# zhizdev/sparsefusion

Measured on AMD Instinct MI355X. Metric: novel views/sec, distillation steps (2 NGP renders fwd+bwd + VAE enc/dec + 51-eval PLMS + LPIPS), 256^2 / 32x32 latents, 2-view synthetic hydrant, higher is better.
Workload: dtype bf16 MFMA operands / f32 accumulate (UNet); f32 (NGP render)

## Files before the change

### sparsefusion_amd/csrc/attn_ln.h

```cpp
#pragma once
#include "sf_dev.h"

SF_KERNEL(256) void k_layernorm(const float* __restrict__ in, const float* __restrict__ gain,
                                                   const float* __restrict__ bias, void* __restrict__ out,
                                                   const float* __restrict__ resid, int R, int C, float eps, int pre_gelu,
                                                   int out_f32) {
  SF_SHARED float red[8];
  const int row = blockIdx.x, lane = threadIdx.x & 63, wv = threadIdx.x >> 6;
  const float* x = in + (long)row * C;
  float v[8];
  float s = 0.0f;
#pragma unroll
  for (int i = 0; i < 8; ++i) {
    const int c = threadIdx.x + i * 256;
    v[i] = 0.0f;
    if (c < C) { const float t = x[c]; v[i] = pre_gelu ? sf_gelu(t) : t; s += v[i]; }
  }
  s = sf_wave_sum(s);
  if (lane == 0) red[wv] = s;
  sf_sync();
  const float mean = (red[0] + red[1] + red[2] + red[3]) / (float)C;
  float q = 0.0f;
#pragma unroll
  for (int i = 0; i < 8; ++i)
    if (threadIdx.x + i * 256 < C) { const float d = v[i] - mean; q = fmaf(d, d, q); }
  q = sf_wave_sum(q);
  if (lane == 0) red[4 + wv] = q;
  sf_sync();
  const float rstd = sf_rsqrt((red[4] + red[5] + red[6] + red[7]) / (float)C + eps);
#pragma unroll
  for (int i = 0; i < 8; ++i) {
    const int c = threadIdx.x + i * 256;
    if (c < C) {
      float y = (v[i] - mean) * rstd * gain[c];
      if (bias) y += bias[c];
      if (out_f32) {
        if (resid) y += resid[(long)row * C + c];
        reinterpret_cast<float*>(out)[(long)row * C + c] = y;
      } else {
        reinterpret_cast<sf_opnd*>(out)[(long)row * C + c] = (sf_opnd)y;
      }
    }
  }
}

template <int NV>
SF_KERNEL(256) void k_layernorm_wave(const float* __restrict__ in, const float* __restrict__ gain, const float* __restrict__ bias,
                                     void* __restrict__ out, const float* __restrict__ resid, int R, float eps, int pre_gelu, int out_f32) {
  constexpr int C = 256 * NV;
  const int lane = threadIdx.x & 63;
  long row = (long)blockIdx.x * 4 + (threadIdx.x >> 6);
  const bool live = row < R;
  if (!live) row = R - 1;
  f32x4 v[NV], g[NV], bq[NV], rq[NV];
  const float* x = in + row * C;
  const float* bp = bias ? bias : gain;
  const float* rp = resid ? resid + row * C : x;
#pragma unroll
  for (int u = 0; u < NV; ++u) v[u] = *reinterpret_cast<const f32x4*>(x + (lane + 64 * u) * 4);
#pragma unroll
  for (int u = 0; u < NV; ++u) g[u] = *reinterpret_cast<const f32x4*>(gain + (lane + 64 * u) * 4);
#pragma unroll
  for (int u = 0; u < NV; ++u) bq[u] = *reinterpret_cast<const f32x4*>(bp + (lane + 64 * u) * 4);
#pragma unroll
  for (int u = 0; u < NV; ++u) rq[u] = *reinterpret_cast<const f32x4*>(rp + (lane + 64 * u) * 4);
  float s = 0.0f;
#pragma unroll
  for (int u = 0; u < NV; ++u) {
    if (pre_gelu) { v[u][0] = sf_gelu(v[u][0]); v[u][1] = sf_gelu(v[u][1]); v[u][2] = sf_gelu(v[u][2]); v[u][3] = sf_gelu(v[u][3]); }
    s += (v[u][0] + v[u][1]) + (v[u][2] + v[u][3]);
  }
  const float mean = sf_wave_sum(s) / (float)C;
  float q = 0.0f;
#pragma unroll
  for (int u = 0; u < NV; ++u)
#pragma unroll
    for (int j = 0; j < 4; ++j) { const float d = v[u][j] - mean; q = fmaf(d, d, q); }
  const float rstd = sf_rsqrt(sf_wave_sum(q) / (float)C + eps);
  if (!live) return;
#pragma unroll
  for (int u = 0; u < NV; ++u) {
    f32x4 y;
#pragma unroll
    for (int j = 0; j < 4; ++j) y[j] = (v[u][j] - mean) * rstd * g[u][j];
    if (bias) y += bq[u];
    if (out_f32) {
      if (resid) y += rq[u];
      *reinterpret_cast<f32x4*>(reinterpret_cast<float*>(out) + row * C + (lane + 64 * u) * 4) = y;
    } else {
      bf16x4 o;
      o[0] = (sf_opnd)y[0]; o[1] = (sf_opnd)y[1]; o[2] = (sf_opnd)y[2]; o[3] = (sf_opnd)y[3];
      *reinterpret_cast<bf16x4*>(reinterpret_cast<sf_opnd*>(out) + row * C + (lane + 64 * u) * 4) = o;
    }
  }
}

SF_KERNEL(256) void k_layernorm_w256(const float* __restrict__ in, const float* __restrict__ gain, const float* __restrict__ bias,
                                     void* __restrict__ out, const float* __restrict__ resid, int R, float eps, int pre_gelu, int out_f32,
                                     sf_opnd* __restrict__ twin) {
  const int lane = threadIdx.x & 63;
  const long row = (long)blockIdx.x * 4 + (threadIdx.x >> 6);
  if (row >= R) return;
  f32x4 v = *reinterpret_cast<const f32x4*>(in + row * 256 + lane * 4);
  const f32x4 g = *reinterpret_cast<const f32x4*>(gain + lane * 4);
  const f32x4 bq = bias ? *reinterpret_cast<const f32x4*>(bias + lane * 4) : f32x4{0.f, 0.f, 0.f, 0.f};
  const f32x4 rq = (resid && out_f32) ? *reinterpret_cast<const f32x4*>(resid + row * 256 + lane * 4) : f32x4{0.f, 0.f, 0.f, 0.f};
  if (pre_gelu) { v[0] = sf_gelu(v[0]); v[1] = sf_gelu(v[1]); v[2] = sf_gelu(v[2]); v[3] = sf_gelu(v[3]); }
  const float mean = sf_wave_sum((v[0] + v[1]) + (v[2] + v[3])) / 256.0f;
  const f32x4 d = v - mean;
  const float rstd = sf_rsqrt(sf_wave_sum(fmaf(d[0], d[0], fmaf(d[1], d[1], fmaf(d[2], d[2], d[3] * d[3])))) / 256.0f + eps);
  f32x4 y;
#pragma unroll
  for (int j = 0; j < 4; ++j) y[j] = d[j] * rstd * g[j] + bq[j];
  if (out_f32) {
    y = y + rq;
    *reinterpret_cast<f32x4*>(reinterpret_cast<float*>(out) + row * 256 + lane * 4) = y;
    if (twin) {
      bf16x4 o;
      o[0] = (sf_opnd)y[0]; o[1] = (sf_opnd)y[1]; o[2] = (sf_opnd)y[2]; o[3] = (sf_opnd)y[3];
      *reinterpret_cast<bf16x4*>(twin + row * 256 + lane * 4) = o;
    }
  } else {
    bf16x4 o;
    o[0] = (sf_opnd)y[0]; o[1] = (sf_opnd)y[1]; o[2] = (sf_opnd)y[2]; o[3] = (sf_opnd)y[3];
    *reinterpret_cast<bf16x4*>(reinterpret_cast<sf_opnd*>(out) + row * 256 + lane * 4) = o;
  }
}

struct AttnSeg { const float* k; const float* v; int rows, row_stride, batch_stride, head_stride; };
SF_KERNEL(256) void k_attn16(const float* __restrict__ q, void* __restrict__ out, AttnSeg s0, AttnSeg s1,
                                                AttnSeg s2, int heads, int ldq, float scale, int out_f32) {
  SF_SHARED float sq[16][65];
  SF_SHARED float sk[24][65];
  SF_SHARED float sv[24][65];
  SF_SHARED float sim[16][25];
  const int b = blockIdx.x / heads, h = blockIdx.x % heads, t = threadIdx.x & 63, wv = threadIdx.x >> 6;
  for (int i = wv; i < 16; i += 4) sq[i][t] = q[((long)b * 16 + i) * ldq + h * 64 + t] * scale;
  const AttnSeg segs[3] = {s0, s1, s2};
  int J = 0;
#pragma unroll
  for (int s = 0; s < 3; ++s) {
    for (int r = wv; r < segs[s].rows; r += 4) {
      const long off = (long)b * segs[s].batch_stride + (long)r * segs[s].row_stride + (long)h * segs[s].head_stride + t;
      sk[J + r][t] = segs[s].k[off];
      sv[J + r][t] = segs[s].v[off];
    }
    J += segs[s].rows;
  }
  sf_sync();
  for (int e = threadIdx.x; e < 16 * J; e += 256) {
    const int i = e / J, j = e - i * J;
    float a = 0.0f;
#pragma unroll 8
    for (int d = 0; d < 64; ++d) a = fmaf(sq[i][d], sk[j][d], a);
    sim[i][j] = a;
  }
  sf_sync();
  if (threadIdx.x < 16) {
    const int i = threadIdx.x;
    float mx = -INFINITY;
    for (int j = 0; j < J; ++j) mx = fmaxf(mx, sim[i][j]);
    float den = 0.0f;
    for (int j = 0; j < J; ++j) { const float e = expf(sim[i][j] - mx); sim[i][j] = e; den += e; }
    const float inv = 1.0f / den;
    for (int j = 0; j < J; ++j) sim[i][j] *= inv;
  }
  sf_sync();
  for (int i = wv; i < 16; i += 4) {
    float a = 0.0f;
    for (int j = 0; j < J; ++j) a = fmaf(sim[i][j], sv[j][t], a);
    const long o = ((long)b * 16 + i) * (heads * 64) + h * 64 + t;
    if (out_f32) reinterpret_cast<float*>(out)[o] = a;
    else reinterpret_cast<sf_opnd*>(out)[o] = (sf_opnd)a;
  }
}
```

### sparsefusion_amd/csrc/gemm_rows.h

```cpp
#pragma once
#include "sf_dev.h"

#define GR_KC 128
#define GR_LD (GR_KC + 8)

struct GemmRowsArgs {
  const float* x;
  const sf_opnd* W;
  const float* bias;
  float* y;
  int M, N, K, Kp, ldx, ldy, in_silu, out_act;
};

SF_KERNEL(256) void k_gemm_rows(GemmRowsArgs a) {
  SF_SHARED __attribute__((aligned(16))) sf_opnd hi[64 * GR_LD];
  SF_SHARED __attribute__((aligned(16))) sf_opnd lo[64 * GR_LD];
  const int tid = threadIdx.x, lane = tid & 63, wave = tid >> 6;
  const int n = lane & 15, g = lane >> 4;
  const int ncol = blockIdx.x * 64 + wave * 16 + n;
  const sf_opnd* __restrict__ wrow = a.W + (long)min(ncol, a.N - 1) * a.Kp;
  const int MF = (a.M + 15) >> 4;
  f32x4 acc[4];
#pragma unroll
  for (int mf = 0; mf < 4; ++mf) acc[mf] = f32x4{0.f, 0.f, 0.f, 0.f};
  for (int kc = 0; kc < a.K; kc += GR_KC) {
#pragma unroll 2
    for (int it = 0; it < 64 * GR_KC / 8 / 256; ++it) {
      const int idx = tid + it * 256;
      const int m = idx / (GR_KC / 8), k8 = (idx % (GR_KC / 8)) * 8;
      const float* __restrict__ xr = a.x + (long)min(m, a.M - 1) * a.ldx;
      float v[8];
#pragma unroll
      for (int j = 0; j < 8; ++j) v[j] = xr[min(kc + k8 + j, a.K - 1)];
      bf16x8 h, l;
#pragma unroll
      for (int j = 0; j < 8; ++j) {
        float t = (m < a.M && kc + k8 + j < a.K) ? v[j] : 0.0f;
        if (a.in_silu) t = sf_silu(t);
        const sf_opnd hb = (sf_opnd)t;
        h[j] = hb;
        l[j] = (sf_opnd)(t - (float)hb);
      }
      *reinterpret_cast<bf16x8*>(&hi[m * GR_LD + k8]) = h;
      *reinterpret_cast<bf16x8*>(&lo[m * GR_LD + k8]) = l;
    }
    sf_sync();
    const int left = a.K - kc;
    const int steps = left >= GR_KC ? GR_KC / 32 : (left + 31) / 32;
    for (int ks = 0; ks < steps; ++ks) {
      const int k0 = kc + ks * 32 + 8 * g;
      bf16x8 b = *reinterpret_cast<const bf16x8*>(wrow + min(k0, a.Kp - 8));
      if (k0 >= a.Kp) b = bf16x8{0, 0, 0, 0, 0, 0, 0, 0};
      const int col = ks * 32 + 8 * g;
#pragma unroll
      for (int mf = 0; mf < 4; ++mf) {
        if (mf < MF) {
          const bf16x8 ah = *reinterpret_cast<const bf16x8*>(&hi[(mf * 16 + n) * GR_LD + col]);
          const bf16x8 al = *reinterpret_cast<const bf16x8*>(&lo[(mf * 16 + n) * GR_LD + col]);
          acc[mf] = sf_mfma16(ah, b, acc[mf]);
          acc[mf] = sf_mfma16(al, b, acc[mf]);
        }
      }
    }
    sf_sync();
  }
  if (ncol < a.N) {
    const float bv = a.bias ? a.bias[ncol] : 0.0f;
#pragma unroll
    for (int mf = 0; mf < 4; ++mf)
#pragma unroll
      for (int r = 0; r < 4; ++r) {
        const int m = mf * 16 + 4 * g + r;
        if (m < a.M) {
          float v = acc[mf][r] + bv;
          if (a.out_act == 1) v = sf_silu(v);
          else if (a.out_act == 2) v = sf_sigmoid(v);
          a.y[(long)m * a.ldy + ncol] = v;
        }
      }
  }
}

template <int NW>
struct GemmRowsKs {
  static constexpr int ROWS = NW == 8 ? 32 : 64, MFMAX = ROWS / 16;
  static constexpr int WAVE_ELEMS = 2 * ROWS * GR_LD;
  static constexpr int RED = MFMAX * 4 * 64;
  static constexpr int LDS_BYTES = NW * WAVE_ELEMS * 2 + (NW - 1) * RED * 4;
  static_assert(LDS_BYTES <= 163840, "LDS");
};

template <int NW>
SF_KERNEL(NW * 64) void k_gemm_rows_ks(GemmRowsArgs a) {
  using Gk = GemmRowsKs<NW>;
  constexpr int MFMAX = Gk::MFMAX;
  SF_DYN_LDS(lds);
  const int tid = threadIdx.x, lane = tid & 63, wave = sf_uniform(tid >> 6);
  sf_opnd* hi = reinterpret_cast<sf_opnd*>(lds) + wave * Gk::WAVE_ELEMS;
  sf_opnd* lo = hi + Gk::ROWS * GR_LD;
  float* red = reinterpret_cast<float*>(lds + NW * Gk::WAVE_ELEMS * 2);
  const int n = lane & 15, g = lane >> 4;
  const int ncol = blockIdx.x * 16 + n;
  const sf_opnd* __restrict__ wrow = a.W + (long)min(ncol, a.N - 1) * a.Kp;
  const int MF = (a.M + 15) >> 4;
  const bool vec = (a.ldx & 3) == 0 && (a.K & 7) == 0 && (reinterpret_cast<uintptr_t>(a.x) & 15) == 0;
  const float bv = (a.bias ? a.bias : reinterpret_cast<const float*>(a.W))[a.bias ? min(ncol, a.N - 1) : 0];
  f32x4 acc[4];
#pragma unroll
  for (int mf = 0; mf < 4; ++mf) acc[mf] = f32x4{0.f, 0.f, 0.f, 0.f};
  for (int kc = wave * GR_KC; kc < a.K; kc += NW * GR_KC) {
    bf16x8 bw[GR_KC / 32];
#pragma unroll
    for (int ks = 0; ks < GR_KC / 32; ++ks) {
      const int k0 = kc + ks * 32 + 8 * g;
      bw[ks] = *reinterpret_cast<const bf16x8*>(wrow + min(k0, a.Kp - 8));
      if (k0 >= a.Kp) bw[ks] = bf16x8{0, 0, 0, 0, 0, 0, 0, 0};
    }
    const int lim = MF * 16 * (GR_KC / 8);
    if (vec && kc + GR_KC <= a.K) {
      f32x4 xv[4 * MFMAX][2];
#pragma unroll
      for (int it = 0; it < 4 * MFMAX; ++it) {
        const int idx = lane + it * 64;
        if (idx < lim) {
          const int m = idx / (GR_KC / 8), k8 = (idx % (GR_KC / 8)) * 8;
          const float* __restrict__ xr = a.x + (long)min(m, a.M - 1) * a.ldx + kc + k8;
          xv[it][0] = *reinterpret_cast<const f32x4*>(xr);
          xv[it][1] = *reinterpret_cast<const f32x4*>(xr + 4);
        }
      }
#pragma unroll
      for (int it = 0; it < 4 * MFMAX; ++it) {
        const int idx = lane + it * 64;
        if (idx < lim) {
          const int m = idx / (GR_KC / 8), k8 = (idx % (GR_KC / 8)) * 8;
          bf16x8 h, l;
#pragma unroll
          for (int j = 0; j < 8; ++j) {
            float t = m < a.M ? xv[it][j >> 2][j & 3] : 0.0f;
            if (a.in_silu) t = sf_silu(t);
            const sf_opnd hb = (sf_opnd)t;
            h[j] = hb;
            l[j] = (sf_opnd)(t - (float)hb);
          }
          *reinterpret_cast<bf16x8*>(&hi[m * GR_LD + k8]) = h;
          *reinterpret_cast<bf16x8*>(&lo[m * GR_LD + k8]) = l;
        }
      }
    } else
    for (int idx = lane; idx < MF * 16 * (GR_KC / 8); idx += 64) {
      const int m = idx / (GR_KC / 8), k8 = (idx % (GR_KC / 8)) * 8;
      const float* __restrict__ xr = a.x + (long)min(m, a.M - 1) * a.ldx;
      float v[8];
      if (vec && kc + k8 + 8 <= a.K) {
        const f32x4 p = *reinterpret_cast<const f32x4*>(xr + kc + k8), q = *reinterpret_cast<const f32x4*>(xr + kc + k8 + 4);
#pragma unroll
        for (int j = 0; j < 4; ++j) { v[j] = p[j]; v[4 + j] = q[j]; }
      } else {
#pragma unroll
        for (int j = 0; j < 8; ++j) v[j] = xr[min(kc + k8 + j, a.K - 1)];
      }
      bf16x8 h, l;
#pragma unroll
      for (int j = 0; j < 8; ++j) {
        float t = (m < a.M && kc + k8 + j < a.K) ? v[j] : 0.0f;
        if (a.in_silu) t = sf_silu(t);
        const sf_opnd hb = (sf_opnd)t;
        h[j] = hb;
        l[j] = (sf_opnd)(t - (float)hb);
      }
      *reinterpret_cast<bf16x8*>(&hi[m * GR_LD + k8]) = h;
      *reinterpret_cast<bf16x8*>(&lo[m * GR_LD + k8]) = l;
    }
    sf_wave_sync();
    const int left = a.K - kc;
    const int steps = left >= GR_KC ? GR_KC / 32 : (left + 31) / 32;
#pragma unroll
    for (int ks = 0; ks < GR_KC / 32; ++ks) {
      if (ks < steps) {
        const bf16x8 b = bw[ks];
        const int col = ks * 32 + 8 * g;
#pragma unroll
        for (int mf = 0; mf < MFMAX; ++mf) {
          if (mf < MF) {
            const bf16x8 ah = *reinterpret_cast<const bf16x8*>(&hi[(mf * 16 + n) * GR_LD + col]);
            const bf16x8 al = *reinterpret_cast<const bf16x8*>(&lo[(mf * 16 + n) * GR_LD + col]);
            acc[mf] = sf_mfma16(ah, b, acc[mf]);
            acc[mf] = sf_mfma16(al, b, acc[mf]);
          }
        }
      }
    }
    sf_wave_sync();
  }
  if (wave > 0) {
#pragma unroll
    for (int mf = 0; mf < MFMAX; ++mf)
#pragma unroll
      for (int r = 0; r < 4; ++r) red[(wave - 1) * Gk::RED + (mf * 4 + r) * 64 + lane] = acc[mf][r];
  }
  sf_sync();
  if (wave != 0 || ncol >= a.N) return;
#pragma unroll
  for (int mf = 0; mf < MFMAX; ++mf)
#pragma unroll
    for (int r = 0; r < 4; ++r) {
      const int m = mf * 16 + 4 * g + r;
      if (m < a.M) {
        const int o = (mf * 4 + r) * 64 + lane;
        float v = acc[mf][r];
#pragma unroll
        for (int w = 0; w < NW - 1; ++w) v += red[w * Gk::RED + o];
        v += a.bias ? bv : 0.0f;
        if (a.out_act == 1) v = sf_silu(v);
        else if (a.out_act == 2) v = sf_sigmoid(v);
        a.y[(long)m * a.ldy + ncol] = v;
      }
    }
}
```

### sparsefusion_amd/csrc/unet_ops.hip

```cpp

#include "sf_common.h"
#include "plan_ops.h"
#include "sf_dev.h"
#include "gemm_rows.h"
#include "conv_halo.h"
#include "conv_halo_small.h"
#include "conv_igemm.h"
#include "conv_igemm_t.h"
#include "attn_ln.h"
#include <math.h>

typedef __attribute__((ext_vector_type(8))) sf_opnd bf16x8;
typedef __attribute__((ext_vector_type(4))) sf_opnd bf16x4;
typedef __attribute__((ext_vector_type(4))) float f32x4;
typedef __attribute__((address_space(1))) float gfloat;

__device__ __forceinline__ void atomic_add_f32(float* p, float v) {
  (void)__builtin_amdgcn_global_atomic_fadd_f32((gfloat*)p, v);
}
__device__ __forceinline__ float silu_f(float v) { return v / (1.0f + __expf(-v)); }
__device__ __forceinline__ float sigmoid_f(float v) { return 1.0f / (1.0f + __expf(-v)); }
__device__ __forceinline__ float gelu_f(float v) { return 0.5f * v * (1.0f + erff(v * 0.70710678118654752f)); }

__device__ __forceinline__ float wave_sum(float v) {
#pragma unroll
  for (int o = 32; o > 0; o >>= 1) v += __shfl_xor(v, o, 64);
  return v;
}
__device__ __forceinline__ float wave_max(float v) {
#pragma unroll
  for (int o = 32; o > 0; o >>= 1) v = fmaxf(v, __shfl_xor(v, o, 64));
  return v;
}



__global__ __launch_bounds__(256) void k_splitk_reduce(const float* __restrict__ ws, const float* __restrict__ bias,
                                                       const float* __restrict__ resid, float* __restrict__ out, int M,
                                                       int Cout, int npad, int groups, int ldc, int co_off, int accum,
                                                       int relu, int nchw_hw) {
  const long total = (long)M * Cout;
  for (long i = blockIdx.x * 256L + threadIdx.x; i < total; i += (long)gridDim.x * 256) {
    int m, n;
    if (nchw_hw) { n = (int)((i / nchw_hw) % Cout); m = (int)(i / ((long)nchw_hw * Cout)) * nchw_hw + (int)(i % nchw_hw); }
    else { m = (int)(i / Cout); n = (int)(i - (long)m * Cout); }
    float v = bias ? bias[n] : 0.0f;
    for (int g = 0; g < groups; ++g) v += ws[((long)g * M + m) * npad + n];
    const long o = nchw_hw ? i : (long)m * ldc + co_off + n;
    if (resid) v += resid[o];
    if (accum) v += out[o];
    if (relu == 1) v = fmaxf(v, 0.0f);
    else if (relu == 2) v = 0.5f * v * (1.0f + erff(v * 0.70710678118654752f));
    out[o] = v;
  }
}

#define GN_CHUNKS_PER_BLOCK 2048

struct LazySrc {
  int mode, groups, npad, M;
  const float* a;
  const float* b;
  const float* r;
};

__device__ __forceinline__ f32x4 lazy_load4(const LazySrc& L, float* __restrict__ dst, int b, long m, int c, int C) {
  float* d = dst + m * C + c;
  f32x4 v;
  if (L.mode == 1) {
    v = L.b ? *reinterpret_cast<const f32x4*>(L.b + c) : f32x4{0.f, 0.f, 0.f, 0.f};
    for (int g = 0; g < L.groups; ++g) v += *reinterpret_cast<const f32x4*>(L.a + ((long)g * L.M + m) * L.npad + c);
    if (L.r) v += *reinterpret_cast<const f32x4*>(L.r + m * C + c);
  } else {
    const f32x4 h = *reinterpret_cast<const f32x4*>(L.a + m * C + c);
    const f32x4 g = *reinterpret_cast<const f32x4*>(L.b + (long)b * C + c);
    const f32x4 r = *reinterpret_cast<const f32x4*>((L.r ? L.r : d) + (L.r ? m * C + c : 0));
    v = h * g + r;
  }
  *reinterpret_cast<f32x4*>(d) = v;
  return v;
}

__device__ __forceinline__ f32x4 gn_load(const float* __restrict__ s1, const float* __restrict__ s2, int b, int HW, int C1,
                                         int C2, int p, int c, float s2_scale) {
  if (c < C1) return *reinterpret_cast<const f32x4*>(s1 + ((long)b * HW + p) * C1 + c);
  f32x4 v = *reinterpret_cast<const f32x4*>(s2 + ((long)b * HW + p) * C2 + (c - C1));
  return v * s2_scale;
}

__global__ __launch_bounds__(256) void k_gn_stats(float* __restrict__ s1, const float* __restrict__ s2,
                                                  double* __restrict__ stats, int HW, int C1, int C2, int slices,
                                                  float s2_scale, LazySrc lz, int G) {
  __shared__ double red[8];
  const int C = C1 + C2, Cg = C / G, cg4 = Cg / 4;
  const int bg = blockIdx.x / slices, sl = blockIdx.x % slices;
  const int b = bg / G, g = bg % G;
  const int chunks = HW * cg4;
  const int per = (chunks + slices - 1) / slices;
  const int c0 = sl * per, c1 = min(chunks, c0 + per);
  float s = 0.0f, q = 0.0f;
  for (int ch = c0 + threadIdx.x; ch < c1; ch += 256) {
    const int p = ch / cg4, c = g * Cg + (ch - p * cg4) * 4;
    const f32x4 v = (lz.mode && c < C1) ? lazy_load4(lz, s1, b, (long)b * HW + p, c, C1)
                                        : gn_load(s1, s2, b, HW, C1, C2, p, c, s2_scale);
    s += (v[0] + v[1]) + (v[2] + v[3]);
    q = fmaf(v[0], v[0], q); q = fmaf(v[1], v[1], q); q = fmaf(v[2], v[2], q); q = fmaf(v[3], v[3], q);
  }
  double ds = (double)wave_sum(s), dq = (double)wave_sum(q);
  const int lane = threadIdx.x & 63, wv = threadIdx.x >> 6;
  if (lane == 0) { red[wv] = ds; red[4 + wv] = dq; }
  __syncthreads();
  if (threadIdx.x == 0) {
    typedef __attribute__((address_space(1))) double gdouble;
    (void)__builtin_amdgcn_global_atomic_fadd_f64((gdouble*)(stats + bg * 2), red[0] + red[1] + red[2] + red[3]);
    (void)__builtin_amdgcn_global_atomic_fadd_f64((gdouble*)(stats + bg * 2 + 1), red[4] + red[5] + red[6] + red[7]);
  }
}

__global__ __launch_bounds__(256) void k_gn_stats_px(const float* __restrict__ s1, double* __restrict__ stats, int HW, int C,
                                                     int G, int slabs) {
  __shared__ float ls[256], lq[256];
  const int b = blockIdx.x / slabs, sl = blockIdx.x % slabs;
  const int c4 = C / 4, ppi = 256 / c4;
  const int chunk = threadIdx.x % c4, pofs = threadIdx.x / c4;
  const int per = (HW + slabs - 1) / slabs;
  const int p0 = sl * per, p1 = min(HW, p0 + per);
  float s = 0.0f, q = 0.0f;
  for (int p = p0 + pofs; p < p1; p += ppi) {
    const f32x4 v = *reinterpret_cast<const f32x4*>(s1 + ((long)b * HW + p) * C + chunk * 4);
    s += (v[0] + v[1]) + (v[2] + v[3]);
    q = fmaf(v[0], v[0], q); q = fmaf(v[1], v[1], q); q = fmaf(v[2], v[2], q); q = fmaf(v[3], v[3], q);
  }
  ls[threadIdx.x] = s; lq[threadIdx.x] = q;
  __syncthreads();
  if ((int)threadIdx.x < G) {
    const int cpg = c4 / G;
    double ds = 0.0, dq = 0.0;
    for (int po = 0; po < ppi; ++po)
      for (int k = 0; k < cpg; ++k) {
        const int idx = po * c4 + threadIdx.x * cpg + k;
        ds += (double)ls[idx]; dq += (double)lq[idx];
      }
    typedef __attribute__((address_space(1))) double gdouble;
    (void)__builtin_amdgcn_global_atomic_fadd_f64((gdouble*)(stats + ((long)b * G + threadIdx.x) * 2), ds);
    (void)__builtin_amdgcn_global_atomic_fadd_f64((gdouble*)(stats + ((long)b * G + threadIdx.x) * 2 + 1), dq);
  }
}

__global__ __launch_bounds__(256) void k_gn_apply(const float* __restrict__ s1, const float* __restrict__ s2,
                                                  const float* __restrict__ gamma, const float* __restrict__ beta,
                                                  const float* __restrict__ ss, const double* __restrict__ stats,
                                                  sf_opnd* __restrict__ out, sf_opnd* __restrict__ raw, int B, int HW, int C1,
                                                  int C2, int ss_stride, float eps, float s2_scale, int no_silu, int G) {
  const int C = C1 + C2, Cg = C / G, c4 = C / 4;
  const long total = (long)B * HW * c4;
  const double inv_n = 1.0 / ((double)HW * Cg);
  for (long i = blockIdx.x * 256L + threadIdx.x; i < total; i += (long)gridDim.x * 256) {
    const int c = (int)(i % c4) * 4;
    const long bp = i / c4;
    const int p = (int)(bp % HW), b = (int)(bp / HW);
    const int g = c / Cg;
    const double m = stats[(b * G + g) * 2] * inv_n;
    const double var = stats[(b * G + g) * 2 + 1] * inv_n - m * m;
    const float mean = (float)m, rstd = rsqrtf((float)(var > 0.0 ? var : 0.0) + eps);
    const f32x4 v = gn_load(s1, s2, b, HW, C1, C2, p, c, s2_scale);
    const f32x4 ga = *reinterpret_cast<const f32x4*>(gamma + c), be = *reinterpret_cast<const f32x4*>(beta + c);
    bf16x4 o, r;
#pragma unroll
    for (int j = 0; j < 4; ++j) {
      float y = (v[j] - mean) * rstd * ga[j] + be[j];
      if (ss) y = y * (ss[(long)b * ss_stride + c + j] + 1.0f) + ss[(long)b * ss_stride + C + c + j];
      if (!no_silu) y = silu_f(y);
      o[j] = (sf_opnd)y;
      r[j] = (sf_opnd)v[j];
    }
    *reinterpret_cast<bf16x4*>(out + ((long)b * HW + p) * C + c) = o;
    if (raw) *reinterpret_cast<bf16x4*>(raw + ((long)b * HW + p) * C + c) = r;
  }
}

template <int NT, int NCH>
__global__ __launch_bounds__(NT) void k_gn_one(float* __restrict__ s1, const float* __restrict__ s2, const float* __restrict__ gamma,
                                               const float* __restrict__ beta, const float* __restrict__ ss, sf_opnd* __restrict__ out,
                                               sf_opnd* __restrict__ raw, int HW, int C1, int C2, int ss_stride, float eps, float s2_scale,
                                               int no_silu, LazySrc lz, int G) {
  __shared__ double red[2][NT / 64];
  const int C = C1 + C2, Cg = C / G, cg4 = Cg / 4;
  const int b = blockIdx.x / G, g = blockIdx.x - b * G;
  const int chunks = HW * cg4;
  f32x4 v[NCH];
  float s = 0.0f, q = 0.0f;
#pragma unroll
  for (int k = 0; k < NCH; ++k) {
    const int ch = threadIdx.x + k * NT;
    v[k] = f32x4{0.f, 0.f, 0.f, 0.f};
    if (ch < chunks) {
      const int p = ch / cg4, c = g * Cg + (ch - p * cg4) * 4;
      v[k] = (lz.mode && c < C1) ? lazy_load4(lz, s1, b, (long)b * HW + p, c, C1) : gn_load(s1, s2, b, HW, C1, C2, p, c, s2_scale);
      s += (v[k][0] + v[k][1]) + (v[k][2] + v[k][3]);
      q = fmaf(v[k][0], v[k][0], q); q = fmaf(v[k][1], v[k][1], q); q = fmaf(v[k][2], v[k][2], q); q = fmaf(v[k][3], v[k][3], q);
    }
  }
  const double ds = (double)wave_sum(s), dq = (double)wave_sum(q);
  const int lane = threadIdx.x & 63, wv = threadIdx.x >> 6;
  if (lane == 0) { red[0][wv] = ds; red[1][wv] = dq; }
  __syncthreads();
  double ts = 0.0, tq = 0.0;
#pragma unroll
  for (int w = 0; w < NT / 64; ++w) { ts += red[0][w]; tq += red[1][w]; }
  const double inv_n = 1.0 / ((double)HW * Cg);
  const double m = ts * inv_n, var = tq * inv_n - m * m;
  const float mean = (float)m, rstd = rsqrtf((float)(var > 0.0 ? var : 0.0) + eps);
#pragma unroll
  for (int k = 0; k < NCH; ++k) {
    const int ch = threadIdx.x + k * NT;
    if (ch < chunks) {
      const int p = ch / cg4, c = g * Cg + (ch - p * cg4) * 4;
      const f32x4 ga = *reinterpret_cast<const f32x4*>(gamma + c), be = *reinterpret_cast<const f32x4*>(beta + c);
      bf16x4 o, r;
#pragma unroll
      for (int j = 0; j < 4; ++j) {
        float y = (v[k][j] - mean) * rstd * ga[j] + be[j];
        if (ss) y = y * (ss[(long)b * ss_stride + c + j] + 1.0f) + ss[(long)b * ss_stride + C + c + j];
        if (!no_silu) y = silu_f(y);
        o[j] = (sf_opnd)y;
        r[j] = (sf_opnd)v[k][j];
      }
      *reinterpret_cast<bf16x4*>(out + ((long)b * HW + p) * C + c) = o;
      if (raw) *reinterpret_cast<bf16x4*>(raw + ((long)b * HW + p) * C + c) = r;
    }
  }
}


template <int GEMV_ROWS>
__global__ __launch_bounds__(256) void k_gemv(const float* __restrict__ x, const sf_opnd* __restrict__ W,
                                              const float* __restrict__ bias, float* __restrict__ y, int M, int N, int K,
                                              int Kp, int ldx, int ldy, int in_silu, int out_act) {
  const int n0 = (blockIdx.x * 4 + (threadIdx.x >> 6)) * GEMV_ROWS, lane = threadIdx.x & 63;
  if (n0 >= N) return;
  float acc[GEMV_ROWS][8];
#pragma unroll
  for (int r = 0; r < GEMV_ROWS; ++r)
#pragma unroll
    for (int m = 0; m < 8; ++m) acc[r][m] = 0.0f;
  for (int k = lane * 8; k < Kp; k += 512) {
    bf16x8 w[GEMV_ROWS];
#pragma unroll
    for (int r = 0; r < GEMV_ROWS; ++r) {
      const int n = min(n0 + r, N - 1);
      w[r] = *reinterpret_cast<const bf16x8*>(W + (long)n * Kp + k);
    }
#pragma unroll
    for (int m = 0; m < 8; ++m) {
      if (m < M) {
        float xv[8];
#pragma unroll
        for (int j = 0; j < 8; ++j) {
          xv[j] = (k + j < K) ? x[(long)m * ldx + k + j] : 0.0f;
          if (in_silu) xv[j] = silu_f(xv[j]);
        }
#pragma unroll
        for (int r = 0; r < GEMV_ROWS; ++r)
#pragma unroll
          for (int j = 0; j < 8; ++j) acc[r][m] = fmaf((float)w[r][j], xv[j], acc[r][m]);
      }
    }
  }
#pragma unroll
  for (int r = 0; r < GEMV_ROWS; ++r) {
#pragma unroll
    for (int m = 0; m < 8; ++m) {
      if (m < M) {
        float v = wave_sum(acc[r][m]);
        if (lane == 0 && n0 + r < N) {
          if (bias) v += bias[n0 + r];
          if (out_act == 1) v = silu_f(v);
          else if (out_act == 2) v = sigmoid_f(v);
          y[(long)m * ldy + n0 + r] = v;
        }
      }
    }
  }
}


__global__ __launch_bounds__(256) void k_gca_logits(float* __restrict__ h, const float* __restrict__ wk,
                                                    const float* __restrict__ bk, float* __restrict__ logit, int rows, int C,
                                                    LazySrc lz) {
  const int p = blockIdx.x * 4 + (threadIdx.x >> 6), lane = threadIdx.x & 63;
  if (p >= rows) return;
  float a = 0.0f;
  for (int c = lane * 4; c < C; c += 256) {
    const f32x4 x = lz.mode ? lazy_load4(lz, h, 0, (long)p, c, C) : *reinterpret_cast<const f32x4*>(h + (long)p * C + c);
    const f32x4 w = *reinterpret_cast<const f32x4*>(wk + c);
    a += x[0] * w[0] + x[1] * w[1] + x[2] * w[2] + x[3] * w[3];
  }
  a = wave_sum(a);
  if (lane == 0) logit[p] = a + bk[0];
}

__global__ __launch_bounds__(256) void k_gca_logits_wg(float* __restrict__ h, const float* __restrict__ wk,
                                                       const float* __restrict__ bk, float* __restrict__ logit, int C, LazySrc lz) {
  __shared__ float red[4];
  const int p = blockIdx.x;
  float a = 0.0f;
  for (int c = threadIdx.x * 4; c < C; c += 1024) {
    const f32x4 x = lz.mode ? lazy_load4(lz, h, 0, (long)p, c, C) : *reinterpret_cast<const f32x4*>(h + (long)p * C + c);
    const f32x4 w = *reinterpret_cast<const f32x4*>(wk + c);
    a += x[0] * w[0] + x[1] * w[1] + x[2] * w[2] + x[3] * w[3];
  }
  a = wave_sum(a);
  if ((threadIdx.x & 63) == 0) red[threadIdx.x >> 6] = a;
  __syncthreads();
  if (threadIdx.x == 0) logit[p] = (red[0] + red[1]) + (red[2] + red[3]) + bk[0];
}

__global__ __launch_bounds__(256) void k_gca_pool(const float* __restrict__ h, const float* __restrict__ logit,
                                                  float* __restrict__ pooled, int HW, int C, int chunks, int csplit) {
  __shared__ float red[8];
  __shared__ float e[32];
  const int cs = blockIdx.x % csplit, bp = blockIdx.x / csplit;
  const int b = bp / chunks, pc = bp % chunks;
  const int lane = threadIdx.x & 63, wv = threadIdx.x >> 6;
  const float* lg = logit + (long)b * HW;
  float mx = -INFINITY;
  for (int p = threadIdx.x; p < HW; p += 256) mx = fmaxf(mx, lg[p]);
  mx = wave_max(mx);
  if (lane == 0) red[wv] = mx;
  __syncthreads();
  mx = fmaxf(fmaxf(red[0], red[1]), fmaxf(red[2], red[3]));
  float s = 0.0f;
  for (int p = threadIdx.x; p < HW; p += 256) s += expf(lg[p] - mx);
  s = wave_sum(s);
  if (lane == 0) red[4 + wv] = s;
  const int p0 = pc * 32;
  if (threadIdx.x < 32) e[threadIdx.x] = (p0 + (int)threadIdx.x < HW) ? expf(lg[p0 + threadIdx.x] - mx) : 0.0f;
  __syncthreads();
  const float inv = 1.0f / (red[4] + red[5] + red[6] + red[7]);
  const int np = min(32, HW - p0);
  const float* hb = h + ((long)b * HW + p0) * C;
  for (int c = cs * 256 + threadIdx.x; c < C; c += 256 * csplit) {
    float a = 0.0f;
    for (int p = 0; p < np; ++p) a = fmaf(e[p], hb[(long)p * C + c], a);
    atomic_add_f32(pooled + (long)b * C + c, a * inv);
  }
}

__global__ __launch_bounds__(256) void k_gate_res(const float* __restrict__ h, const float* __restrict__ gate,
                                                  const float* __restrict__ res, float* __restrict__ out, int B, int HW,
                                                  int C) {
  const long n4 = (long)B * HW * C / 4;
  for (long i = blockIdx.x * 256L + threadIdx.x; i < n4; i += (long)gridDim.x * 256) {
    const long e = i * 4;
    const int c = (int)(e % C);
    const int b = (int)(e / ((long)HW * C));
    const f32x4 hv = *reinterpret_cast<const f32x4*>(h + e);
    const f32x4 gv = *reinterpret_cast<const f32x4*>(gate + (long)b * C + c);
    const f32x4 rv = *reinterpret_cast<const f32x4*>((res ? res : out) + e);
    *reinterpret_cast<f32x4*>(out + e) = hv * gv + rv;
  }
}
__global__ __launch_bounds__(256) void k_pack_in(const float* __restrict__ cond, const float* __restrict__ x,
                                                 float* __restrict__ out, int B, int HW, int Cc, int Cx, int Cp) {
  const long n = (long)B * HW * Cp;
  for (long i = blockIdx.x * 256L + threadIdx.x; i < n; i += (long)gridDim.x * 256) {
    const int c = (int)(i % Cp);
    const long bp = i / Cp;
    const int p = (int)(bp % HW), b = (int)(bp / HW);
    float v = 0.0f;
    if (c < Cc) v = cond[((long)b * Cc + c) * HW + p];
    else if (c < Cc + Cx) v = x[((long)b * Cx + (c - Cc)) * HW + p];
    out[i] = v;
  }
}
__global__ __launch_bounds__(256) void k_pack_act(const float* __restrict__ src, bf16x8* __restrict__ out, int N, int K, int ld,
                                                  int T) {
  const int kchunks = (K + 31) / 32, n_frags = (N + 15) / 16;
  const long total = (long)n_frags * kchunks * 64;
  for (long i = blockIdx.x * 256L + threadIdx.x; i < total; i += (long)gridDim.x * 256) {
    const int lane = (int)(i & 63);
    const long r = i >> 6;
    const int ks = (int)(r % kchunks), nf = (int)(r / kchunks);
    const int n = nf * 16 + (lane & 15), c0 = ks * 32 + 8 * (lane >> 4);
    bf16x8 v;
#pragma unroll
    for (int j = 0; j < 8; ++j) {
      const int c = c0 + j;
      float x = 0.0f;
      if (n < N && c < K) x = T ? src[(long)c * ld + n] : src[(long)n * ld + c];
      v[j] = (sf_opnd)x;
    }
    out[i] = v;
  }
}

__global__ __launch_bounds__(256) void k_softmax_rows(const float* __restrict__ in, sf_opnd* __restrict__ out, int N, float scale) {
  __shared__ float red[8];
  const float* x = in + (long)blockIdx.x * N;
  const int lane = threadIdx.x & 63, wv = threadIdx.x >> 6;
  float mx = -INFINITY;
  for (int i = threadIdx.x; i < N; i += 256) mx = fmaxf(mx, x[i] * scale);
  mx = wave_max(mx);
  if (lane == 0) red[wv] = mx;
  __syncthreads();
  mx = fmaxf(fmaxf(red[0], red[1]), fmaxf(red[2], red[3]));
  float s = 0.0f;
  for (int i = threadIdx.x; i < N; i += 256) s += expf(x[i] * scale - mx);
  s = wave_sum(s);
  if (lane == 0) red[4 + wv] = s;
  __syncthreads();
  const float inv = 1.0f / (red[4] + red[5] + red[6] + red[7]);
  for (int i = threadIdx.x; i < N; i += 256) out[(long)blockIdx.x * N + i] = (sf_opnd)(expf(x[i] * scale - mx) * inv);
}

__global__ __launch_bounds__(256) void k_unpack_out(const float* __restrict__ in, float* __restrict__ out, int B, int HW,
                                                    int C, int ldi) {
  const long n = (long)B * C * HW;
  for (long i = blockIdx.x * 256L + threadIdx.x; i < n; i += (long)gridDim.x * 256) {
    const int p = (int)(i % HW);
    const long bc = i / HW;
    const int c = (int)(bc % C), b = (int)(bc / C);
    out[i] = in[((long)b * HW + p) * ldi + c];
  }
}
__global__ __launch_bounds__(256) void k_add(const float* __restrict__ a, float* __restrict__ out, long n) {
  for (long i = blockIdx.x * 256L + threadIdx.x; i < n; i += (long)gridDim.x * 256) out[i] += a[i];
}

__global__ void k_time_emb(const float* __restrict__ t, const float* __restrict__ w, float* __restrict__ out, int B,
                           int half) {
  const int i = blockIdx.x * blockDim.x + threadIdx.x;
  if (i >= B * half) return;
  const int b = i / half, j = i - b * half;
  const float fr = t[b] * w[j] * 2.0f * 3.14159265358979323846f;
  float* o = out + (long)b * (1 + 2 * half);
  if (j == 0) o[0] = t[b];
  o[1 + j] = sinf(fr);
  o[1 + half + j] = cosf(fr);
}

template <int WM, int WN>
static void launch_conv(const ConvArgs& a, bool a_fp32, int blocks, hipStream_t st) {
  if (a_fp32) k_conv_igemm<WM, WN, true><<<blocks, 256, 0, st>>>(a);
  else k_conv_igemm<WM, WN, false><<<blocks, 256, 0, st>>>(a);
}

static unsigned long long g_igemm_t_launches = 0;
extern "C" uint64_t sf_conv_igemm_t_launches(void) { return g_igemm_t_launches; }
static bool launch_conv_t(const ConvArgs& a, int WM, int WN, bool a_fp32, int blocks, hipStream_t st) {
  if (a.B != 1 || a.H != a.W || a.kh != a.kw || a.accum || a.resid || a.relu || a.co_off) return false;
  const int epi = a.pixshuf ? SF_IGT_PIXSHUF : SF_IGT_SPLITK;
  if (a.pixshuf ? (!a.slots_out || !a.bias || a.ldc * 4 != a.Cout || a.groups != 1) : (a.groups < 2 || !a.ws)) return false;
#define SF_TRY_IGT(hl_, cin_, cout_, k_, s_, p_, ups_, wm_, wn_, g_, f32_, epi_) \
  if (a.H == (1 << hl_) && a.Cin == cin_ && a.Cout == cout_ && a.kh == k_ && a.stride == s_ && a.pad == p_ && a.ups == ups_ && WM == wm_ && \
      WN == wn_ && a.groups == g_ && a_fp32 == (bool)f32_ && epi == epi_ && a.Ho == ((1 << hl_) + 2 * p_ - k_) / s_ + 1 && a.Wo == a.Ho) { \
    k_conv_igemm_t<hl_, cin_, cout_, k_, s_, p_, ups_, wm_, wn_, g_, (bool)f32_, epi_><<<blocks, 256, 0, st>>>(a); \
    ++g_igemm_t_launches; \
    return true; \
  }
  SF_IGEMM_T_VARIANTS(SF_TRY_IGT)
#undef SF_TRY_IGT
  return false;
}

static int conv_glds_depth() { return 4; }
template <int BNF, int NST, bool GN>
static int launch_conv_glds(const ConvArgs& a, int nblk, double* part, int cg, hipStream_t st) {
  static unsigned mask = 0;
  const uint32_t lds = conv_glds_lds_bytes(BNF, NST);
  int dev = 0;
  if (hipGetDevice(&dev) != hipSuccess) SF_FAIL(SF_ERR_LAUNCH, "hipGetDevice failed");
  if (dev >= 32 || !(mask & (1u << dev))) {
    if (hipFuncSetAttribute(reinterpret_cast<const void*>(&k_conv_glds<BNF, NST, GN>), hipFuncAttributeMaxDynamicSharedMemorySize, (int)lds) != hipSuccess)
      SF_FAIL(SF_ERR_LAUNCH, "hipFuncSetAttribute(max dynamic LDS) failed");
    if (dev < 32) mask |= 1u << dev;
  }
  k_conv_glds<BNF, NST, GN><<<nblk, 512, lds, st>>>(a, part, cg);
  SF_CHECK_LAUNCH("conv_glds");
  return SF_OK;
}
static bool conv_halo_enabled() { return true; }
template <int BNF, int NST, bool GN>
static int launch_conv_halo(const ConvArgs& a, int nblk, double* part, int cg, hipStream_t st) {
  static unsigned mask = 0;
  const uint32_t lds = conv_halo_lds_bytes(BNF, NST);
  int dev = 0;
  if (hipGetDevice(&dev) != hipSuccess) SF_FAIL(SF_ERR_LAUNCH, "hipGetDevice failed");
  if (dev >= 32 || !(mask & (1u << dev))) {
    if (hipFuncSetAttribute(reinterpret_cast<const void*>(&k_conv3_halo<BNF, NST, GN>), hipFuncAttributeMaxDynamicSharedMemorySize, (int)lds) != hipSuccess)
      SF_FAIL(SF_ERR_LAUNCH, "hipFuncSetAttribute(max dynamic LDS) failed");
    if (dev < 32) mask |= 1u << dev;
  }
  k_conv3_halo<BNF, NST, GN><<<nblk, 512, lds, st>>>(a, part, cg);
  SF_CHECK_LAUNCH("conv3_halo");
  return SF_OK;
}
template <int BNF, bool GN>
static int launch_conv_halo_nst(const ConvArgs& a, int nblk, double* part, int cg, int nst, hipStream_t st) {
  return nst == 3 ? launch_conv_halo<BNF, 3, GN>(a, nblk, part, cg, st) : launch_conv_halo<BNF, 4, GN>(a, nblk, part, cg, st);
}

template <int BNF, int NST, int MAPL>
static int launch_conv_halo_sm(const ConvArgs& a, int nblk, hipStream_t st) {
  static unsigned mask = 0;
  const uint32_t lds = conv_halo_sm_lds_bytes(BNF, NST, MAPL);
  int dev = 0;
  if (hipGetDevice(&dev) != hipSuccess) SF_FAIL(SF_ERR_LAUNCH, "hipGetDevice failed");
  if (dev >= 32 || !(mask & (1u << dev))) {
    if (hipFuncSetAttribute(reinterpret_cast<const void*>(&k_conv3_halo_sm<BNF, NST, MAPL>), hipFuncAttributeMaxDynamicSharedMemorySize, (int)lds) != hipSuccess)
      SF_FAIL(SF_ERR_LAUNCH, "hipFuncSetAttribute(max dynamic LDS) failed");
    if (dev < 32) mask |= 1u << dev;
  }
  k_conv3_halo_sm<BNF, NST, MAPL><<<nblk, 512, lds, st>>>(a);
  SF_CHECK_LAUNCH("conv3_halo_sm");
  return SF_OK;
}
template <int BNF>
static int launch_conv_halo_sm_nst(const ConvArgs& a, int nblk, int nst, hipStream_t st) {
  if (a.H == 4) return nst == 3 ? launch_conv_halo_sm<BNF, 3, 2>(a, nblk, st) : launch_conv_halo_sm<BNF, 4, 2>(a, nblk, st);
  return nst == 3 ? launch_conv_halo_sm<BNF, 3, 3>(a, nblk, st) : launch_conv_halo_sm<BNF, 4, 3>(a, nblk, st);
}

template <int BNF, bool GN>
static int launch_conv_glds_nst(const ConvArgs& a, int nblk, double* part, int cg, int nst, hipStream_t st) {
  return nst == 3 ? launch_conv_glds<BNF, 3, GN>(a, nblk, part, cg, st) : launch_conv_glds<BNF, 4, GN>(a, nblk, part, cg, st);
}

static int conv_splitk_tail(const sf_op& op, const ConvArgs& a, int M, hipStream_t st) {
  if (a.groups <= 1) return SF_OK;
  if (!a.ws) SF_FAIL(SF_ERR_INVALID, "conv: split-K needs a workspace");
  if (op.flags & 8) return SF_OK;
  k_splitk_reduce<<<sf_grid_cap(sf_div_up((long)M * a.Cout, 256)), 256, 0, st>>>(a.ws, a.bias, a.resid, a.out, M, a.Cout, a.npad,
                                                                                a.groups, a.ldc, a.co_off, a.accum, a.relu, a.out_nchw_hw);
  SF_CHECK_LAUNCH("splitk_reduce");
  return SF_OK;
}

static int run_conv(const sf_op& op, hipStream_t st) {
  ConvArgs a;
  a.in = op.p[0]; a.w = (const bf16x8*)op.p[1]; a.bias = (const float*)op.p[2]; a.out = (float*)op.p[3];
  a.resid = (const float*)op.p[4]; a.ws = (float*)op.p[5];
  a.accum = (op.flags & 4) ? 1 : 0;
  a.B = op.i[0]; a.H = op.i[1]; a.W = op.i[2]; a.Cin = op.i[3]; a.Ho = op.i[4]; a.Wo = op.i[5]; a.Cout = op.i[6];
  a.ldc = op.i[7]; a.co_off = op.i[8]; a.kh = op.i[9]; a.kw = op.i[10]; a.stride = op.i[11]; a.pad = op.i[12];
  a.groups = op.i[13] > 0 ? op.i[13] : 1;
  const int tile = op.i[14];
  const int WM = tile / 16, WN = tile % 16;
  a.pixshuf = (op.flags & 2) ? 1 : 0;
  a.slots_out = (float*)op.p[7];
  a.out_nchw_hw = (op.flags & 256) ? op.i[4] * op.i[5] : 0;
  a.ups = (op.flags & 16) ? 1 : 0;
  a.relu = (op.flags & 32) ? 1 : ((op.flags & 64) ? 2 : 0);
  if (a.ups && ((a.H | a.W) & 1)) SF_FAIL(SF_ERR_INVALID, "conv: upsampled input dims must be even");
  if (a.Cin % 32) SF_FAIL(SF_ERR_INVALID, "conv: Cin_pad must be a multiple of 32");
  if (a.pixshuf && a.groups != 1) SF_FAIL(SF_ERR_INVALID, "conv: pixel-shuffle epilogue cannot be split-K");
  a.cchunks = a.Cin / 32;
  a.KS = a.kh * a.kw * a.cchunks;
  const int M = a.B * a.Ho * a.Wo;
  a.m_frags = (M + 15) / 16;
  a.n_frags = (a.Cout + 15) / 16;
  a.m_tiles = (a.m_frags + WM - 1) / WM;
  a.n_tiles = (a.n_frags + WN - 1) / WN;
  a.npad = a.n_frags * 16;
  if (a.pixshuf) a.groups = 1;
  if (a.slots_out && (!a.pixshuf || tile >= 256 || (a.Cout / 4) % 16 || a.ldc % 16 || a.co_off % 16 || M % 16 || (a.Ho * a.Wo) % 16))
    SF_FAIL(SF_ERR_INVALID, "conv: output slots ride on the pixel-shuffle epilogue only (16 | Cout / 4, ldc, co_off, Ho * Wo)");
  if (a.out_nchw_hw && (a.groups < 2 || (op.flags & (8 | 4)) || op.p[4] || tile >= 256 || a.co_off || a.ldc != a.Cout))
    SF_FAIL(SF_ERR_INVALID, "conv: NCHW output is written by the (non-deferred) split-K reduction of a plain conv only");
  a.steps_per_wave = (a.KS + a.groups * 4 - 1) / (a.groups * 4);
  const int blocks = a.m_tiles * a.n_tiles * a.groups;
  const bool f32 = (op.flags & 1) != 0;
  if (tile >= 256) {
    const int bnf = (tile - 256) & 15, sel = (tile - 256) >> 4;
    if (sel != 0 && sel != 1 && sel != 3 && sel != 4 && sel != 6 && sel != 7 && sel != 8 && sel != 9)
      SF_FAIL(SF_ERR_INVALID, "conv: unknown LDS kernel selector %d", sel);
    const bool glds_ok = !f32 && a.Cin % 64 == 0 && a.Cout % 4 == 0 && a.ldc % 4 == 0 && a.co_off % 4 == 0 && (bnf == 8 || bnf == 4);
    if (sel >= 3 && !glds_ok) SF_FAIL(SF_ERR_INVALID, "conv: k_conv_glds takes operand-type activations with Cin %% 64 == 0 and float4-aligned output rows only");
    const bool special = a.groups != 1 || a.pixshuf;
    if (special && ((op.flags & 128) || sel == 6 || sel == 7 || (a.groups != 1 && !a.ws) || (a.pixshuf && ((op.flags & 4) || op.p[4] || a.relu))))
      SF_FAIL(SF_ERR_INVALID, "conv: split-K / pixel shuffle on the LDS-tiled kernels: no GroupNorm partials, not k_conv3_halo; no residual / accumulate / ReLU under the shuffle");
    const bool sm_ok = glds_ok && conv_halo_sm_ok(a) && !a.pixshuf && !(op.flags & 128);
    if (sel >= 8 && !sm_ok) SF_FAIL(SF_ERR_INVALID, "conv: k_conv3_halo_sm takes 3x3 / stride 1 / pad 1 layers on 4x4 / 8x8 maps, groups <= Cin / 64");
    const int sm = sel >= 8 ? sel - 5 : ((sel == 0 && sm_ok) ? conv_glds_depth() : 0);
    if (!sm && a.groups > (((glds_ok && sel != 1) ? a.KS : a.KS + 1) >> 1)) SF_FAIL(SF_ERR_INVALID, "conv: more split-K groups than stages");
    if (a.groups == 1 && a.pixshuf) a.ws = nullptr;
    a.m_tiles = (a.m_frags + 7) / 8;
    a.n_tiles = (a.n_frags + bnf - 1) / bnf;
    const int nblk = a.m_tiles * a.n_tiles * a.groups;
    const bool halo_ok = glds_ok && conv_halo_ok(a) && M % 128 == 0 && !special;
    if ((sel == 6 || sel == 7) && !halo_ok) SF_FAIL(SF_ERR_INVALID, "conv: k_conv3_halo takes 3x3 / stride 1 / pad 1 layers with W %% 16 == 0, H %% 8 == 0 only");
    if (sm) {
      if (int rc = bnf == 8 ? launch_conv_halo_sm_nst<8>(a, nblk, sm, st) : launch_conv_halo_sm_nst<4>(a, nblk, sm, st)) return rc;
      return conv_splitk_tail(op, a, M, st);
    }
    const int glds = (glds_ok && sel != 1 && sel < 6) ? (sel >= 3 ? sel : conv_glds_depth()) : 0;
    const int halo = (sel == 6 || sel == 7) ? sel - 3 : ((sel == 0 && halo_ok && glds && conv_halo_enabled()) ? glds : 0);
    if (op.flags & 128) {
      double* part = (double*)op.p[6];
      const int cg = op.i[15];
      if (!part || (cg != 4 && cg != 8 && cg != 16) || a.Cout % cg || a.co_off || a.ldc != a.Cout || (a.Ho * a.Wo) % 128)
        SF_FAIL(SF_ERR_INVALID, "conv: GroupNorm-partials epilogue needs whole rows, 128 | Ho*Wo, group width 4 / 8 / 16");
      if (halo) return bnf == 8 ? launch_conv_halo_nst<8, true>(a, nblk, part, cg, halo, st) : launch_conv_halo_nst<4, true>(a, nblk, part, cg, halo, st);
      if (glds) return bnf == 8 ? launch_conv_glds_nst<8, true>(a, nblk, part, cg, glds, st) : launch_conv_glds_nst<4, true>(a, nblk, part, cg, glds, st);
      if (bnf == 8) {
        if (f32) k_conv_lds_gn<8, true><<<nblk, 256, 0, st>>>(a, part, cg); else k_conv_lds_gn<8, false><<<nblk, 256, 0, st>>>(a, part, cg);
      } else if (bnf == 4) {
        if (f32) k_conv_lds_gn<4, true><<<nblk, 256, 0, st>>>(a, part, cg); else k_conv_lds_gn<4, false><<<nblk, 256, 0, st>>>(a, part, cg);
      } else {
        SF_FAIL(SF_ERR_INVALID, "conv: unsupported LDS tile %d", bnf);
      }
      SF_CHECK_LAUNCH("conv_lds_gn");
      return SF_OK;
    }
    if (halo) return bnf == 8 ? launch_conv_halo_nst<8, false>(a, nblk, nullptr, 0, halo, st) : launch_conv_halo_nst<4, false>(a, nblk, nullptr, 0, halo, st);
    if (glds) {
      if (int rc = bnf == 8 ? launch_conv_glds_nst<8, false>(a, nblk, nullptr, 0, glds, st) : launch_conv_glds_nst<4, false>(a, nblk, nullptr, 0, glds, st)) return rc;
      return conv_splitk_tail(op, a, M, st);
    }
    if (bnf == 8) {
      if (f32) k_conv_lds<8, true><<<nblk, 256, 0, st>>>(a); else k_conv_lds<8, false><<<nblk, 256, 0, st>>>(a);
    } else if (bnf == 4) {
      if (f32) k_conv_lds<4, true><<<nblk, 256, 0, st>>>(a); else k_conv_lds<4, false><<<nblk, 256, 0, st>>>(a);
    } else {
      SF_FAIL(SF_ERR_INVALID, "conv: unsupported LDS tile %d", bnf);
    }
    SF_CHECK_LAUNCH("conv_lds");
    return conv_splitk_tail(op, a, M, st);
  }
  if ((op.flags & 512) && launch_conv_t(a, WM, WN, f32, blocks, st)) {
    SF_CHECK_LAUNCH("conv_igemm_t");
    return conv_splitk_tail(op, a, M, st);
  }
  switch (tile) {
    case 1 * 16 + 1: launch_conv<1, 1>(a, f32, blocks, st); break;
    case 1 * 16 + 2: launch_conv<1, 2>(a, f32, blocks, st); break;
    case 1 * 16 + 4: launch_conv<1, 4>(a, f32, blocks, st); break;
    case 2 * 16 + 1: launch_conv<2, 1>(a, f32, blocks, st); break;
    case 2 * 16 + 2: launch_conv<2, 2>(a, f32, blocks, st); break;
    case 2 * 16 + 4: launch_conv<2, 4>(a, f32, blocks, st); break;
    case 4 * 16 + 1: launch_conv<4, 1>(a, f32, blocks, st); break;
    case 4 * 16 + 2: launch_conv<4, 2>(a, f32, blocks, st); break;
    case 4 * 16 + 4: launch_conv<4, 4>(a, f32, blocks, st); break;
    default: SF_FAIL(SF_ERR_INVALID, "conv: unsupported wave tile %dx%d", WM, WN);
  }
  SF_CHECK_LAUNCH("conv_igemm");
  return conv_splitk_tail(op, a, M, st);
}

static int lazy_from_op(const sf_op& op, int ibase, int M, LazySrc& lz) {
  lz.mode = op.i[ibase]; lz.groups = op.i[ibase + 1]; lz.npad = op.i[ibase + 2]; lz.M = M;
  lz.a = (const float*)op.p[8]; lz.b = (const float*)op.p[9]; lz.r = (const float*)op.p[10];
  if (lz.mode < 0 || lz.mode > 2) SF_FAIL(SF_ERR_INVALID, "lazy source: unknown mode %d", lz.mode);
  if (lz.mode && !lz.a) SF_FAIL(SF_ERR_INVALID, "lazy source: missing operand");
  if (lz.mode == 1 && (lz.groups < 1 || lz.npad % 4)) SF_FAIL(SF_ERR_INVALID, "lazy source: bad split-K geometry");
  if (lz.mode == 2 && !lz.b) SF_FAIL(SF_ERR_INVALID, "lazy source: gate missing");
  return SF_OK;
}

static int run_gn(const sf_op& op, hipStream_t st) {
  const int B = op.i[0], HW = op.i[1], C1 = op.i[2], C2 = op.i[3];
  const int C = C1 + C2, G = op.i[8] > 0 ? op.i[8] : 8;
  if (C % (4 * G) || C1 % 4 || !op.p[7])
    SF_FAIL(SF_ERR_INVALID, "gn_act: unsupported shape HW=%d C=%d G=%d (or missing stats buffer)", HW, C, G);
  const int chunks = HW * (C / G) / 4;
  LazySrc lz;
  if (int rc = lazy_from_op(op, 5, B * HW, lz)) return rc;
  const int c4 = C / 4;
  if (!(op.flags & (2 | 4)) && (B * G >= 256 || (B * G >= 64 && (long)B * HW * C <= (1L << 19)) || (op.flags & 8)) && chunks <= 1024 * 16) {
    float* s1 = (float*)op.p[0];
    const float *s2 = (const float*)op.p[1], *ga = (const float*)op.p[2], *be = (const float*)op.p[3], *ssp = (const float*)op.p[4];
    sf_opnd *o = (sf_opnd*)op.p[5], *rw = (sf_opnd*)op.p[6];
#define SF_GN_ONE(NT, NCH) k_gn_one<NT, NCH><<<B * G, NT, 0, st>>>(s1, s2, ga, be, ssp, o, rw, HW, C1, C2, op.i[4], op.f[0], op.f[1], op.flags & 1, lz, G)
    if (chunks <= 256 * 2) SF_GN_ONE(256, 2);
    else if (chunks <= 256 * 4) SF_GN_ONE(256, 4);
    else if (chunks <= 256 * 8) SF_GN_ONE(256, 8);
    else if (chunks <= 256 * 16) SF_GN_ONE(256, 16);
    else if (chunks <= 1024 * 8) SF_GN_ONE(1024, 8);
    else SF_GN_ONE(1024, 16);
#undef SF_GN_ONE
    SF_CHECK_LAUNCH("gn_one");
    return SF_OK;
  }
  if (op.flags & 2) {
    if (op.p[1] || lz.mode) SF_FAIL(SF_ERR_INVALID, "gn_act: ready-made statistics need a plain single source");
  } else if (!op.p[1] && !lz.mode && C / G <= 16 && c4 <= 256 && 256 % c4 == 0) {
    const int ppi = 256 / c4;
    int slabs = HW / (ppi * 16);
    slabs = slabs < 1 ? 1 : (slabs > 1024 ? 1024 : slabs);
    k_gn_stats_px<<<B * slabs, 256, 0, st>>>((const float*)op.p[0], (double*)op.p[7], HW, C, G, slabs);
  } else {
    const int per_block = lz.mode == 1 ? 256 : GN_CHUNKS_PER_BLOCK;
    int slices = (chunks + per_block - 1) / per_block;
    const int want = 128 / (B * G), max_slices = (chunks + 255) / 256;
    if (slices < want) slices = want < max_slices ? want : max_slices;
    if (slices < 1) slices = 1;
    k_gn_stats<<<B * G * slices, 256, 0, st>>>((float*)op.p[0], (const float*)op.p[1], (double*)op.p[7], HW, C1, C2, slices,
                                               op.f[1], lz, G);
  }
  SF_CHECK_LAUNCH("gn_stats");
  const long total = (long)B * HW * (C / 4);
  k_gn_apply<<<sf_grid_cap(sf_div_up(total, 256)), 256, 0, st>>>(
      (const float*)op.p[0], (const float*)op.p[1], (const float*)op.p[2], (const float*)op.p[3], (const float*)op.p[4],
      (const double*)op.p[7], (sf_opnd*)op.p[5], (sf_opnd*)op.p[6], B, HW, C1, C2, op.i[4], op.f[0], op.f[1], op.flags & 1, G);
  SF_CHECK_LAUNCH("gn_apply");
  return SF_OK;
}

static int run_ln(const sf_op& op, hipStream_t st) {
  const int R = op.i[0], C = op.i[1];
  if (C % 64 || C > 2048) SF_FAIL(SF_ERR_INVALID, "layernorm: C must be a multiple of 64 and <= 2048");
  if (C == 256 && R >= 1024) {
    k_layernorm_w256<<<sf_div_up(R, 4), 256, 0, st>>>((const float*)op.p[0], (const float*)op.p[1], (const float*)op.p[2], op.p[3],
                                                      (const float*)op.p[4], R, op.f[0], op.flags & 1, (op.flags & 2) ? 1 : 0, (sf_opnd*)op.p[5]);
    SF_CHECK_LAUNCH("layernorm_w256");
    return SF_OK;
  }
  if (op.p[5]) SF_FAIL(SF_ERR_INVALID, "layernorm: the operand-type twin output exists for >= 1024 rows of 256 channels only");
  if (R <= 256 && (C == 512 || C == 1024 || C == 2048) && !(op.flags & 4) &&
      !(((uintptr_t)op.p[0] | (uintptr_t)op.p[1] | (uintptr_t)op.p[2] | (uintptr_t)op.p[3] | (uintptr_t)op.p[4]) & 15)) {
    const uint32_t grid = sf_div_up(R, 4);
    if (C == 512) k_layernorm_wave<2><<<grid, 256, 0, st>>>((const float*)op.p[0], (const float*)op.p[1], (const float*)op.p[2], op.p[3], (const float*)op.p[4], R, op.f[0], op.flags & 1, (op.flags & 2) ? 1 : 0);
    else if (C == 1024) k_layernorm_wave<4><<<grid, 256, 0, st>>>((const float*)op.p[0], (const float*)op.p[1], (const float*)op.p[2], op.p[3], (const float*)op.p[4], R, op.f[0], op.flags & 1, (op.flags & 2) ? 1 : 0);
    else k_layernorm_wave<8><<<grid, 256, 0, st>>>((const float*)op.p[0], (const float*)op.p[1], (const float*)op.p[2], op.p[3], (const float*)op.p[4], R, op.f[0], op.flags & 1, (op.flags & 2) ? 1 : 0);
    SF_CHECK_LAUNCH("layernorm_wave");
    return SF_OK;
  }
  k_layernorm<<<R, 256, 0, st>>>((const float*)op.p[0], (const float*)op.p[1], (const float*)op.p[2], op.p[3],
                                              (const float*)op.p[4], R, C, op.f[0], op.flags & 1, (op.flags & 2) ? 1 : 0);
  SF_CHECK_LAUNCH("layernorm");
  return SF_OK;
}

static int run_gemv(const sf_op& op, hipStream_t st) {
  const int M = op.i[0], N = op.i[1];
  if (M > 64) SF_FAIL(SF_ERR_INVALID, "gemv: at most 64 rows");
  if (M > 8 || (M == 8 && N <= 4096 && !(op.flags & 8))) {
    GemmRowsArgs a{(const float*)op.p[0], (const sf_opnd*)op.p[1], (const float*)op.p[2], (float*)op.p[3], M, N, op.i[2], op.i[3], op.i[4],
                   op.i[5], (int)(op.flags & 1), (int)((op.flags >> 1) & 3)};
    if (a.Kp < 8 || a.Kp % 8) SF_FAIL(SF_ERR_INVALID, "gemv: padded K must be a multiple of 8");
    if (N <= 4096 && !(op.flags & 8)) {
      const bool w8 = M <= 32 && a.K > 4 * GR_KC;
      static unsigned mask = 0;
      int dev = 0;
      if (hipGetDevice(&dev) != hipSuccess) SF_FAIL(SF_ERR_LAUNCH, "hipGetDevice failed");
      if (dev >= 32 || !(mask & (1u << dev))) {
        if (hipFuncSetAttribute(reinterpret_cast<const void*>(&k_gemm_rows_ks<4>), hipFuncAttributeMaxDynamicSharedMemorySize, GemmRowsKs<4>::LDS_BYTES) != hipSuccess ||
            hipFuncSetAttribute(reinterpret_cast<const void*>(&k_gemm_rows_ks<8>), hipFuncAttributeMaxDynamicSharedMemorySize, GemmRowsKs<8>::LDS_BYTES) != hipSuccess)
          SF_FAIL(SF_ERR_LAUNCH, "gemv: cannot raise the dynamic LDS limit of k_gemm_rows_ks");
        if (dev < 32) mask |= 1u << dev;
      }
      if (w8) k_gemm_rows_ks<8><<<sf_div_up(N, 16), 512, GemmRowsKs<8>::LDS_BYTES, st>>>(a);
      else k_gemm_rows_ks<4><<<sf_div_up(N, 16), 256, GemmRowsKs<4>::LDS_BYTES, st>>>(a);
      SF_CHECK_LAUNCH("gemm_rows_ks");
      return SF_OK;
    }
    k_gemm_rows<<<sf_div_up(N, 64), 256, 0, st>>>(a);
    SF_CHECK_LAUNCH("gemm_rows");
    return SF_OK;
  }
  if (N <= 2048)
    k_gemv<1><<<sf_div_up(N, 4), 256, 0, st>>>((const float*)op.p[0], (const sf_opnd*)op.p[1], (const float*)op.p[2], (float*)op.p[3], M,
                                              N, op.i[2], op.i[3], op.i[4], op.i[5], op.flags & 1, (op.flags >> 1) & 3);
  else
    k_gemv<4><<<sf_div_up(N, 16), 256, 0, st>>>((const float*)op.p[0], (const sf_opnd*)op.p[1], (const float*)op.p[2], (float*)op.p[3], M,
                                               N, op.i[2], op.i[3], op.i[4], op.i[5], op.flags & 1, (op.flags >> 1) & 3);
  SF_CHECK_LAUNCH("gemv");
  return SF_OK;
}

static int run_attn(const sf_op& op, hipStream_t st) {
  AttnSeg s[3];
  int J = 0;
  for (int k = 0; k < 3; ++k) {
    s[k].k = (const float*)op.p[2 + 2 * k]; s[k].v = (const float*)op.p[3 + 2 * k];
    s[k].rows = op.i[4 + 4 * k]; s[k].row_stride = op.i[5 + 4 * k]; s[k].batch_stride = op.i[6 + 4 * k];
    s[k].head_stride = op.i[7 + 4 * k];
    J += s[k].rows;
  }
  if (J < 1 || J > 24) SF_FAIL(SF_ERR_INVALID, "attn: 1..24 keys");
  k_attn16<<<op.i[0] * op.i[1], 256, 0, st>>>((const float*)op.p[0], op.p[1], s[0], s[1], s[2], op.i[1], op.i[2], op.f[0], op.flags & 1);
  SF_CHECK_LAUNCH("attn16");
  return SF_OK;
}

static int run_gca_pool(const sf_op& op, hipStream_t st) {
  const int B = op.i[0], HW = op.i[1], C = op.i[2];
  if (HW > 1024 || C % 32 || !op.p[4]) SF_FAIL(SF_ERR_INVALID, "gca_pool: HW <= 1024, C %% 32 == 0, logits scratch required");
  LazySrc lz;
  if (int rc = lazy_from_op(op, 3, B * HW, lz)) return rc;
  if (lz.mode == 2) SF_FAIL(SF_ERR_INVALID, "gca_pool: only split-K lazy sources");
  if (B * HW <= 256)
    k_gca_logits_wg<<<B * HW, 256, 0, st>>>((float*)op.p[0], (const float*)op.p[1], (const float*)op.p[2], (float*)op.p[4], C, lz);
  else
    k_gca_logits<<<sf_div_up(B * HW, 4), 256, 0, st>>>((float*)op.p[0], (const float*)op.p[1], (const float*)op.p[2],
                                                      (float*)op.p[4], B * HW, C, lz);
  SF_CHECK_LAUNCH("gca_logits");
  const int chunks = (HW + 31) / 32;
  const int csplit = chunks < 8 ? (C + 255) / 256 : 1;
  k_gca_pool<<<B * chunks * csplit, 256, 0, st>>>((const float*)op.p[0], (const float*)op.p[4], (float*)op.p[3], HW, C, chunks,
                                                  csplit);
  SF_CHECK_LAUNCH("gca_pool");
  return SF_OK;
}

static int run_eltwise(const sf_op& op, hipStream_t st) {
  switch (op.flags) {
    case 1: {
      const long n4 = (long)op.i[0] * op.i[1] * op.i[2] / 4;
      k_gate_res<<<sf_grid_cap(sf_div_up(n4, 256)), 256, 0, st>>>((const float*)op.p[0], (const float*)op.p[1],
                                                                 (const float*)op.p[2], (float*)op.p[3], op.i[0], op.i[1], op.i[2]);
      break;
    }
    case 2: {
      const long n = (long)op.i[0] * op.i[1] * op.i[4];
      k_pack_in<<<sf_grid_cap(sf_div_up(n, 256)), 256, 0, st>>>((const float*)op.p[0], (const float*)op.p[1], (float*)op.p[3],
                                                               op.i[0], op.i[1], op.i[2], op.i[3], op.i[4]);
      break;
    }
    case 3: {
      const long n = (long)op.i[0] * op.i[1] * op.i[2];
      k_unpack_out<<<sf_grid_cap(sf_div_up(n, 256)), 256, 0, st>>>((const float*)op.p[0], (float*)op.p[3], op.i[0], op.i[1],
                                                                  op.i[2], op.i[3]);
      break;
    }
    case 4: {
      const long n = (long)(uint32_t)op.i[0];
      k_add<<<sf_grid_cap(sf_div_up(n, 256)), 256, 0, st>>>((const float*)op.p[0], (float*)op.p[3], n);
      break;
    }
    case 5: {
      const long total = (long)((op.i[0] + 15) / 16) * ((op.i[1] + 31) / 32) * 64;
      k_pack_act<<<sf_grid_cap(sf_div_up(total, 256)), 256, 0, st>>>((const float*)op.p[0], (bf16x8*)op.p[3], op.i[0], op.i[1],
                                                                   op.i[2], op.i[3]);
      break;
    }
    case 6:
      k_softmax_rows<<<op.i[0], 256, 0, st>>>((const float*)op.p[0], (sf_opnd*)op.p[3], op.i[1], op.f[0]);
      break;
    case 7: case 8: case 9: return sf_plan_extra_op(&op, st);
    default: SF_FAIL(SF_ERR_INVALID, "eltwise: unknown mode %d", op.flags);
  }
  SF_CHECK_LAUNCH("eltwise");
  return SF_OK;
}


static int plan_run_impl(const sf_op* ops, uint32_t n_ops, hipStream_t st_main, hipEvent_t* ev) {
  for (uint32_t k = 0; k < n_ops; ++k) {
    const sf_op& op = ops[k];
    int rc = SF_OK;
    hipStream_t st = st_main;
    if (ev && hipEventRecord(ev[k], st) != hipSuccess) SF_FAIL(SF_ERR_LAUNCH, "plan: hipEventRecord failed");
    switch (op.type) {
      case SF_OP_CONV: rc = run_conv(op, st); break;
      case SF_OP_GN_ACT: rc = run_gn(op, st); break;
      case SF_OP_LN: rc = run_ln(op, st); break;
      case SF_OP_GEMV: rc = run_gemv(op, st); break;
      case SF_OP_ATTN: rc = run_attn(op, st); break;
      case SF_OP_GCA_POOL: rc = run_gca_pool(op, st); break;
      case SF_OP_ELTWISE: rc = run_eltwise(op, st); break;
      case SF_OP_MEMSET:
        if (hipMemsetAsync(op.p[0], 0, (size_t)(uint32_t)op.i[0] * 4, st) != hipSuccess) SF_FAIL(SF_ERR_LAUNCH, "memset failed");
        break;
      case SF_OP_SPLITK_REDUCE: {
        const int M = op.i[0], Cout = op.i[1];
        if (!op.p[0] || !op.p[3] || op.i[3] < 1) SF_FAIL(SF_ERR_INVALID, "splitk_reduce: bad operands");
        k_splitk_reduce<<<sf_grid_cap(sf_div_up((long)M * Cout, 256)), 256, 0, st>>>(
            (const float*)op.p[0], (const float*)op.p[1], (const float*)op.p[2], (float*)op.p[3], M, Cout, op.i[2], op.i[3], Cout, 0, 0, 0, 0);
        if (hipGetLastError() != hipSuccess) SF_FAIL(SF_ERR_LAUNCH, "splitk_reduce launch failed");
        break;
      }
      case SF_OP_TIME_EMB:
        k_time_emb<<<sf_div_up(op.i[0] * op.i[1], 64), 64, 0, st>>>((const float*)op.p[0], (const float*)op.p[1], (float*)op.p[3],
                                                                  op.i[0], op.i[1]);
        if (hipGetLastError() != hipSuccess) SF_FAIL(SF_ERR_LAUNCH, "time_emb launch failed");
        break;
      case SF_OP_POOL:
      case SF_OP_LPIPS: rc = sf_plan_extra_op(&op, st); break;
      case SF_OP_EFT: rc = sf_plan_eft_op(&op, st); break;
      case SF_OP_INITX: rc = sf_plan_initx_op(&op, st); break;
      case SF_OP_GN_FINALIZE: {
        const int G = op.i[2];
        if (!op.p[0] || !op.p[1] || op.i[0] < 1 || op.i[1] < 1 || G < 1 || G > 256 || 256 % G)
          SF_FAIL(SF_ERR_INVALID, "gn_finalize: bad operands");
        k_gn_finalize<<<op.i[0] * G, 256, 0, st>>>((const double*)op.p[0], (double*)op.p[1], op.i[1], G);
        SF_CHECK_LAUNCH("gn_finalize");
        rc = SF_OK;
        break;
      }
      case SF_OP_FCONV:
        if (op.flags & 16) {
          if (k + 1 >= n_ops) SF_FAIL(SF_ERR_INVALID, "plan: a paired fconv needs a successor");
          rc = sf_plan_fused_pair(&op, &ops[k + 1], st);
          if (!rc) {
            ++k;
            if (ev && hipEventRecord(ev[k], st) != hipSuccess) SF_FAIL(SF_ERR_LAUNCH, "plan: hipEventRecord failed");
          }
          break;
        }
        rc = sf_plan_fused_op(&op, st);
        break;
      case SF_OP_SLOTS:
      case SF_OP_GCA: rc = sf_plan_fused_op(&op, st); break;
      default: SF_FAIL(SF_ERR_INVALID, "plan: unknown op type %d at %u", op.type, k);
    }
    if (rc) {
      char tmp[400];
      snprintf(tmp, sizeof(tmp), "%s", sf_err_buf);
      snprintf(sf_err_buf, sizeof(sf_err_buf), "plan op %u (type %d): %s", k, op.type, tmp);
      return rc;
    }
  }
  if (ev && hipEventRecord(ev[n_ops], st_main) != hipSuccess) SF_FAIL(SF_ERR_LAUNCH, "plan: hipEventRecord failed");
  return SF_OK;
}

extern "C" int sf_plan_run(const sf_op* ops, uint32_t n_ops, void* stream) {
  return plan_run_impl(ops, n_ops, (hipStream_t)stream, nullptr);
}

extern "C" int sf_plan_profile(const sf_op* ops, uint32_t n_ops, void* stream, float* h_ms) {
  hipStream_t st = (hipStream_t)stream;
  hipEvent_t* ev = new hipEvent_t[n_ops + 1];
  uint32_t made = 0;
  int rc = SF_OK;
  for (; made <= n_ops; ++made)
    if (hipEventCreate(&ev[made]) != hipSuccess) { rc = SF_ERR_LAUNCH; break; }
  if (rc == SF_OK) rc = plan_run_impl(ops, n_ops, st, ev);
  else snprintf(sf_err_buf, sizeof(sf_err_buf), "plan_profile: hipEventCreate failed");
  if (rc == SF_OK && hipEventSynchronize(ev[n_ops]) != hipSuccess) rc = SF_ERR_LAUNCH;
  for (uint32_t k = 0; k < n_ops && rc == SF_OK; ++k)
    if (hipEventElapsedTime(&h_ms[k], ev[k], ev[k + 1]) != hipSuccess) rc = SF_ERR_LAUNCH;
  for (uint32_t k = 0; k < made; ++k) (void)hipEventDestroy(ev[k]);
  delete[] ev;
  return rc;
}

#if SF_OPERAND_F16
static inline uint16_t f32_to_bf16_rne(float f) {
  const _Float16 h = (_Float16)f;
  uint16_t u;
  memcpy(&u, &h, 2);
  return u;
}
#else
static inline uint16_t f32_to_bf16_rne(float f) {
  uint32_t u;
  memcpy(&u, &f, 4);
  if ((u & 0x7fffffffu) > 0x7f800000u) return (uint16_t)((u >> 16) | 0x40);
  u += 0x7fffu + ((u >> 16) & 1u);
  return (uint16_t)(u >> 16);
}
#endif

extern "C" uint64_t sf_conv_packed_elems(uint32_t Cout, uint32_t cin_pad, uint32_t kh, uint32_t kw) {
  const uint64_t nfr = (Cout + 15) / 16;
  return nfr * kh * kw * (cin_pad / 32) * 64 * 8;
}

extern "C" int sf_conv_pack_weights(const float* h_w, uint32_t Cout, uint32_t Cin, uint32_t cin_pad, uint32_t kh,
                                    uint32_t kw, uint16_t* h_out) {
  if (cin_pad % 32 || cin_pad < Cin) SF_FAIL(SF_ERR_INVALID, "pack: cin_pad must be a multiple of 32 and >= Cin");
  const uint32_t nfr = (Cout + 15) / 16, cch = cin_pad / 32, taps = kh * kw;
  const uint64_t KS = (uint64_t)taps * cch;
  for (uint32_t nf = 0; nf < nfr; ++nf)
    for (uint32_t tap = 0; tap < taps; ++tap)
      for (uint32_t cc = 0; cc < cch; ++cc)
        for (uint32_t lane = 0; lane < 64; ++lane) {
          const uint32_t n = nf * 16 + (lane & 15);
          uint16_t* dst = h_out + (((uint64_t)nf * KS + (uint64_t)tap * cch + cc) * 64 + lane) * 8;
          for (uint32_t j = 0; j < 8; ++j) {
            const uint32_t c = cc * 32 + 8 * (lane >> 4) + j;
            float v = 0.0f;
            if (n < Cout && c < Cin) v = h_w[((uint64_t)n * Cin + c) * taps + tap];
            dst[j] = f32_to_bf16_rne(v);
          }
        }
  return SF_OK;
}

struct Coef6 { float alpha, sigma, alpha_next, c, noise_scale, clip; };
__global__ __launch_bounds__(256) void k_plms_update(const float* x, const float* __restrict__ eps,
                                                     const float* __restrict__ noise, Coef6 k, long n,
                                                     float* x_prev, float* __restrict__ x0) {
  for (long i = blockIdx.x * 256L + threadIdx.x; i < n; i += (long)gridDim.x * 256) {
    const float xv = x[i];
    float s = __fdiv_rn(__fsub_rn(xv, __fmul_rn(k.sigma, eps[i])), fmaxf(k.alpha, 1e-8f));
    s = fminf(fmaxf(s, -k.clip), k.clip);
    const float mean = __fmul_rn(k.alpha_next, __fadd_rn(__fdiv_rn(__fmul_rn(xv, __fsub_rn(1.0f, k.c)), k.alpha), __fmul_rn(k.c, s)));
    float out = mean;
    if (noise) out = __fadd_rn(mean, __fmul_rn(k.noise_scale, noise[i]));
    x_prev[i] = out;
    if (x0) x0[i] = s;
  }
}
__global__ __launch_bounds__(256) void k_plms_combine(const float* __restrict__ e0, const float* __restrict__ e1,
                                                      const float* __restrict__ e2, const float* __restrict__ e3, float c0,
                                                      float c1, float c2, float c3, long n, float* __restrict__ out,
                                                      float* __restrict__ keep) {
  for (long i = blockIdx.x * 256L + threadIdx.x; i < n; i += (long)gridDim.x * 256) {
    if (keep) keep[i] = e0[i];
    float v = c0 * e0[i];
    if (e1) v += c1 * e1[i];
    if (e2) v += c2 * e2[i];
    if (e3) v += c3 * e3[i];
    out[i] = v;
  }
}

__global__ __launch_bounds__(256) void k_plms_step(const float* __restrict__ e0, const float* __restrict__ e1,
                                                   const float* __restrict__ e2, const float* __restrict__ e3, float c0, float c1,
                                                   float c2, float c3, float* __restrict__ keep, const float* x,
                                                   const float* __restrict__ noise, Coef6 k, long n, float* x_prev,
                                                   int step_blocks, const float* __restrict__ row_src, float* __restrict__ row_dst, long row_n4) {
  if ((int)blockIdx.x >= step_blocks) {
    const long nb = gridDim.x - step_blocks;
    for (long i = (blockIdx.x - step_blocks) * 256L + threadIdx.x; i < row_n4; i += nb * 256)
      reinterpret_cast<float4*>(row_dst)[i] = reinterpret_cast<const float4*>(row_src)[i];
    return;
  }
  for (long i = blockIdx.x * 256L + threadIdx.x; i < n; i += (long)step_blocks * 256) {
    if (keep) keep[i] = e0[i];
    float v = c0 * e0[i];
    if (e1) v += c1 * e1[i];
    if (e2) v += c2 * e2[i];
    if (e3) v += c3 * e3[i];
    const float xv = x[i];
    float s = __fdiv_rn(__fsub_rn(xv, __fmul_rn(k.sigma, v)), fmaxf(k.alpha, 1e-8f));
    s = fminf(fmaxf(s, -k.clip), k.clip);
    const float mean = __fmul_rn(k.alpha_next, __fadd_rn(__fdiv_rn(__fmul_rn(xv, __fsub_rn(1.0f, k.c)), k.alpha), __fmul_rn(k.c, s)));
    float out = mean;
    if (noise) out = __fadd_rn(mean, __fmul_rn(k.noise_scale, noise[i]));
    x_prev[i] = out;
  }
}

extern "C" int sf_plms_step(const float* e0, const float* e1, const float* e2, const float* e3, const float* h_c4, float* keep_e0,
                            const float* x, const float* noise, const float* h_coef6, uint64_t n, float* x_prev,
                            const float* row_src, float* row_dst, uint64_t row_n, void* stream) {
  if (!e0 || !h_c4 || !x || !h_coef6 || !x_prev) SF_FAIL(SF_ERR_INVALID, "plms_step: null argument");
  if (n == 0) return SF_OK;
  if (row_n && (!row_src || !row_dst || row_n % 4 || ((uintptr_t)row_src | (uintptr_t)row_dst) % 16)) SF_FAIL(SF_ERR_INVALID, "plms_step: the row copy wants 16-byte aligned rows of 4 n floats");
  Coef6 k{h_coef6[0], h_coef6[1], h_coef6[2], h_coef6[3], h_coef6[4], h_coef6[5]};
  const int sb = (int)sf_grid_cap(sf_div_up(n, 256));
  const int rb = row_n ? (int)sf_grid_cap(sf_div_up(row_n / 4, 256)) : 0;
  k_plms_step<<<sb + rb, 256, 0, (hipStream_t)stream>>>(e0, e1, e2, e3, h_c4[0], h_c4[1], h_c4[2], h_c4[3], keep_e0, x,
                                                        noise, k, (long)n, x_prev, sb, row_src, row_dst, (long)(row_n / 4));
  SF_CHECK_LAUNCH("plms_step");
  return SF_OK;
}

extern "C" int sf_plms_update(const float* x, const float* eps, const float* noise, const float* h_coef6, uint64_t n,
                              float* x_prev, float* x0, void* stream) {
  if (!x || !eps || !h_coef6 || !x_prev) SF_FAIL(SF_ERR_INVALID, "plms_update: null argument");
  if (n == 0) return SF_OK;
  Coef6 k{h_coef6[0], h_coef6[1], h_coef6[2], h_coef6[3], h_coef6[4], h_coef6[5]};
  k_plms_update<<<sf_grid_cap(sf_div_up(n, 256)), 256, 0, (hipStream_t)stream>>>(x, eps, noise, k, (long)n, x_prev, x0);
  SF_CHECK_LAUNCH("plms_update");
  return SF_OK;
}

extern "C" int sf_plms_combine(const float* e0, const float* e1, const float* e2, const float* e3, const float* h_c4,
                               uint64_t n, float* out, float* keep_e0, void* stream) {
  if (!e0 || !h_c4 || !out) SF_FAIL(SF_ERR_INVALID, "plms_combine: null argument");
  if (n == 0) return SF_OK;
  k_plms_combine<<<sf_grid_cap(sf_div_up(n, 256)), 256, 0, (hipStream_t)stream>>>(e0, e1, e2, e3, h_c4[0], h_c4[1], h_c4[2],
                                                                                  h_c4[3], (long)n, out, keep_e0);
  SF_CHECK_LAUNCH("plms_combine");
  return SF_OK;
}
```

### sparsefusion_amd/plan.py

```python
import torch

from . import _lib

OP_CONV, OP_GN_ACT, OP_LN, OP_GEMV, OP_ATTN, OP_GCA_POOL, OP_ELTWISE, OP_MEMSET, OP_TIME_EMB, OP_SPLITK_REDUCE = range(1, 11)
OP_FCONV, OP_SLOTS, OP_GCA, OP_INITX, OP_GN_FINALIZE = 14, 15, 16, 17, 18
FNORM_NONE, FNORM_GN_SELF, FNORM_GN_SLOTS, FNORM_LN, FNORM_ATTN = range(5)
LDS_MAX = 163840
SKIP_SCALE = 2 ** -0.5


class _Arena:

    def __init__(self, nbytes=None, device=None):
        self.off = 0
        self.buf = torch.empty(nbytes, dtype=torch.uint8, device=device) if nbytes else None

    def alloc(self, nbytes):
        nbytes = (nbytes + 255) // 256 * 256
        off = self.off
        self.off += nbytes
        return (self.buf.data_ptr() + off) if self.buf is not None else (1 << 20) + off


class _T:
    __slots__ = ("ptr", "rows", "C", "HW", "lazy", "slots", "writer", "twin")

    def __init__(self, ptr, rows, C, HW=None):
        self.ptr, self.rows, self.C, self.HW = ptr, rows, C, HW
        self.lazy = None
        self.slots = None
        self.twin = None
        self.writer = None


class PlanOwner:
    conv_waves_target = 1024
    lds_conv_min_blocks = 0
    lds_mid_min_rows = 0
    lds_mid_min_batch = 8
    gn_epilogue = False
    gn_one = True
    ln_wave = True
    tb_stride = 0
    lazy_consumers = 0
    ss_total = 0
    igemm_t = 0
    igemm_t_variants = ()
    tile_override = None

    def conv_tiling(self, m_frags, n_frags, KS, pixshuf=False):
        ov = self.tile_override
        if ov and (m_frags, n_frags, KS, bool(pixshuf)) in ov:
            return ov[(m_frags, n_frags, KS, bool(pixshuf))]
        best = None
        mfma = m_frags * n_frags * KS
        w_bytes = n_frags * KS * 1024
        for WM in (1, 2, 4):
            if m_frags % WM or (m_frags <= 4 and WM != m_frags and m_frags in (1, 2, 4)):
                continue
            for WN in (1, 2, 4):
                if n_frags % WN:
                    continue
                tiles = (m_frags // WM) * (n_frags // WN)
                for groups in ((1,) if pixshuf else (1, 2, 4, 8, 16, 32)):
                    if groups > 1 and KS // (4 * groups) < 2:
                        continue
                    waves = tiles * groups * 4
                    util = min(1.0, waves / self.conv_waves_target)
                    t_hbm = w_bytes / 4.0e12 / util
                    t_l2 = mfma * 1024 * (1.0 / WN + 1.0 / WM) / 12.0e12 / util
                    t_mfma = mfma * 20 / (1024 * 2.1e9) / util
                    t_part = (2.0 * groups * m_frags * n_frags * 1024 / 3.0e12 + 2.0e-6) if groups > 1 else 0.0
                    cost = max(t_hbm, t_l2, t_mfma) + t_part + 1e-9 * WM * WN
                    if best is None or cost < best[0]:
                        best = (cost, WM, WN, groups)
        return best[1], best[2], best[3]


class Plan:

    def __init__(self, unet, B, device, sizing=None):
        self.u, self.B, self.dev = unet, B, device
        self.ops = []
        self.graph = None
        if sizing is None:
            self.zero, self.misc = _Arena(), _Arena()
        else:
            self.zero, self.misc = _Arena(sizing[0], device), _Arena(sizing[1], device)
        self.w = unet._packed(device)
        self.written = set()
        self.ws_need = [0, 0]
        self.ws_ptrs = [self.misc.alloc(sizing[2]) if sizing is not None else 0,
                        self.misc.alloc(sizing[3]) if sizing is not None and len(sizing) > 3 and sizing[3] else 0]
        self.ws_owners = [None, None]

    @property
    def ws_bytes(self):
        return self.ws_need[0]

    @property
    def ws2_bytes(self):
        return self.ws_need[1]

    @property
    def ws_owner(self):
        return next((o for o in self.ws_owners if o is not None and o.lazy is not None), None)

    def acquire_ws(self, nbytes, avoid=()):
        for i in sorted(range(2), key=lambda j: (self.ws_owners[j] is not None and self.ws_owners[j].lazy is not None, j)):
            o = self.ws_owners[i]
            if o is not None and o.lazy is not None:
                if any(o is t for t in avoid):
                    continue
                self.need(o)
            self.ws_need[i] = max(self.ws_need[i], nbytes)
            self.ws_owners[i] = None
            return i
        raise AssertionError("no split-K workspace available")

    def f32(self, rows, C, HW=None):
        return _T(self.misc.alloc(rows * C * 4), rows, C, HW)

    def bf16(self, rows, C, HW=None):
        return _T(self.misc.alloc(rows * C * 2), rows, C, HW)

    def op(self, type_, flags=0, p=(), i=(), f=()):
        o = _lib.SfOp()
        o.type, o.flags = type_, flags
        for k, v in enumerate(p):
            o.p[k] = v if v else None
        for k, v in enumerate(i):
            o.i[k] = int(v)
        for k, v in enumerate(f):
            o.f[k] = float(v)
        self.ops.append(o)

    def wptr(self, name):
        return self.w[name].data_ptr()

    def need(self, t):
        if t is None or t.lazy is None:
            return t
        lz, t.lazy = t.lazy, None
        if lz[0] == "splitk":
            _, ws, bias, resid, groups, npad, wi = lz
            self.op(OP_SPLITK_REDUCE, 0, p=(ws, bias, resid, t.ptr), i=(t.rows, t.C, npad, groups))
            self.ws_owners[wi] = None
        else:
            _, h, gate, res = lz
            self.op(OP_ELTWISE, 1, p=(h, gate, res, t.ptr), i=(self.B, t.HW, t.C))
        return t

    def take_lazy(self, t, allow):
        if t.lazy is None or t.lazy[0] not in allow:
            self.need(t)
            return (0, 0, 0), (0, 0, 0)
        lz, t.lazy = t.lazy, None
        if lz[0] == "splitk":
            self.ws_owners[lz[6]] = None
            return (lz[1], lz[2], lz[3]), (1, lz[4], lz[5])
        return (lz[1], lz[2], lz[3]), (2, 0, 0)

    def conv(self, x, x_f32, H, W, wname, bname, out, ldc, co_off, Cout, k, stride=1, pad=0, resid=None, pixshuf=False,
             defer=False, w_ptr=None, batch=None, out_hw=None, upsampled=False, relu=False, gelu=False, twin=None, want_slots=False,
             nchw=False, defer_max_groups=8):
        B = self.B if batch is None else batch
        self.need(x)
        self.need(resid)
        Ho, Wo = out_hw or ((H + 2 * pad - k) // stride + 1, (W + 2 * pad - k) // stride + 1)
        M = B * Ho * Wo
        m_frags, n_frags = (M + 15) // 16, (Cout + 15) // 16
        KS = k * k * (x.C // 32)
        WM, WN, groups = self.u.conv_tiling(m_frags, n_frags, KS, pixshuf)
        accum = (out.ptr, co_off) in self.written
        self.written.add((out.ptr, co_off))
        tile = WM * 16 + WN
        twin_ws = 0
        lds_min = self.u.lds_conv_min_blocks
        mid = self.u.lds_mid_min_rows if B >= self.u.lds_mid_min_batch else 0
        if lds_min and n_frags >= 4 and (not pixshuf or (mid and M >= mid and Cout % 4 == 0)):
            bnf = 8 if n_frags > 4 else 4
            blocks = ((m_frags + 7) // 8) * ((n_frags + bnf - 1) // bnf)
            if bnf == 8 and blocks < 256:
                bnf, blocks = 4, ((m_frags + 7) // 8) * ((n_frags + 3) // 4)
            halo = (k == 3 and stride == 1 and pad == 1 and not x_f32 and x.C % 64 == 0 and W % 16 == 0 and H % 8 == 0 and M % 128 == 0
                    and Cout % 4 == 0 and ldc % 4 == 0 and co_off % 4 == 0 and (Ho, Wo) == (H, W) and not pixshuf)
            if blocks >= (min(lds_min, 64) if halo else lds_min) and not pixshuf:
                tile, groups = 256 + bnf, 1
                if twin is not None and ldc == Cout and co_off == 0:
                    twin_ws = twin.ptr
            elif mid and M >= mid:
                glds_ok = not x_f32 and x.C % 64 == 0 and Cout % 4 == 0 and ldc % 4 == 0 and co_off % 4 == 0
                stages = KS // 2 if glds_ok else (KS + 1) // 2
                g = 1 if pixshuf else max(1, min(256 // blocks, stages // 4, 16))
                if glds_ok and k == 3 and stride == 1 and pad == 1 and H == W and H in (4, 8) and not pixshuf:
                    g = max(1, min(256 // blocks, x.C // 128, 16))
                tile, groups = 256 + bnf, g
        ws, wi = 0, 0
        if groups > 1:
            wi = self.acquire_ws(groups * M * n_frags * 16 * 4)
            ws = self.ws_ptrs[wi]
        elif twin_ws:
            ws = twin_ws
        defer = bool(defer and not relu and not gelu and 1 < groups <= defer_max_groups and not accum and not pixshuf and co_off == 0 and ldc == Cout == out.C and M == out.rows
                     and (self.u.lazy_consumers & 1))
        bias, res = self.wptr(bname) if bname else 0, resid.ptr if resid else 0
        slots = 0
        if want_slots and pixshuf and tile < 256 and (Cout // 4) % 16 == 0 and ldc % 16 == 0 and co_off % 16 == 0 and (Ho * Wo) % 16 == 0 and not accum:
            slots = self.misc.alloc(4 * M // 16 * (ldc // 16) * 2 * 4)
        nchw = bool(nchw and groups > 1 and not defer and not accum and not resid and tile < 256 and co_off == 0 and ldc == Cout)
        igt = False
        if self.u.igemm_t and tile < 256 and B == 1 and H == W and (Ho, Wo) == ((H + 2 * pad - k) // stride + 1,) * 2 and not (accum or res or relu or gelu or co_off):
            key = (H.bit_length() - 1, x.C, Cout, k, stride, pad, int(bool(upsampled)), WM, WN, groups, int(bool(x_f32)), 1 if pixshuf else 0)
            if key in self.u.igemm_t_variants and H == 1 << key[0] and (self.u.igemm_t >> self.u.igemm_t_variants.index(key)) & 1:
                igt = bool(slots and bias and ldc * 4 == Cout) if pixshuf else groups > 1
        self.op(OP_CONV, (1 if x_f32 else 0) | (2 if pixshuf else 0) | (4 if accum else 0) | (8 if defer else 0) |
                (16 if upsampled else 0) | (32 if relu else 0) | (64 if gelu else 0) | (256 if nchw else 0) | (512 if igt else 0),
                p=(x.ptr, w_ptr if w_ptr is not None else self.wptr(wname), bias, out.ptr, res, ws, 0, slots),
                i=(B, H, W, x.C, Ho, Wo, Cout, ldc, co_off, k, k, stride, pad, groups, tile))
        if defer:
            out.lazy = ("splitk", ws, bias, res, groups, n_frags * 16, wi)
            self.ws_owners[wi] = out
        out.slots = slots or None
        self.last_conv_nchw = nchw
        out.writer = self.ops[-1] if (tile >= 256 and co_off == 0 and ldc == Cout == out.C and M == out.rows) else None
        out.twin = twin if (twin is not None and tile >= 256 and groups == 1 and ws == twin.ptr) else None
        return Ho, Wo

    def gn_act(self, x, skip, gname, ss_ptr, out, raw=None, silu=True, groups=8, eps=1e-5):
        C1, C2 = x.C, (skip.C if skip else 0)
        self.need(skip)
        lp, li = self.take_lazy(x, ("splitk", "gate"))
        stats = self.zero.alloc(self.B * groups * 2 * 8)
        ready = 0
        wr = x.writer
        cg = (C1 // groups) if not skip else 0
        if (self.u.gn_epilogue and wr is not None and not (wr.flags & 128) and li[0] == 0 and cg in (4, 8, 16)
                and x.HW and x.HW % 128 == 0 and x.rows == self.B * x.HW):
            part = self.misc.alloc(x.rows // 128 * groups * 2 * 8)
            wr.flags |= 128
            wr.p[6] = part or None
            wr.i[15] = cg
            self.op(OP_GN_FINALIZE, 0, p=(part, stats), i=(self.B, x.HW // 128, groups))
            ready = 2
        self.op(OP_GN_ACT, (0 if silu else 1) | ready | (0 if self.u.gn_one else 4),
                p=(x.ptr, skip.ptr if skip else 0, self.wptr(gname + ".weight"), self.wptr(gname + ".bias"), ss_ptr, out.ptr,
                   raw.ptr if raw else 0, stats) + lp,
                i=(self.B, x.HW, C1, C2, self.u.tb_stride) + li + (groups,), f=(eps, SKIP_SCALE))

    def ln(self, x, gname, bname, out, C, rows, eps=1e-5, gelu=False, out_f32=False, resid=None, twin=None):
        self.need(x)
        self.need(resid)
        assert twin is None or (out_f32 and C == 256 and rows >= 1024)
        self.op(OP_LN, (1 if gelu else 0) | (2 if out_f32 else 0) | (0 if self.u.ln_wave else 4),
                p=(x.ptr, self.wptr(gname), self.wptr(bname) if bname else 0, out.ptr, resid.ptr if resid else 0, twin.ptr if twin else 0),
                i=(rows, C), f=(eps,))
        out.twin = twin

    def gemv(self, x_ptr, M, ldx, wname, bname, y_ptr, ldy, N, K, in_silu=False, out_act=0):
        Kp = (K + 7) // 8 * 8
        step = 8 if M <= 8 else 64
        for m0 in range(0, M, step):
            mm = min(step, M - m0)
            self.op(OP_GEMV, (1 if in_silu else 0) | (out_act << 1),
                    p=(x_ptr + m0 * ldx * 4, self.wptr(wname), self.wptr(bname) if bname else 0, y_ptr + m0 * ldy * 4),
                    i=(mm, N, K, Kp, ldx, ldy))

    def attn(self, q, out, segs, heads, ldq, scale, out_f32=False):
        p = [q.ptr, out.ptr]
        i = [self.B, heads, ldq, 0]
        for s in (segs + [None] * 3)[:3]:
            if s is None:
                p += [0, 0]
                i += [0, 0, 0, 0]
            else:
                p += [s[0], s[1]]
                i += list(s[2:])
        self.op(OP_ATTN, 1 if out_f32 else 0, p=p, i=i, f=(scale,))

    def tview(self, t):
        off = t.ptr - self.misc.buf.data_ptr()
        return self.misc.buf[off:off + t.rows * t.C * 4].view(torch.float32).view(t.rows, t.C)
```

### sparsefusion_amd/unet.py

```python
import math
import os

import numpy as np
import torch
import torch.nn as nn

from . import _lib
from .plan import (FNORM_ATTN, FNORM_GN_SELF, FNORM_GN_SLOTS, FNORM_LN, FNORM_NONE, LDS_MAX, OP_ATTN, OP_CONV, OP_ELTWISE, OP_FCONV, OP_GCA,
                   OP_GCA_POOL, OP_GEMV, OP_GN_ACT, OP_GN_FINALIZE, OP_INITX, OP_LN, OP_MEMSET, OP_SLOTS, OP_SPLITK_REDUCE, OP_TIME_EMB,
                   SKIP_SCALE, Plan, PlanOwner, _T)

PAIR_TILES = {(1, 1, 1), (1, 1, 2), (1, 2, 2), (2, 2, 2), (4, 2, 2)}
PIPE_TILES = {(1, 1, 4), (1, 2, 4), (1, 1, 6), (1, 2, 6), (2, 1, 6), (2, 2, 6), (2, 1, 8), (2, 2, 8), (2, 1, 12), (2, 2, 12), (4, 1, 16), (4, 2, 16)}
CONV3S_VARIANTS = {(5, 256, 5, 2, 2), (5, 256, 3, 2, 2), (4, 256, 4, 1, 1), (4, 256, 2, 1, 1), (4, 512, 4, 1, 2), (4, 512, 2, 1, 2),
                   (3, 512, 3, 1, 1), (3, 1024, 3, 1, 1), (5, 256, 5, 4, 2), (5, 256, 3, 4, 2),
                   (4, 256, 2, 2, 1), (4, 256, 2, 2, 2), (4, 512, 2, 2, 2), (3, 512, 3, 2, 1), (3, 1024, 3, 2, 1), (3, 1024, 3, 2, 2)}
CONV3S_RC_VARIANTS = {(5, 256, 256, 256, 3, 2, 2), (4, 512, 256, 512, 2, 1, 2), (3, 1024, 512, 1024, 3, 1, 1)}
IGEMM_T_VARIANTS = ((5, 256, 256, 4, 2, 1, 0, 2, 2, 4, 1, 0), (4, 256, 512, 4, 2, 1, 0, 1, 2, 8, 1, 0), (3, 512, 1024, 4, 2, 1, 0, 1, 1, 4, 1, 0),
                    (2, 1024, 4096, 1, 1, 0, 0, 1, 1, 1, 1, 1), (3, 1024, 2048, 1, 1, 0, 0, 1, 1, 1, 1, 1), (4, 512, 1024, 1, 1, 0, 0, 1, 2, 1, 1, 1),
                    (5, 256, 4, 3, 1, 1, 0, 1, 1, 4, 1, 0))
ATTN_LDS_BYTES = 8 * 16 * 36 * 4 + 2 * 8 * 4 * 68 * 4
TILE_PICKS = {(4, 32, 128, False): (1, 2, 8),
              (4, 128, 32, True): (1, 1, 1),
              (16, 64, 16, True): (1, 2, 1),
              (64, 1, 72, False): (1, 1, 4),
              (64, 16, 128, False): (2, 4, 4), (16, 32, 128, False): (1, 4, 4), (4, 64, 256, False): (1, 2, 4),
              (4, 64, 288, False): (1, 4, 4), (4, 256, 32, True): (1, 2, 1), (16, 128, 32, True): (1, 4, 1),
              (64, 64, 16, True): (1, 2, 1)}

SWITCHES = (
    ("conv_waves_target", 1024, "waves wanted per conv launch (4 per CU) before split-K stops"),
    ("lds_conv_min_blocks", 96, "use k_conv_lds when a layer has at least this many 128 x 128 output tiles"),
    ("lds_mid_min_rows", 128, "r06: convs of >= this many rows that have too few 128-row tiles for lds_conv_min_blocks run on the LDS-tiled kernels with split-K groups (Plan.conv); 0 = off"),
    ("igemm_t", 127, "the one-of-a-kind implicit GEMMs of the B = 1 eval on k_conv_igemm_t (compile-time geometry, csrc/conv_igemm_t.h; op flag 512): bit j = row j of IGEMM_T_VARIANTS; 0: k_conv_igemm"),
    ("gca4", 15, "the 4x4 level of the B = 1 eval on compile-time geometry (csrc/fused_gca4.h): bit 0 the stand-alone GlobalContext pooling on k_gca_pool4_t (0: k_gca_pool, op field i[8] bit 0), bit 1 the stand-alone res_conv on k_conv4_1x1_t (0: k_conv_fused, op flag 256), bit 2 pooling || res_conv on k_gca_pool4_rc_t (0: k_gca_pool_rc, both), bit 3 net0 of the 16x16 down blocks on k_gca_net0_t<256, 16> (0: k_gca_net0<16>, op field i[5] bit 0)"),
    ("merged_down_conv4", True, "r06: the merged 3x3 + 1x1 conv of the last Downsample on k_conv4_gn<64, 0, false> at B = 1; False: k_conv_igemm"),
    ("rc_small_tiles", 32, "r06: bit mask of map sides (32 | 16 | 8) whose B >= 2 (conv1 || res_conv) pairs keep the B = 1 tile of k_conv3s_rc (32: B = 2 eval 1.155 -> 1.139 ms, B = 4 1.562 -> 1.520; 32 | 16: B = 4 1.580, B = 8 2.451 -> 2.550)"),
    ("gn_one", True, "r06: GroupNorm passes of B >= 32 plans (B * 8 >= 256 workgroups) in one launch (k_gn_one); False: k_gn_stats + k_gn_apply everywhere"),
    ("lds_mid_min_batch", 8, "... in plans of at least this many images (the B = 1 .. 4 plans keep their measured kernels)"),
    ("unfused_min_rows_4", 256, "r06: 4x4-level ResnetBlocks with B*16 >= this leave the fused kernels (as unfused_min_rows at 32x32 / 16x16; measured: B = 8 loses 0.12 ms, B = 16 gains 0.22, B = 32 0.49); 0 = never"),
    ("unfused_min_rows_8", 1024, "... 8x8 level (k_conv3_halo_sm; measured: B = 8 loses 0.14 ms, B = 16 gains 0.04, B = 32 0.56)"),
    ("unfused_lin_min_rows", 256, "r06: attention / feed-forward linears of the 4x4 level with >= this many token rows leave the fused kernels (measured: B = 16 3.683 -> 3.670 ms, B = 32 4.664 -> 4.472)"),
    ("unfused_min_rows_16", 4096, "r06: the 16x16 level's own threshold (0 = unfused_min_rows; measured with k_gemm_rows_ks / the r06 plans: B = 16 3.641 -> 3.313 ms; 2048 rows lose: B = 8 2.454 -> 2.512)"),
    ("unfused_min_rows_32", 0, "... 32x32 level (4096 rows lose: B = 4 1.575 -> 1.686 ms)"),
    ("unfused_min_rows", 8192, "ResnetBlocks with B*H*W >= this at the 32x32 / 16x16 levels leave the fused kernels (_Plan.resnet; measured r03: B = 8 eval 3.33 -> 2.96 ms, B = 32 11.5 -> 7.8 ms, B = 4 unchanged)"),
    ("lazy_consumers", 3, "bit 0: split-K reductions, bit 1: gated residuals are materialised by their first consumer"),
    ("fused", True, "GroupNorm inside the conv launches (k_conv_fused) wherever the layer fits; False = the first-round plan"),
    ("pair_res_conv", True, "conv1 || res_conv of a ResnetBlock in one launch"),
    ("res_conv_beside_pool", True, "4x4 gca blocks: the res_conv shares the GlobalContext pooling launch instead"),
    ("initx_direct", True, "latent half of the init conv as one direct-convolution launch"),
    ("big_tile_min_batch", 2, "batch from which the 8x8 / 16x16 / 32x32 maps use 32- / 32- / 64-pixel tiles (r03: B = 2 eval 1.70 -> 1.50 ms, B = 4 2.62 -> 2.02, B = 32 16.4 -> 11.5; at B = 1 they would leave half the CUs idle; 999 = never)"),
    ("gca_epilogue_pool", True, "GlobalContext pooling in conv2's epilogue (False = k_gca_pool launch)"),
    ("fconv_pipe", True, "slot-GroupNorm 3x3 convs on k_conv_fused_pipe (staging || matrix work)"),
    ("producer_slots", True, "r04: k_init_x / the Upsample epilogue leave their consumers' statistics slots, the final conv's split-K reduction writes NCHW (False: the r03 k_slots / k_unpack_out launches; parity tests)"),
    ("attn_in_out_proj", True, "the 16-token attention core in the prologue of its output projection (False: k_attn16 launch; parity tests)"),
    ("ln_wave", True, "r05: LayerNorm of <= 256 rows of 512 | 1024 | 2048 channels on k_layernorm_wave (False: op flag 4 = k_layernorm)"),
    ("gate_t", True, "r05: GlobalContext gate with a compile-time hidden width (k_gca_gate_t; False: k_gca_gate)"),
    ("conv4_reduce_min_batch", 4, "r05: from this batch on a 4x4 split-K conv1 is reduced by its own launch instead of by conv2's gather (0 = never)"),
    ("conv4_mb", True, "r05: even B: the 4x4 GroupNorm-self convs run 2 | 4 images per workgroup (k_conv4_gn_mb; False = op field i[19] bit 0)"),
    ("conv4_slices_max_batch", 4, "r05: up to this batch the 4x4 GroupNorm-self convs keep 4 input-channel slices (= k_conv4_gn's geometry); 0 = the workgroup-count rule alone"),
    ("conv3s", True, "r06: the recurring single-source slot-GroupNorm 3x3 convs on k_conv3s (compile-time geometry, csrc/fused_conv3s.h); False: op field i[19] bit 1 = k_conv_fused_pipe"),
    ("conv3s_tw32", 8, "r06: tile width of k_conv3s's 2-D pixel tiles per map size (0 = full-width strips)"),
    ("conv3s_tw16", 4, "... 16x16 maps"),
    ("conv3s_tw8", 0, "... 8x8 maps"),
    ("conv4", True, "r05: the 4x4 level's GroupNorm-self 3x3 convs on k_conv4_gn (csrc/fused_conv4.h); False: op flag 128 = k_conv_fused (parity tests)"),
    ("use_hip_graph", True, "replay one captured hipGraph per eval instead of ~370 host launches"),
)


def init_x_weight_table(ws, dtype=torch.bfloat16):
    parts, offs, acc = [], [], 0
    for w in ws:
        cw, ci, k, _ = w.shape
        steps = {15: 30, 7: 7, 3: 2}[k]
        nfr = cw // 16
        wp = torch.zeros(cw, 4, k + 2, 16 + 2)
        wp[:, :ci, :k, :k] = w
        t = torch.zeros(steps, nfr, 64, 8)
        for s in range(steps):
            for g in range(4):
                if k == 15:
                    ky, kx0 = s // 2, 8 * (s % 2) + 2 * g
                elif k == 7:
                    ky, kx0 = s, 2 * g
                else:
                    ky, kx0 = 2 * s + g // 2, 2 * (g % 2)
                blk = wp[:, :, ky, kx0:kx0 + 2]
                t[s, :, g * 16:(g + 1) * 16, :] = blk.permute(0, 2, 1).reshape(nfr, 16, 8)
        parts.append(t.reshape(-1))
        offs.append(acc)
        acc += steps * nfr
    return torch.cat(parts).to(dtype).view(torch.int16).contiguous(), offs


def _cast_tuple(v, n):
    return tuple(v) if isinstance(v, (tuple, list)) else (v,) * n


def unet_param_spec(dim=256, dim_mults=(1, 2, 4, 4), num_resnet_blocks=(2, 2, 2, 2),
                    layer_attns=(False, False, False, True), cond_images_channels=256, channels=4, cond_dim=None,
                    attn_heads=8, attn_dim_head=64, ff_mult=2, learned_sinu_pos_emb_dim=16, max_conditional_len=256):
    cond_dim = cond_dim or dim
    tdim = dim * 4
    inner = attn_heads * attn_dim_head
    dims = [dim] + [dim * m for m in dim_mults]
    in_out = list(zip(dims[:-1], dims[1:]))
    n_lv = len(in_out)
    nres = _cast_tuple(num_resnet_blocks, n_lv)
    attns = _cast_tuple(layer_attns, n_lv)
    spec = [("null_conditional_embed", (1, max_conditional_len, cond_dim)), ("null_conditional_hidden", (1, tdim))]
    cin0 = channels + cond_images_channels
    scales = [dim // 2, dim // 4]
    scales.append(dim - sum(scales))
    for i, (k, co) in enumerate(zip((3, 7, 15), scales)):
        spec += [(f"init_conv.convs.{i}.weight", (co, cin0, k, k)), (f"init_conv.convs.{i}.bias", (co,))]
    spec += [("to_time_hiddens.0.weights", (learned_sinu_pos_emb_dim // 2,)),
             ("to_time_hiddens.1.weight", (tdim, learned_sinu_pos_emb_dim + 1)), ("to_time_hiddens.1.bias", (tdim,)),
             ("to_time_cond.0.weight", (tdim, tdim)), ("to_time_cond.0.bias", (tdim,)),
             ("to_time_tokens.0.weight", (cond_dim * 2, tdim)), ("to_time_tokens.0.bias", (cond_dim * 2,)),
             ("norm_cond.weight", (cond_dim,)), ("norm_cond.bias", (cond_dim,))]

    def resnet(p, cin, cout, gca, cross):
        s = [(f"{p}.time_mlp.1.weight", (cout * 2, tdim)), (f"{p}.time_mlp.1.bias", (cout * 2,))]
        if cross:
            s += [(f"{p}.cross_attn.fn.null_kv", (2, attn_dim_head)), (f"{p}.cross_attn.fn.norm.g", (cout,)),
                  (f"{p}.cross_attn.fn.to_q.weight", (inner, cout)), (f"{p}.cross_attn.fn.to_kv.weight", (inner * 2, cond_dim)),
                  (f"{p}.cross_attn.fn.to_out.0.weight", (cout, inner)), (f"{p}.cross_attn.fn.to_out.1.g", (cout,))]
        for b, ci in (("block1", cin), ("block2", cout)):
            s += [(f"{p}.{b}.groupnorm.weight", (ci,)), (f"{p}.{b}.groupnorm.bias", (ci,)),
                  (f"{p}.{b}.project.weight", (cout, ci, 3, 3)), (f"{p}.{b}.project.bias", (cout,))]
        if gca:
            s += [(f"{p}.gca.to_k.weight", (1, cout, 1, 1)), (f"{p}.gca.to_k.bias", (1,)),
                  (f"{p}.gca.net.0.weight", (max(3, cout // 2), cout, 1, 1)), (f"{p}.gca.net.0.bias", (max(3, cout // 2),)),
                  (f"{p}.gca.net.2.weight", (cout, max(3, cout // 2), 1, 1)), (f"{p}.gca.net.2.bias", (cout,))]
        if cin != cout:
            s += [(f"{p}.res_conv.weight", (cout, cin, 1, 1)), (f"{p}.res_conv.bias", (cout,))]
        return s

    def attention(p, d, context):
        s = [(f"{p}.null_kv", (2, attn_dim_head)), (f"{p}.norm.g", (d,)), (f"{p}.to_q.weight", (inner, d)),
             (f"{p}.to_kv.weight", (attn_dim_head * 2, d))]
        if context:
            s += [(f"{p}.to_context.0.weight", (cond_dim,)), (f"{p}.to_context.0.bias", (cond_dim,)),
                  (f"{p}.to_context.1.weight", (attn_dim_head * 2, cond_dim)), (f"{p}.to_context.1.bias", (attn_dim_head * 2,))]
        return s + [(f"{p}.to_out.0.weight", (d, inner)), (f"{p}.to_out.1.g", (d,))]

    def transformer(p, d):
        hid = int(d * ff_mult)
        return attention(f"{p}.layers.0.0.fn", d, True) + [
            (f"{p}.layers.0.1.0.g", (1, d, 1, 1)), (f"{p}.layers.0.1.1.weight", (hid, d, 1, 1)),
            (f"{p}.layers.0.1.3.g", (1, hid, 1, 1)), (f"{p}.layers.0.1.4.weight", (d, hid, 1, 1))]

    for lv, (di, do) in enumerate(in_out):
        last = lv == n_lv - 1
        spec += resnet(f"downs.{lv}.1", di, di, False, False)
        for r in range(nres[lv]):
            spec += resnet(f"downs.{lv}.2.{r}", di, di, True, False)
        if attns[lv]:
            spec += transformer(f"downs.{lv}.3", di)
        if not last:
            spec += [(f"downs.{lv}.4.weight", (do, di, 4, 4)), (f"downs.{lv}.4.bias", (do,))]
        else:
            spec += [(f"downs.{lv}.4.fns.0.weight", (do, di, 3, 3)), (f"downs.{lv}.4.fns.0.bias", (do,)),
                     (f"downs.{lv}.4.fns.1.weight", (do, di, 1, 1)), (f"downs.{lv}.4.fns.1.bias", (do,))]
    for ui, lv in enumerate(reversed(range(n_lv))):
        di, do = in_out[lv]
        last = ui == n_lv - 1
        spec += resnet(f"ups.{ui}.0", do + di, do, False, False)
        for r in range(nres[lv]):
            spec += resnet(f"ups.{ui}.1.{r}", do + di, do, True, False)
        if attns[lv]:
            spec += transformer(f"ups.{ui}.2", do)
        if not last:
            spec += [(f"ups.{ui}.3.net.0.weight", (di * 4, do, 1, 1)), (f"ups.{ui}.3.net.0.bias", (di * 4,))]
    mid = dims[-1]
    spec += resnet("mid_block1", mid, mid, False, True)
    spec += attention("mid_attn.fn.fn", mid, False)
    spec += resnet("mid_block2", mid, mid, False, True)
    spec += resnet("final_res_block", dim, dim, True, False)
    spec += [("final_conv.weight", (channels, dim, 3, 3)), ("final_conv.bias", (channels,))]
    return spec


class _Node(nn.Module):
    """Anonymous container used to reproduce the reference's dotted parameter names."""


def _register(root, dotted, tensor):
    parts = dotted.split(".")
    node = root
    for p in parts[:-1]:
        if p not in node._modules:
            node.add_module(p, _Node())
        node = node._modules[p]
    node.register_parameter(parts[-1], nn.Parameter(tensor))


class _Plan(Plan):

    def fused_geometry(self, H, C, Cout, norm, k):
        B = self.B
        if not self.u.fused or H not in (4, 8, 16, 32) or C % 32 or Cout % 16:
            return None
        TR, WM = {4: (4, 1), 8: (2, 1), 16: (1, 1), 32: (1, 2)}[H]
        if B >= self.u.big_tile_min_batch and H in (8, 16, 32):
            fit3 = self._fused_geometry(H, C, Cout, norm if k == 3 else FNORM_GN_SLOTS, 3, 2 * TR, 2 * WM)
            g = self._fused_geometry(H, C, Cout, norm, k, 2 * TR, 2 * WM)
            if fit3 is not None and g is not None:
                return g
        return self._fused_geometry(H, C, Cout, norm, k, TR, WM)

    def _fused_geometry(self, H, C, Cout, norm, k, TR, WM):
        B = self.B
        n_frags = Cout // 16
        MT = B * (H // TR)
        h = k // 2

        pipe_ok = (self.u.fconv_pipe and norm == FNORM_GN_SLOTS and k == 3 and C % 128 == 0
                   and ((TR + 2) * H) % 8 == 0)

        def lds_bytes(S_, WN_):
            if pipe_ok and S_ == 1 and (WM, WN_, (TR + 2) * H // 8) in PIPE_TILES:
                return self.pipe_lds_bytes(H, C, TR, WM, WN_)
            Cs = C // S_
            stride = Cs * 2 + ((32 - (Cs * 2) % 256) + 256) % 256
            return ((TR + 2 * h) * (H + 2 * h) + 1) * stride + 8192 * WM * WN_ + 2 * Cs * 4 + 2688 + (ATTN_LDS_BYTES + 16 if norm == FNORM_ATTN else 0)

        cand = [1]
        if norm in (FNORM_GN_SELF, FNORM_GN_SLOTS):
            if C % 8:
                return None
            Cg = C // 8
            if Cg % 4 or (norm == FNORM_GN_SLOTS and Cg % 16):
                return None
            if norm == FNORM_GN_SELF:
                if H != 4:
                    return None
                cand = [d for d in (1, 2, 4, 8) if (C // 32) % d == 0 and (C // d) % Cg == 0]
        cand = [d for d in cand if lds_bytes(d, 1) <= LDS_MAX]
        if not cand:
            return None
        S = next((d for d in cand if MT * n_frags * d >= 256), cand[-1])
        if ((B <= self.u.conv4_slices_max_batch or (self.u.conv4_mb and B % 2 == 0)) and self.u.conv4
                and norm == FNORM_GN_SELF and H == 4 and k == 3 and C in (1024, 2048) and 4 in cand):
            S = 4
        WN = 2 if (n_frags % 2 == 0 and MT * (n_frags // 2) * S >= 256 and lds_bytes(S, 2) <= LDS_MAX and norm != FNORM_GN_SELF) else 1
        return TR, WM, WN, S

    @staticmethod
    def pipe_lds_bytes(H, C, TR, WM, WN, pool=False):
        buf = (((TR + 2) * (H + 2) + 1) * 288 + 15) // 16 * 16
        return 2 * buf + 4096 * (WM * WN + (WM if pool else 0)) + 2 * C * 4 + 2688 + (9 * (C // 32) * 64 if pool else 0)

    def ensure_slots(self, t):
        if t.slots is not None and t.lazy is None:
            return t
        assert t.rows % 16 == 0 and t.C % 16 == 0
        slots = self.misc.alloc(t.rows // 16 * (t.C // 16) * 2 * 4)
        if t.lazy is not None and t.lazy[0] == "gate" and t.lazy[3] and t.lazy[3] != t.ptr:
            _, h, gate, res = t.lazy
            t.lazy = None
            self.op(OP_SLOTS, 0, p=(h, gate, res, t.ptr, slots), i=(t.rows, t.C, t.HW))
        elif t.lazy is not None and t.lazy[0] == "splitk" and not t.lazy[3] and t.lazy[5] % 4 == 0:
            _, ws, bias, _, groups, npad, wi = t.lazy
            t.lazy = None
            self.ws_owners[wi] = None
            self.op(OP_SLOTS, 0, p=(0, 0, 0, t.ptr, slots, ws, bias), i=(t.rows, t.C, t.HW or t.rows, groups, npad))
        else:
            self.need(t)
            self.op(OP_SLOTS, 0, p=(t.ptr, 0, 0, 0, slots), i=(t.rows, t.C, t.HW or t.rows))
        t.slots = slots
        return t

    def fconv(self, x, skip, H, wname, bname, out, Cout, k, norm, geom, gname=None, ss_ptr=0, silu=True, resid=None,
              want_slots=False, pre_gelu=False, beta_name=None, ldc=None, co_off=0, logit=None, out_gelu=False,
              pair_first=False, pair_lazy=None, pool=None, attn=None):
        TR, WM, WN, S = geom
        B = self.B
        C1, C2 = x.C, (skip.C if skip else 0)
        self.need(skip)
        self.need(resid)
        if norm == FNORM_GN_SLOTS:
            self.ensure_slots(x)
            if skip:
                self.ensure_slots(skip)
        ldc = ldc or Cout
        accum = (out.ptr, co_off) in self.written
        n_frags = (Cout + 15) // 16
        ws, wi = 0, 0
        if S > 1:
            assert not accum and ldc == Cout and co_off == 0
            wi = self.acquire_ws(S * x.rows * n_frags * 16 * 4, avoid=(x,))
            ws = self.ws_ptrs[wi]
        else:
            self.written.add((out.ptr, co_off))
        lp, li = (0, 0, 0), (0, 0, 0)
        x_ptr = x.ptr
        if pair_lazy is not None:
            lp, li = pair_lazy
            if li[0]:
                x_ptr = 0
        elif x.lazy is not None:
            if x.lazy[0] == "gate" and (not x.lazy[3] or x.lazy[3] == x.ptr):
                self.need(x)
            else:
                lp, li = self.take_lazy(x, ("splitk", "gate"))
        slots_out = 0
        if want_slots and S == 1:
            if out.slots is None:
                out.slots = self.misc.alloc(out.rows // 16 * (ldc // 16) * 2 * 4)
            slots_out = out.slots
        bias, res = (self.wptr(bname) if bname else 0), (resid.ptr if resid else 0)
        gam = self.wptr(gname + ".weight") if norm in (FNORM_GN_SELF, FNORM_GN_SLOTS) else (self.wptr(gname) if gname else 0)
        bet = self.wptr(gname + ".bias") if norm in (FNORM_GN_SELF, FNORM_GN_SLOTS) else (self.wptr(beta_name) if beta_name else 0)
        assert not (out_gelu and S > 1)
        pipe = self.pipe_ok(C1, C2, H, geom, norm, k, silu) and li[0] == 0 and pair_lazy is None
        if pool is not None:
            assert pipe and logit is None and not accum and resid is None and ldc == Cout and co_off == 0
            logit = pool
        ap, ai, af = (), (), ()
        if attn is not None:
            segs, ldq, scale = attn
            assert norm == FNORM_ATTN and len(segs) <= 3 and not silu and x.lazy is None and lp == (0, 0, 0)
            segs = list(segs) + [(0, 0, 0, 0, 0, 0)] * (3 - len(segs))
            assert all((sv - sk) % 4 == 0 and 0 <= (sv - sk) // 4 < (1 << 24) for sk, sv, *_ in segs)
            ap = tuple(sk for sk, *_ in segs)
            ai = (ldq,) + tuple(v for _, _, rows, rs, bs, hs in segs for v in (rows, rs, bs, hs))
            af = tuple((sv - sk) // 4 for sk, sv, *_ in segs) + (scale,)
        elif norm == FNORM_GN_SELF and not self.u.conv4_mb:
            ai = (1,)
        elif pipe:
            code = 0 if self.u.conv3s else 2
            tw = self.conv3s_tw(H)
            if (code == 0 and tw and tw != H and C2 == 0 and Cout == C1 and ldc == Cout and co_off == 0 and not accum and not out_gelu and not pre_gelu
                    and not pair_first and pair_lazy is None and (logit is None or pool is not None) and bname
                    and (H.bit_length() - 1, C1, tw.bit_length() - 1, WM, WN) in CONV3S_VARIANTS):
                code |= tw << 2
            elif (code == 0 and pair_first and C2 and ldc == Cout and co_off == 0 and not accum and not out_gelu and not pre_gelu and logit is None and bname
                    and (H.bit_length() - 1, C1, C2, Cout, (tw or H).bit_length() - 1, WM, WN) in CONV3S_RC_VARIANTS):
                code |= (tw if tw != H else 0) << 2
            ai = (code,)
# ... 17 lines not shown
    def conv3s_tw(self, H):
        return getattr(self.u, f"conv3s_tw{H}")

    def pipe_ok(self, C1, C2, H, geom, norm, k, silu=True):
        TR, WM, WN, S = geom
        return bool(self.u.fconv_pipe and norm == FNORM_GN_SLOTS and k == 3 and S == 1 and silu
                    and (C1 + C2) % 128 == 0 and C1 % 4 == 0 and ((TR + 2) * H) % 8 == 0 and (WM, WN, (TR + 2) * H // 8) in PIPE_TILES)

    def resnet_fused(self, name, x, skip, cout, H, gca=False, cross=False):
        B, HW = self.B, H * H
        cin = x.C + (skip.C if skip else 0)
        rows = B * HW
        norm = FNORM_GN_SELF if H == 4 else FNORM_GN_SLOTS
        g1 = self.fused_geometry(H, cin, cout, norm, 3)
        g2 = self.fused_geometry(H, cout, cout, norm, 3)
        gr = self.fused_geometry(H, cin, cout, FNORM_NONE, 1) if cin != cout else g1
        if g1 is None or g2 is None or gr is None or x.C % 32 or rows % 16:
            return None
        if (B >= 2 and (self.u.rc_small_tiles & H) and cin != cout and skip is not None and self.u.conv3s
                and self.u.pair_res_conv):
            TR0, WM0 = {8: (2, 1), 16: (1, 1), 32: (1, 2)}[H]
            s1, sr = self._fused_geometry(H, cin, cout, norm, 3, TR0, WM0), self._fused_geometry(H, cin, cout, FNORM_NONE, 1, TR0, WM0)
            tw = self.conv3s_tw(H) or H
            if (s1 is not None and sr is not None and s1[1:3] == sr[1:3] and sr[3] == 1
                    and (H.bit_length() - 1, x.C, skip.C, cout, tw.bit_length() - 1, s1[1], s1[2]) in CONV3S_RC_VARIANTS):
                g1, gr = s1, sr
        slots = norm == FNORM_GN_SLOTS
        h = self.f32(rows, cout, HW)
        pair = (cin != cout and self.u.pair_res_conv and g1[1:3] == gr[1:3] and gr[3] == 1
                and (g1[1], g1[2], norm) in PAIR_TILES)
        late_rc = (cin != cout and gca and H == 4 and self.u.res_conv_beside_pool and gr[1:4] == (1, 1, 1)
                   and cout % 64 == 0 and cout <= 2048 and cin <= 4096)
        conv4_geom = (H == 4 and self.u.conv4 and g1[1:3] == (1, 1) and g1[3] > 1 and cin // g1[3] in (256, 512)
                      and (cin // 8) * 2 == cin // g1[3])
        pair = pair and not late_rc and not conv4_geom
        lz = self.fconv(x, skip, H, f"{name}.block1.project.weight", f"{name}.block1.project.bias", h, cout, 3, norm, g1,
                        gname=f"{name}.block1.groupnorm", want_slots=slots, pair_first=pair)
        rc = None
        emit_rc = None
        if cin != cout:
            rc = self.f32(rows, cout, HW)
            emit_rc = lambda first=False: self.fconv(x, skip, H, f"{name}.res_conv.weight", f"{name}.res_conv.bias", rc, cout, 1,
                                                     FNORM_NONE, gr, silu=False, pair_lazy=lz if pair else None, pair_first=first)
            if not late_rc:
                emit_rc()
                thr = self.u.conv4_reduce_min_batch
                if pair and thr and B >= thr and H == 4 and norm == FNORM_GN_SELF and h.lazy is not None and h.lazy[0] == "splitk":
                    self.need(h)
        if cross:
            h = self.cross_attention(f"{name}.cross_attn.fn", h)
        ss_ptr = self.ss.ptr + self.u.ss_offset[name] * 4
        w2, b2, gn2 = f"{name}.block2.project.weight", f"{name}.block2.project.bias", f"{name}.block2.groupnorm"
        res = rc if rc is not None else x
        out = self.f32(rows, cout, HW)
        if not gca:
            self.fconv(h, None, H, w2, b2, out, cout, 3, norm, g2, gname=gn2, ss_ptr=ss_ptr, resid=res, want_slots=slots)
            return out
        h2 = self.f32(rows, cout, HW)
        if (self.u.gca_epilogue_pool and cout % 64 == 0 and cout <= 2048 and HW % 16 == 0 and HW // 16 <= 64
                and self.pipe_ok(cout, 0, H, g2, norm, 3) and h.lazy is None and f"{name}.__weff__" in self.w
                and self.pipe_lds_bytes(H, cout, g2[0], g2[1], g2[2], pool=True) <= LDS_MAX):
            if late_rc:
                emit_rc()
            pbuf = self.f32(rows // 16, cout + 2)
            self.fconv(h, None, H, w2, b2, h2, cout, 3, norm, g2, gname=gn2, ss_ptr=ss_ptr, pool=(self.wptr(f"{name}.__weff__"), pbuf.ptr))
            self.gca_fused(name, h2, cout, res, out, None, 0, slots, pooled=(pbuf.ptr, pbuf.ptr + rows // 16 * cout * 4, HW // 16))
            return out
        if cout % 64 == 0 and cout <= 2048 and HW % 16 == 0:
            nparts = g2[3] * (cout // 16)
            lpart = self.f32(nparts, rows)
            self.fconv(h, None, H, w2, b2, h2, cout, 3, norm, g2, gname=gn2, ss_ptr=ss_ptr,
                       logit=(self.wptr(f"{name}.gca.to_k.weight"), lpart.ptr))
            self.gca_fused(name, h2, cout, res, out, lpart, nparts, slots, before_pool=emit_rc if late_rc else None)
            return out
        if late_rc:
            emit_rc()
        self.fconv(h, None, H, w2, b2, h2, cout, 3, norm, g2, gname=gn2, ss_ptr=ss_ptr)
        gate = self.gca_gate(name, h2, cout)
        out.lazy = ("gate", h2.ptr, gate.ptr, res.ptr)
        return out

    def gca_fused(self, name, h2, cout, res, out, lpart, nparts, want_slots, pooled=None, before_pool=None):
        B, HW, rows = self.B, h2.HW, h2.rows
        chunks = min(8, HW // 16)
        CH = HW // chunks
        hidc = max(3, cout // 2)
        part_pool, part_ms, hid = self.f32(B * chunks, cout), self.f32(B * chunks, 2), self.f32(B, hidc)
        ws = bias = groups = npad = 0
        if h2.lazy is not None:
            assert h2.lazy[0] == "splitk" and not h2.lazy[3]
            _, ws, bias, _, groups, npad, wi = h2.lazy
            h2.lazy = None
            self.ws_owners[wi] = None
        if before_pool is None:
            self.need(res)
        if pooled is not None:
            pp, pm, chunks = pooled
        else:
            pp, pm = part_pool.ptr, part_ms.ptr
            if before_pool is not None:
                before_pool(True)
            keep4 = B == 1 and HW == 16 and not (self.u.gca4 >> (2 if before_pool is not None else 0)) & 1
            self.op(OP_GCA, 1, p=(h2.ptr, ws, bias, lpart.ptr, pp, pm), i=(rows, cout, HW, CH, chunks, nparts, groups, npad, 1 if keep4 else 0))
        if want_slots:
            out.slots = self.misc.alloc(rows // 16 * (cout // 16) * 2 * 4)
        self.op(OP_GCA, 2, p=(pp, pm, self.wptr(f"{name}.gca.net.0.weight"), self.wptr(f"{name}.gca.net.0.bias"),
                              hid.ptr), i=(B, cout, (cout + 7) // 8 * 8, hidc, chunks,
                                           0 if self.u.gate_t and not (B == 1 and cout == 256 and 8 < chunks <= 16 and not self.u.gca4 & 8) else 1))
        self.op(OP_GCA, 3, p=(h2.ptr, res.ptr, hid.ptr, self.wptr(f"{name}.gca.net.2.weight"), self.wptr(f"{name}.gca.net.2.bias"),
                              out.ptr, out.slots or 0), i=(rows, cout, HW, hidc, (hidc + 7) // 8 * 8, 0 if self.u.gate_t else 1))

    def gca_gate(self, name, h2, cout):
        B, HW = self.B, h2.HW
        pooled = _T(self.zero.alloc(B * cout * 4), B, cout)
        hid = self.f32(B, max(3, cout // 2))
        gate = self.f32(B, cout)
        logits = self.f32(B, HW)
        lp, li = self.take_lazy(h2, ("splitk",))
        self.op(OP_GCA_POOL, 0, p=(h2.ptr, self.wptr(f"{name}.gca.to_k.weight"), self.wptr(f"{name}.gca.to_k.bias"), pooled.ptr,
                                   logits.ptr, 0, 0, 0) + lp, i=(B, HW, cout) + li)
        self.gemv(pooled.ptr, B, cout, f"{name}.gca.net.0.weight", f"{name}.gca.net.0.bias", hid.ptr, hid.C, hid.C, cout,
                  out_act=1)
        self.gemv(hid.ptr, B, hid.C, f"{name}.gca.net.2.weight", f"{name}.gca.net.2.bias", gate.ptr, cout, cout, hid.C,
                  out_act=2)
        return gate

    def resnet(self, name, x, skip, cout, H, gca=False, cross=False):
        B, HW = self.B, H * H
        cin = x.C + (skip.C if skip else 0)
        rows = B * HW
        lvl = getattr(self.u, f"unfused_min_rows_{H}") if H in (4, 8, 16, 32) else 0
        big = (rows >= (lvl or self.u.unfused_min_rows) and H % 16 == 0 and cin % 64 == 0
               and cout % 64 == 0)
        low = lvl if H in (4, 8) else 0
        big = big or bool(low and rows >= low and self.u.lds_mid_min_rows and cin % 64 == 0 and cout % 64 == 0)
        if self.u.fused and not big:
            y = self.resnet_fused(name, x, skip, cout, H, gca, cross)
            if y is not None:
                return y
        a1 = self.bf16(rows, cin, HW)
        raw = self.bf16(rows, cin, HW) if cin != cout else None
        self.gn_act(x, skip, f"{name}.block1.groupnorm", 0, a1, raw)
        h = self.f32(rows, cout, HW)
        self.conv(a1, False, H, H, f"{name}.block1.project.weight", f"{name}.block1.project.bias", h, cout, 0, cout, 3, 1, 1,
                  defer=True)
        if cross:
            h = self.cross_attention(f"{name}.cross_attn.fn", h)
        a2 = self.bf16(rows, cout, HW)
        ss_ptr = self.ss.ptr + self.u.ss_offset[name] * 4
        self.gn_act(h, None, f"{name}.block2.groupnorm", ss_ptr, a2)
        out = self.f32(rows, cout, HW)
        w2, b2 = f"{name}.block2.project.weight", f"{name}.block2.project.bias"
        if gca:
            h2 = self.f32(rows, cout, HW)
            self.conv(a2, False, H, H, w2, b2, h2, cout, 0, cout, 3, 1, 1, defer=True)
            pooled = _T(self.zero.alloc(B * cout * 4), B, cout)
            hid = self.f32(B, max(3, cout // 2))
            gate = self.f32(B, cout)
            logits = self.f32(B, HW)
            lp, li = self.take_lazy(h2, ("splitk",))
            self.op(OP_GCA_POOL, 0, p=(h2.ptr, self.wptr(f"{name}.gca.to_k.weight"), self.wptr(f"{name}.gca.to_k.bias"), pooled.ptr,
                                       logits.ptr, 0, 0, 0) + lp, i=(B, HW, cout) + li)
            self.gemv(pooled.ptr, B, cout, f"{name}.gca.net.0.weight", f"{name}.gca.net.0.bias", hid.ptr, hid.C, hid.C, cout,
                      out_act=1)
            self.gemv(hid.ptr, B, hid.C, f"{name}.gca.net.2.weight", f"{name}.gca.net.2.bias", gate.ptr, cout, cout, hid.C,
                      out_act=2)
            if raw is not None:
                self.conv(raw, False, H, H, f"{name}.res_conv.weight", f"{name}.res_conv.bias", out, cout, 0, cout, 1)
                out.lazy = ("gate", h2.ptr, gate.ptr, 0)
            else:
                out.lazy = ("gate", h2.ptr, gate.ptr, x.ptr)
            if not (self.u.lazy_consumers & 2):
                self.need(out)
        else:
            if raw is not None:
                self.conv(raw, False, H, H, f"{name}.res_conv.weight", f"{name}.res_conv.bias", out, cout, 0, cout, 1)
                self.conv(a2, False, H, H, w2, b2, out, cout, 0, cout, 3, 1, 1)
            else:
                self.conv(a2, False, H, H, w2, b2, out, cout, 0, cout, 3, 1, 1, resid=x)
        return out

    def _attn_out(self, name, att, x, d, rows):
        o = self.f32(rows, d)
        self.conv(att, False, 1, rows // self.B, f"{name}.to_out.0.weight", None, o, d, 0, d, 1)
        y = self.f32(rows, d, x.HW)
        self.ln(o, f"{name}.to_out.1.g", None, y, d, rows, out_f32=True, resid=x)
        return y

    def lin_geometry(self, x, N, norm):
        if x.HW != 16 or x.rows != self.B * 16:
            return None
        if x.rows >= self.u.unfused_lin_min_rows and self.u.lds_mid_min_rows:
            return None
        return self.fused_geometry(4, x.C, N, norm, 1)

    def attention_fused(self, name, x, context, cross):
        B, d, rows = self.B, x.C, x.rows
        heads, dh = self.u.attn_heads, self.u.attn_dim_head
        inner = heads * dh
        nq = inner if cross else inner + 2 * dh
        g1, g2 = self.lin_geometry(x, nq, FNORM_LN), None
        if g1 is None or d % 32:
            return None
        att = _T(self.misc.alloc(rows * inner * 4), rows, inner, 16)
        g2 = self.lin_geometry(att, d, FNORM_ATTN)
        if g2 is None:
            return None
        self.need(x)
        qkv = self.f32(rows, nq, 16)
        self.fconv(x, None, 4, f"{name}.to_q.weight" if cross else f"{name}.__qkv__", None, qkv, nq, 1, FNORM_LN, g1,
                   gname=f"{name}.norm.g", silu=False)
        nk = self.wptr(f"{name}.null_kv")
        segs = []
        if cross:
            kvp = self.tb.ptr + self.u.tb_off[name] * 4
            segs = [(nk, nk + dh * 4, 1, 0, 0, 0), (kvp, kvp + inner * 4, 2, inner * 2, self.u.tb_stride, dh)]
        else:
            if context:
                ckvp = self.tb.ptr + self.u.tb_off[name] * 4
                segs.append((ckvp, ckvp + dh * 4, 2, 2 * dh, self.u.tb_stride, 0))
            kp = qkv.ptr + inner * 4
            segs += [(nk, nk + dh * 4, 1, 0, 0, 0), (kp, kp + dh * 4, 16, nq, 16 * nq, 0)]
        o = self.f32(rows, d, 16)
        nkeys, per_head = sum(sg[2] for sg in segs), any(sg[5] for sg in segs if sg[2])
        if self.u.attn_in_out_proj and heads == 8 and dh == 64 and len(segs) <= 3 and 1 <= nkeys <= (4 if per_head else 24):
            qv = _T(qkv.ptr, rows, inner, 16)
            self.fconv(qv, None, 4, f"{name}.to_out.0.weight", None, o, d, 1, FNORM_ATTN, g2, silu=False, attn=(segs, nq, dh ** -0.5))
        else:
            self.attn(qkv, att, segs, heads, nq, dh ** -0.5, out_f32=True)
            self.fconv(att, None, 4, f"{name}.to_out.0.weight", None, o, d, 1, FNORM_NONE, g2, silu=False)
        y = self.f32(rows, d, x.HW)
        self.ln(o, f"{name}.to_out.1.g", None, y, d, rows, out_f32=True, resid=x)
        return y

    def cross_attention(self, name, h):
        if self.u.fused:
            y = self.attention_fused(name, h, False, True)
            if y is not None:
                return y
        B, d, rows = self.B, h.C, h.rows
        heads, dh = self.u.attn_heads, self.u.attn_dim_head
        inner = heads * dh
        xn = self.bf16(rows, d)
        self.ln(h, f"{name}.norm.g", None, xn, d, rows)
        q = self.f32(rows, inner)
        self.conv(xn, False, 1, rows // B, f"{name}.to_q.weight", None, q, inner, 0, inner, 1)
        att = self.bf16(rows, inner)
        nk = self.wptr(f"{name}.null_kv")
        kvp = self.tb.ptr + self.u.tb_off[name] * 4
        segs = [(nk, nk + dh * 4, 1, 0, 0, 0), (kvp, kvp + inner * 4, 2, inner * 2, self.u.tb_stride, dh)]
        self.attn(q, att, segs, heads, inner, dh ** -0.5)
        return self._attn_out(name, att, h, d, rows)

    def self_attention(self, name, x, context):
        if self.u.fused:
            y = self.attention_fused(name, x, context, False)
            if y is not None:
                return y
        B, d, rows = self.B, x.C, x.rows
        heads, dh = self.u.attn_heads, self.u.attn_dim_head
        inner = heads * dh
        xn = self.bf16(rows, d)
        self.ln(x, f"{name}.norm.g", None, xn, d, rows)
        q, kv = self.f32(rows, inner), self.f32(rows, 2 * dh)
        self.conv(xn, False, 1, rows // B, f"{name}.to_q.weight", None, q, inner, 0, inner, 1)
        self.conv(xn, False, 1, rows // B, f"{name}.to_kv.weight", None, kv, 2 * dh, 0, 2 * dh, 1)
        segs = []
        if context:
            ckvp = self.tb.ptr + self.u.tb_off[name] * 4
            segs.append((ckvp, ckvp + dh * 4, 2, 2 * dh, self.u.tb_stride, 0))
        nk = self.wptr(f"{name}.null_kv")
        tok = rows // B
        segs += [(nk, nk + dh * 4, 1, 0, 0, 0), (kv.ptr, kv.ptr + dh * 4, tok, 2 * dh, tok * 2 * dh, 0)]
        att = self.bf16(rows, inner)
        self.attn(q, att, segs, heads, inner, dh ** -0.5)
        return self._attn_out(name, att, x, d, rows)

    def transformer(self, name, x):
        B, d, rows = self.B, x.C, x.rows
        x1 = self.self_attention(f"{name}.layers.0.0.fn", x, True)
        hid = int(d * self.u.ff_mult)
        if self.u.fused:
            ga, gb = self.lin_geometry(x1, hid, FNORM_LN), None
            if ga is not None and hid % 32 == 0:
                f1 = self.f32(rows, hid, 16)
                gb = self.lin_geometry(f1, d, FNORM_LN)
            if ga is not None and gb is not None:
                self.fconv(x1, None, 4, f"{name}.layers.0.1.1.weight", None, f1, hid, 1, FNORM_LN, ga,
                           gname=f"{name}.layers.0.1.0.g", silu=False, out_gelu=True)
                x2 = self.f32(rows, d, x.HW)
                self.fconv(f1, None, 4, f"{name}.layers.0.1.4.weight", None, x2, d, 1, FNORM_LN, gb,
                           gname=f"{name}.layers.0.1.3.g", silu=False, resid=x1)
                return x2
        xn = self.bf16(rows, d)
        self.ln(x1, f"{name}.layers.0.1.0.g", None, xn, d, rows)
        f1 = self.f32(rows, hid)
        self.conv(xn, False, 1, rows // B, f"{name}.layers.0.1.1.weight", None, f1, hid, 0, hid, 1)
        xn3 = self.bf16(rows, hid)
        self.ln(f1, f"{name}.layers.0.1.3.g", None, xn3, hid, rows, gelu=True)
        x2 = self.f32(rows, d, x.HW)
        self.conv(xn3, False, 1, rows // B, f"{name}.layers.0.1.4.weight", None, x2, d, 0, d, 1, resid=x1)
        return x2

    def emit_time(self, rows, tb_ptr, t_ptr):
        u = self.u
        st = u.tb_stride
        half = u.learned_sinu_pos_emb_dim // 2
        heads, dh = u.attn_heads, u.attn_dim_head
        four, hid, t = self.f32(rows, 2 * half + 1), self.f32(rows, u.tdim), self.f32(rows, u.tdim)
        tok = self.f32(rows, 2 * u.cond_dim)
        self.op(OP_TIME_EMB, 0, p=(t_ptr, self.wptr("to_time_hiddens.0.weights"), 0, four.ptr), i=(rows, half))
        self.gemv(four.ptr, rows, four.C, "to_time_hiddens.1.weight", "to_time_hiddens.1.bias", hid.ptr, u.tdim, u.tdim, four.C, out_act=1)
        self.gemv(hid.ptr, rows, u.tdim, "to_time_cond.0.weight", "to_time_cond.0.bias", t.ptr, u.tdim, u.tdim, u.tdim)
        self.gemv(hid.ptr, rows, u.tdim, "to_time_tokens.0.weight", "to_time_tokens.0.bias", tok.ptr, 2 * u.cond_dim, 2 * u.cond_dim, u.tdim)
        c = self.f32(2 * rows, u.cond_dim)
        self.ln(tok, "norm_cond.weight", "norm_cond.bias", c, u.cond_dim, 2 * rows, out_f32=True)
        self.gemv(t.ptr, rows, u.tdim, "__time_mlps__.weight", "__time_mlps__.bias", tb_ptr, st, u.ss_total, u.tdim, in_silu=True)
        for name, off in u.tb_off.items():
            if name.endswith(".cross_attn.fn"):
                n_out, src, wname, bname = 2 * heads * dh, c, f"{name}.to_kv.weight", None
            else:
                src = self.f32(2 * rows, u.cond_dim)
                self.ln(c, f"{name}.to_context.0.weight", f"{name}.to_context.0.bias", src, u.cond_dim, 2 * rows, out_f32=True)
                n_out, wname, bname = 2 * dh, f"{name}.to_context.1.weight", f"{name}.to_context.1.bias"
            for tk in range(2):
                self.gemv(src.ptr + tk * u.cond_dim * 4, rows, 2 * u.cond_dim, wname, bname, tb_ptr + (off + tk * n_out) * 4, st,
                          n_out, u.cond_dim)

    def build(self):
        u, B = self.u, self.B
        R = u.image_size
        HW = R * R
        cin0 = u.channels + u.cond_images_channels
        cpad = (cin0 + 31) // 32 * 32
        self.x_in, self.t_in = self.f32(B, u.channels * HW), self.f32(B, 1)
        self.cond_in = self.f32(B, u.cond_images_channels * HW)
        self.tb = self.f32(B, u.tb_stride)
        self.ss = self.tb
        self.emit_time(B, self.tb.ptr, self.t_in.ptr)
        self.n_time_ops = len(self.ops)
        self.op(OP_MEMSET, 0, p=(self.zero.buf.data_ptr() if self.zero.buf is not None else 1,), i=(0,))
        memset_op = self.ops[-1]
        xin = self.f32(B * HW, cpad, HW)
        self.op(OP_ELTWISE, 2, p=(self.cond_in.ptr, self.x_in.ptr, 0, xin.ptr), i=(B, HW, u.cond_images_channels, u.channels, cpad))
        x = self.f32(B * HW, u.dim, HW)
        co = 0
        for i, k in enumerate((3, 7, 15)):
            cw = u.spec_shapes[f"init_conv.convs.{i}.weight"][0]
            self.conv(xin, True, R, R, f"init_conv.convs.{i}.weight", f"init_conv.convs.{i}.bias", x, u.dim, co, cw, k, 1, k // 2)
            co += cw
        self.n_init_ops = len(self.ops)
        self.x0, self.base = x, self.f32(B * HW, u.dim, HW)
        full_ops, full_written, self.ops, self.written = self.ops, self.written, [], set()
        cws = [u.spec_shapes[f"init_conv.convs.{i}.weight"][0] for i in range(3)]
        if (u.initx_direct and u.fused and R % 8 == 0 and u.channels <= 4 and cws[0] in (64, 128)
                and cws[1] in (32, 64) and cws[2] in (32, 64) and "__init_xw__" in self.w):
            offs, woffs = [0, cws[0], cws[0] + cws[1]], u.initx_woffs
            self.op(OP_INITX, 0, p=(self.x_in.ptr, self.base.ptr, self.wptr("__init_xw__"), x.ptr),
                    i=(B, R, R, u.channels, u.dim, cws[0], cws[1], cws[2], offs[0], offs[1], offs[2], woffs[0], woffs[1], woffs[2]))
        else:
            xin_x = self.f32(B * HW, 32, HW)
            self.op(OP_ELTWISE, 2, p=(self.x_in.ptr, self.x_in.ptr, 0, xin_x.ptr), i=(B, HW, 0, u.channels, 32))
            co = 0
            for i, k in enumerate((3, 7, 15)):
                cw = cws[i]
                self.conv(xin_x, True, R, R, f"__init_x__.{i}", None, x, u.dim, co, cw, k, 1, k // 2, resid=self.base)
                co += cw
        self.init_x_ops, self.ops, self.written = self.ops, full_ops, full_written
        hiddens = []
        H = R
        n_lv = len(u.in_out)
        for lv, (di, do) in enumerate(u.in_out):
            x = self.resnet(f"downs.{lv}.1", x, None, di, H)
            for r in range(u.nres[lv]):
                x = self.resnet(f"downs.{lv}.2.{r}", x, None, di, H, gca=True)
                hiddens.append(x)
            if u.attns[lv]:
                x = self.transformer(f"downs.{lv}.3", x)
            hiddens.append(x)
            if lv < n_lv - 1:
                y = self.f32(B * (H // 2) ** 2, do, (H // 2) ** 2)
                self.conv(x, True, H, H, f"downs.{lv}.4.weight", f"downs.{lv}.4.bias", y, do, 0, do, 4, 2, 1, defer=bool(u.fused),
                          defer_max_groups=4 if (H // 2 == 4 and u.conv4) else 8)
                H //= 2
            else:
                y = self.f32(B * H * H, do, H * H)
                if (B == 1 and u.fused and u.conv4 and u.merged_down_conv4 and H == 4 and x.C == do == 1024
                        and x.rows == 16 and (x.lazy is None or x.lazy[0] != "splitk")):
                    self.need(x)
                    self.fconv(x, None, 4, f"downs.{lv}.4.__merged__.weight", f"downs.{lv}.4.__merged__.bias", y, do, 3, FNORM_NONE, (4, 1, 1, 4),
                               silu=False)
                else:
                    self.conv(x, True, H, H, f"downs.{lv}.4.__merged__.weight", f"downs.{lv}.4.__merged__.bias", y, do, 0, do, 3, 1, 1,
                              defer=bool(u.fused), defer_max_groups=4 if (H == 4 and u.conv4) else 8)
            x = y
        mid = x.C
        x = self.resnet("mid_block1", x, None, mid, H, cross=True)
        x = self.self_attention("mid_attn.fn.fn", x, False)
        x = self.resnet("mid_block2", x, None, mid, H, cross=True)
        for ui, lv in enumerate(reversed(range(n_lv))):
            di, do = u.in_out[lv]
            x = self.resnet(f"ups.{ui}.0", x, hiddens.pop(), do, H)
            for r in range(u.nres[lv]):
                x = self.resnet(f"ups.{ui}.1.{r}", x, hiddens.pop(), do, H, gca=True)
            if u.attns[lv]:
                x = self.transformer(f"ups.{ui}.2", x)
            if ui < n_lv - 1:
                y = self.f32(B * 4 * H * H, di, 4 * H * H)
                self.conv(x, True, H, H, f"ups.{ui}.3.net.0.weight", f"ups.{ui}.3.net.0.bias", y, di, 0, di * 4, 1, pixshuf=True,
                          want_slots=bool(u.fused and u.producer_slots))
                H *= 2
                x = y
        x = self.resnet("final_res_block", x, None, u.dim, H, gca=True)
        self.out = self.f32(B, u.channels * HW)
        _, _, fgroups = u.conv_tiling((B * HW + 15) // 16, (u.channels + 15) // 16, 9 * (x.C // 32), False)
        if u.producer_slots and fgroups > 1 and (u.channels + 15) // 16 < 4:
            o = _T(self.out.ptr, B * HW, u.channels, HW)
            self.conv(x, True, R, R, "final_conv.weight", "final_conv.bias", o, u.channels, 0, u.channels, 3, 1, 1, nchw=True)
            assert self.last_conv_nchw, "final conv: the split-K reduction was expected to write NCHW"
        else:
            o = self.f32(B * HW, u.channels, HW)
            self.conv(x, True, R, R, "final_conv.weight", "final_conv.bias", o, u.channels, 0, u.channels, 3, 1, 1)
            self.op(OP_ELTWISE, 3, p=(o.ptr, 0, 0, self.out.ptr), i=(B, HW, u.channels, u.channels))
        first = self.ops[self.n_init_ops] if self.n_init_ops < len(self.ops) else None
        if (u.producer_slots and first is not None and first.type == OP_SLOTS and first.p[0] == self.x0.ptr and not first.p[1]
                and not first.p[5] and self.x0.slots and len(self.init_x_ops) == 1 and self.init_x_ops[0].type == OP_INITX):
            self.init_x_ops[0].p[4] = self.x0.slots
            self.n_init_ops += 1
        memset_op.i[0] = (self.zero.off + 3) // 4
        if self.zero.off == 0:
            self.ops.remove(memset_op)
        self.op_array = (_lib.SfOp * len(self.ops))(*self.ops)
        n_init = self.n_init_ops - (1 if self.zero.off == 0 else 0)
        pre = [o for o in self.ops[self.n_time_ops:n_init] if o.type == OP_MEMSET]
        body = pre + self.init_x_ops + self.ops[n_init:]
        self.body_array, self.n_body_ops = (_lib.SfOp * len(body))(*body), len(body)
        init = self.ops[self.n_time_ops:n_init]
        self.init_array, self.n_init_run = (_lib.SfOp * len(init))(*init), len(init)
        if self.misc.buf is not None:
            self.tb_view = self.tview(self.tb)
            self.x_view, self.t_view = self.tview(self.x_in), self.tview(self.t_in)
            self.cond_view, self.out_view = self.tview(self.cond_in), self.tview(self.out)
            self.x0_view, self.base_view = self.tview(self.x0), self.tview(self.base)
        return self



class _TimePlan(_Plan):

    def build(self):
        T = self.B
        self.t_in = self.f32(T, 1)
        self.table = self.f32(T, self.u.tb_stride)
        self.emit_time(T, self.table.ptr, self.t_in.ptr)
        self.op_array = (_lib.SfOp * len(self.ops))(*self.ops)
        if self.misc.buf is not None:
            self.t_view, self.table_view = self.tview(self.t_in), self.tview(self.table)
        return self


class Unet(PlanOwner, nn.Module):
    def __init__(self, *, dim, dim_mults=(1, 2, 4, 8), num_resnet_blocks=1, layer_attns=True, layer_cross_attns=True,
                 cond_images_channels=0, channels=3, channels_out=None, attn_pool_text=True, cond_dim=None,
                 attn_dim_head=64, attn_heads=8, ff_mult=2., learned_sinu_pos_emb_dim=16, max_conditional_len=256,
                 cond_on_z=False, lowres_cond=False, image_size=32, **unsupported):
        super().__init__()
        n_lv = len(dim_mults)
        if any(_cast_tuple(layer_cross_attns, n_lv)) or lowres_cond or cond_on_z or cond_images_channels <= 0:
            raise NotImplementedError("sparsefusion_amd.Unet covers the SparseFusion configuration only "
                                      "(utils/load_model.py:58-69: image-conditioned, no text, no lowres, no layer cross-attn)")
        for k, v in unsupported.items():
            if k not in ("image_embed_dim", "conditional_embed_dim", "num_image_tokens", "num_time_tokens", "out_dim"):
                raise NotImplementedError(f"Unet keyword '{k}' is not supported by the HIP plan")
        if channels_out not in (None, channels):
            raise NotImplementedError("channels_out != channels")
        self.dim, self.channels, self.cond_images_channels = dim, channels, cond_images_channels
        self.channels_out = channels
        self.cond_dim = cond_dim or dim
        self.tdim = dim * 4
        self.attn_heads, self.attn_dim_head, self.ff_mult = attn_heads, attn_dim_head, ff_mult
        self.learned_sinu_pos_emb_dim = learned_sinu_pos_emb_dim
        self.image_size = image_size
        self.lowres_cond, self.cond_on_z, self.has_cond_image = False, False, True
        dims = [dim] + [dim * m for m in dim_mults]
        self.in_out = list(zip(dims[:-1], dims[1:]))
        self.nres = _cast_tuple(num_resnet_blocks, n_lv)
        self.attns = _cast_tuple(layer_attns, n_lv)
        self._locals = dict(dim=dim, dim_mults=tuple(dim_mults), num_resnet_blocks=num_resnet_blocks, layer_attns=layer_attns,
                            layer_cross_attns=layer_cross_attns, cond_images_channels=cond_images_channels, channels=channels,
                            attn_pool_text=attn_pool_text, cond_dim=cond_dim, attn_dim_head=attn_dim_head, attn_heads=attn_heads,
                            ff_mult=ff_mult, learned_sinu_pos_emb_dim=learned_sinu_pos_emb_dim,
                            max_conditional_len=max_conditional_len, image_size=image_size)
        if attn_heads * attn_dim_head != 512 or attn_dim_head != 64:
            raise NotImplementedError("attention kernel is built for 8 heads x 64")
        spec = unet_param_spec(dim, tuple(dim_mults), self.nres, self.attns, cond_images_channels, channels, self.cond_dim,
                               attn_heads, attn_dim_head, ff_mult, learned_sinu_pos_emb_dim, max_conditional_len)
        self.spec_shapes = dict(spec)
        g = torch.Generator().manual_seed(0)
        for name, shape in spec:
            _register(self, name, self._default_init(name, shape, g))
        self.ss_offset, off = {}, 0
        for name, shape in spec:
            if name.endswith(".time_mlp.1.weight"):
                self.ss_offset[name[:-len(".time_mlp.1.weight")]] = off
                off += shape[0]
        self.ss_total = off
        self.tb_off = {}
        for name, shape in spec:
            if name.endswith(".to_context.1.weight"):
                self.tb_off[name[:-len(".to_context.1.weight")]] = off
                off += 2 * shape[0]
            elif name.endswith(".cross_attn.fn.to_kv.weight"):
                self.tb_off[name[:-len(".to_kv.weight")]] = off
                off += 2 * shape[0]
        self.tb_stride = (off + 63) // 64 * 64
        for name, default, _ in SWITCHES:
            setattr(self, name, default)
        self._pack_cache = None
        self._plans = {}
        self.tile_override = dict(TILE_PICKS)
        self.igemm_t_variants = IGEMM_T_VARIANTS

    @staticmethod
    def _default_init(name, shape, g):
        if name.startswith("final_conv"):
            return torch.zeros(shape)
        if name.endswith(".g") or name.endswith("groupnorm.weight") or name in ("norm_cond.weight",) or name.endswith("to_context.0.weight"):
            return torch.ones(shape)
        if name.endswith("bias"):
            return torch.zeros(shape)
        if name.endswith("null_kv") or name.startswith("null_conditional") or name.endswith("weights"):
            return torch.randn(shape, generator=g)
        fan_in = int(np.prod(shape[1:])) if len(shape) > 1 else shape[0]
        return (torch.rand(shape, generator=g) * 2 - 1) / math.sqrt(fan_in)

    def set_switches(self, spec):
        pairs = [kv.split("=") for kv in spec.split(",") if kv]
        unknown = [name for name, _ in pairs if name not in {n for n, _, _ in SWITCHES}]
        if unknown:
            raise KeyError(f"Unet.set_switches: no planner switch named {unknown} (unet.SWITCHES)")
        for name, value in pairs:
            setattr(self, name, int(value))
        self.drop_plans()
        return self

    def cast_model_parameters(self, *, lowres_cond, conditional_embed_dim, channels, channels_out, cond_on_z):
        if lowres_cond or cond_on_z or channels != self.channels or channels_out != self.channels_out:
            raise NotImplementedError("only the first, unconditional-on-text unet of a cascade is supported")
        return self

    def to_config_and_state_dict(self):
        return self._locals, self.state_dict()

    @classmethod
    def from_config_and_state_dict(klass, config, state_dict):
        unet = klass(**config)
        unet.load_state_dict(state_dict)
        return unet

    def load_state_dict(self, *args, **kwargs):
        r = super().load_state_dict(*args, **kwargs)
        self.invalidate()
        return r

    def drop_plans(self):
        for plan in self._plans.values():
            plan.generation = -1
        self._plans = {}

    MAX_TIME_PLANS = 4

    def invalidate(self):
        for plan in self._plans.values():
            plan.generation = -1
        self._pack_cache, self._plans = None, {}
        self.__dict__["_table_cache"] = {}

    def _apply(self, fn, *a, **k):
        r = super()._apply(fn, *a, **k)
        self.invalidate()
        return r

    def _packed(self, device):
        if self._pack_cache is not None and self._pack_cache[0] == str(device):
            return self._pack_cache[1]
        lib = self.clib
        odt = _lib.operand_dtype(lib)
        packed = {}
        sd = {k: v.detach() for k, v in self.named_parameters()}
        tm_w, tm_b = [], []
        for name, w in sd.items():
            wc = w.float().cpu().contiguous()
            is_conv = name.endswith(".weight") and (
                w.dim() == 4 or any(s in name for s in (".to_q.", ".to_out.0.")) or
                (".to_kv." in name and ".cross_attn." not in name))
            if name.endswith(".time_mlp.1.weight"):
                tm_w.append(wc)
                tm_b.append(sd[name[:-6] + "bias"].float().cpu())
            elif name.endswith(".time_mlp.1.bias"):
                pass
            elif ".gca.to_k.weight" in name:
                packed[name] = wc.reshape(-1).to(device)
            elif ".gca.net." in name and name.endswith(".weight"):
                packed[name] = self._gemv_pack(wc.reshape(wc.shape[0], -1), device)
            elif is_conv:
                w4 = wc if wc.dim() == 4 else wc.reshape(wc.shape[0], wc.shape[1], 1, 1)
                co, ci, kh, kw = w4.shape
                cpad = (ci + 31) // 32 * 32
                n = lib.sf_conv_packed_elems(co, cpad, kh, kw)
                buf = torch.empty(n, dtype=torch.int16)
                _lib.check(lib.sf_conv_pack_weights(w4.data_ptr(), co, ci, cpad, kh, kw, buf.data_ptr()), "pack " + name)
                packed[name] = buf.to(device)
            elif name.endswith(".weight") and w.dim() == 2:
                packed[name] = self._gemv_pack(wc, device)
            else:
                packed[name] = wc.reshape(-1).to(device)
        for name in [k[:-len(".to_kv.weight")] for k in sd if k.endswith(".to_kv.weight") and ".cross_attn." not in k]:
            wq, wkv = sd[name + ".to_q.weight"].float().cpu(), sd[name + ".to_kv.weight"].float().cpu()
            w4 = torch.cat([wq, wkv], 0).contiguous()
            co, ci = w4.shape
            if ci % 32 == 0:
                buf = torch.empty(lib.sf_conv_packed_elems(co, ci, 1, 1), dtype=torch.int16)
                _lib.check(lib.sf_conv_pack_weights(w4.data_ptr(), co, ci, ci, 1, 1, buf.data_ptr()), "pack qkv " + name)
                packed[name + ".__qkv__"] = buf.to(device)
        for name in [k[:-len(".fns.0.weight")] for k in sd if k.endswith(".fns.0.weight")]:
            w3, w1 = sd[name + ".fns.0.weight"].float().cpu().clone(), sd[name + ".fns.1.weight"].float().cpu()
            w3[:, :, 1, 1] += w1[:, :, 0, 0]
            co, ci, kh, kw = w3.shape
            cpad = (ci + 31) // 32 * 32
            buf = torch.empty(lib.sf_conv_packed_elems(co, cpad, kh, kw), dtype=torch.int16)
            _lib.check(lib.sf_conv_pack_weights(w3.contiguous().data_ptr(), co, ci, cpad, kh, kw, buf.data_ptr()), "pack merged " + name)
            packed[name + ".__merged__.weight"] = buf.to(device)
            packed[name + ".__merged__.bias"] = (sd[name + ".fns.0.bias"].float().cpu() + sd[name + ".fns.1.bias"].float().cpu()).to(device)
        for name in [k[:-len(".gca.to_k.weight")] for k in sd if k.endswith(".gca.to_k.weight")]:
            w2c = sd.get(name + ".block2.project.weight")
            if w2c is not None and w2c.shape[1] % 32 == 0 and tuple(w2c.shape[2:]) == (3, 3):
                wk = sd[name + ".gca.to_k.weight"].float().cpu().reshape(-1)
                weff = torch.einsum("n,ncyx->yxc", wk, w2c.float().cpu()).reshape(-1).to(odt).contiguous()
                packed[name + ".__weff__"] = weff.to(device)
        for i in range(3):
            w4 = sd[f"init_conv.convs.{i}.weight"].float().cpu()[:, self.cond_images_channels:].contiguous()
            co, ci, kh, kw = w4.shape
            buf = torch.empty(lib.sf_conv_packed_elems(co, 32, kh, kw), dtype=torch.int16)
            _lib.check(lib.sf_conv_pack_weights(w4.data_ptr(), co, ci, 32, kh, kw, buf.data_ptr()), "pack init x")
            packed[f"__init_x__.{i}"] = buf.to(device)
        if self.channels <= 4:
            tab, self.initx_woffs = init_x_weight_table([sd[f"init_conv.convs.{i}.weight"].float().cpu()[:, self.cond_images_channels:]
                                                         for i in range(3)], dtype=odt)
            packed["__init_xw__"] = tab.to(device)
        packed["__time_mlps__.weight"] = self._gemv_pack(torch.cat(tm_w, 0), device)
        packed["__time_mlps__.bias"] = torch.cat(tm_b, 0).to(device)
        self._pack_cache = (str(device), packed)
        return packed

    def _gemv_pack(self, w2, device):
        K = w2.shape[1]
        Kp = (K + 7) // 8 * 8
        if Kp != K:
            w2 = torch.nn.functional.pad(w2, (0, Kp - K))
        return w2.to(_lib.operand_dtype(self.clib)).contiguous().to(device)

    def set_operand(self, operand):
        if operand not in (None, "bf16", "f16"):
            raise ValueError("operand must be None, 'bf16' or 'f16'")
        self._operand_override = operand
        self.invalidate()
        return self

    @property
    def operand(self):
        ov = getattr(self, "_operand_override", None)
        if ov is not None:
            return ov
        p = next(self.parameters(), None)
        return "f16" if (p is not None and p.dtype == torch.float16) else None

    @property
    def clib(self):
        return _lib.lib(self.operand)

    def _plan(self, B, device):
        key = (B, str(device))
        if key not in self._plans:
            sizing = _Plan(self, B, device).build()
            plan = _Plan(self, B, device, (sizing.zero.off, sizing.misc.off + sizing.ws_bytes + sizing.ws2_bytes + 512,
                                           sizing.ws_bytes, sizing.ws2_bytes)).build()
            plan.generation = 0
            self._plans[key] = plan
        return self._plans[key]

    @torch.no_grad()
    def forward(self, x, time, *, cond_images=None, cond_drop_prob=0., **unsupported):
        if cond_images is None:
            raise AssertionError("you requested to condition on an image on the unet, but the conditioning image is not supplied")
        for k, v in unsupported.items():
            if v is not None:
                raise NotImplementedError(f"Unet.forward argument '{k}' is not supported")
        _lib.require_cuda(x, time, cond_images)
        B = x.shape[0]
        assert x.shape[1:] == (self.channels, self.image_size, self.image_size), x.shape
        assert cond_images.shape[1] == self.cond_images_channels, \
            'the number of channels on the conditioning image you are passing in does not match'
        if cond_images.shape[-1] != self.image_size:
            cond_images = torch.nn.functional.interpolate(cond_images, self.image_size, mode='nearest')
        if cond_drop_prob != 0.:
            if cond_drop_prob >= 1.:
                keep = torch.zeros(B, dtype=torch.bool, device=x.device)
            else:
                keep = torch.zeros(B, device=x.device).float().uniform_(0, 1) < (1 - cond_drop_prob)
            cond_images = cond_images * keep.view(B, 1, 1, 1)
        plan = self._plan(B, x.device)
        plan.generation += 1
        plan.x_view.copy_(x.reshape(B, -1))
        plan.t_view.copy_(time.reshape(-1).expand(B).reshape(B, 1))
        plan.cond_view.copy_(cond_images.reshape(B, -1))
        if self.use_hip_graph and not torch.cuda.is_current_stream_capturing():
            if plan.graph is None:
                self._run_plan(plan)
                torch.cuda.synchronize()
                g = torch.cuda.CUDAGraph()
                with torch.cuda.graph(g, capture_error_mode="thread_local"):
                    self._run_plan(plan)
                plan.graph = g
            plan.graph.replay()
        else:
            self._run_plan(plan)
        y = plan.out_view.clone().view(B, self.channels, self.image_size, self.image_size)
        return y if x.dtype == torch.float32 else y.to(x.dtype)

    @staticmethod
    def _run_plan(plan, body_only=False):
        if body_only:
            _lib.check(plan.u.clib.sf_plan_run(plan.body_array, plan.n_body_ops, _lib.stream_ptr()), "unet plan", plan.u.clib)
        else:
            _lib.check(plan.u.clib.sf_plan_run(plan.op_array, len(plan.ops), _lib.stream_ptr()), "unet plan", plan.u.clib)

    def _time_plan(self, T, device):
        key = ("time", T, str(device))
        if key not in self._plans:
            old = [k for k in self._plans if k[0] == "time"]
            for k in old[:max(0, len(old) + 1 - self.MAX_TIME_PLANS)]:
                del self._plans[k]
            sizing = _TimePlan(self, T, device).build()
            self._plans[key] = _TimePlan(self, T, device, (sizing.zero.off, sizing.misc.off + 512, 0, 0)).build()
        else:
            self._plans[key] = self._plans.pop(key)
        return self._plans[key]

    @torch.no_grad()
    def time_table(self, log_snrs, key=None):
        _lib.require_cuda(log_snrs)
        ck = None
        if key is not None:
            ck = (key, str(log_snrs.device), self.operand)
            hit = self.__dict__.get("_table_cache", {}).get(ck)
            if hit is not None:
                cache = self.__dict__["_table_cache"]
# ... 67 lines not shown
```

### sparsefusion_amd/vae.py

```python
import math

import numpy as np
import os

import torch
import torch.nn as nn

from . import _lib
from .plan import OP_ELTWISE, OP_MEMSET, Plan, PlanOwner, _T
from .unet import _register

SD_VAE_DDCONFIG = dict(double_z=True, z_channels=4, resolution=256, in_channels=3, out_ch=3, ch=128, ch_mult=(1, 2, 4, 4),
                       num_res_blocks=2, attn_resolutions=(), dropout=0.0)


def _resnet_spec(out, p, cin, cout):
    out += [(f"{p}.norm1.weight", (cin,)), (f"{p}.norm1.bias", (cin,)), (f"{p}.conv1.weight", (cout, cin, 3, 3)),
            (f"{p}.conv1.bias", (cout,)), (f"{p}.norm2.weight", (cout,)), (f"{p}.norm2.bias", (cout,)),
            (f"{p}.conv2.weight", (cout, cout, 3, 3)), (f"{p}.conv2.bias", (cout,))]
    if cin != cout:
        out += [(f"{p}.nin_shortcut.weight", (cout, cin, 1, 1)), (f"{p}.nin_shortcut.bias", (cout,))]


def _attn_spec(out, p, c):
    out += [(f"{p}.norm.weight", (c,)), (f"{p}.norm.bias", (c,))]
    for n in ("q", "k", "v", "proj_out"):
        out += [(f"{p}.{n}.weight", (c, c, 1, 1)), (f"{p}.{n}.bias", (c,))]


def vae_param_spec(*, ch, ch_mult, num_res_blocks, in_channels, out_ch, z_channels, embed_dim, double_z=True, **_):
    mult = tuple(ch_mult)
    out = [("encoder.conv_in.weight", (ch, in_channels, 3, 3)), ("encoder.conv_in.bias", (ch,))]
    in_mult = (1,) + mult
    block_in = ch
    for lv in range(len(mult)):
        block_in, block_out = ch * in_mult[lv], ch * mult[lv]
        for b in range(num_res_blocks):
            _resnet_spec(out, f"encoder.down.{lv}.block.{b}", block_in, block_out)
            block_in = block_out
        if lv != len(mult) - 1:
            out += [(f"encoder.down.{lv}.downsample.conv.weight", (block_in, block_in, 3, 3)),
                    (f"encoder.down.{lv}.downsample.conv.bias", (block_in,))]
    _resnet_spec(out, "encoder.mid.block_1", block_in, block_in)
    _attn_spec(out, "encoder.mid.attn_1", block_in)
    _resnet_spec(out, "encoder.mid.block_2", block_in, block_in)
    zo = 2 * z_channels if double_z else z_channels
    out += [("encoder.norm_out.weight", (block_in,)), ("encoder.norm_out.bias", (block_in,)),
            ("encoder.conv_out.weight", (zo, block_in, 3, 3)), ("encoder.conv_out.bias", (zo,))]
    block_in = ch * mult[-1]
    out += [("decoder.conv_in.weight", (block_in, z_channels, 3, 3)), ("decoder.conv_in.bias", (block_in,))]
    _resnet_spec(out, "decoder.mid.block_1", block_in, block_in)
    _attn_spec(out, "decoder.mid.attn_1", block_in)
    _resnet_spec(out, "decoder.mid.block_2", block_in, block_in)
    levels = {}
    for lv in reversed(range(len(mult))):
        cur = []
        for b in range(num_res_blocks + 1):
            _resnet_spec(cur, f"decoder.up.{lv}.block.{b}", block_in, ch * mult[lv])
            block_in = ch * mult[lv]
        if lv != 0:
            cur += [(f"decoder.up.{lv}.upsample.conv.weight", (block_in, block_in, 3, 3)),
                    (f"decoder.up.{lv}.upsample.conv.bias", (block_in,))]
        levels[lv] = cur
    for lv in range(len(mult)):
        out += levels[lv]
    out += [("decoder.norm_out.weight", (block_in,)), ("decoder.norm_out.bias", (block_in,)),
            ("decoder.conv_out.weight", (out_ch, block_in, 3, 3)), ("decoder.conv_out.bias", (out_ch,)),
            ("quant_conv.weight", (2 * embed_dim, 2 * z_channels, 1, 1)), ("quant_conv.bias", (2 * embed_dim,)),
            ("post_quant_conv.weight", (z_channels, embed_dim, 1, 1)), ("post_quant_conv.bias", (z_channels,))]
    return out


class _VaePlan(Plan):

    def __init__(self, vae, kind, B, device, sizing=None):
        super().__init__(vae, B, device, sizing)
        self.kind = kind

    def gn(self, x, name, out, silu=True):
        self.gn_act(x, None, name, 0, out, None, silu=silu, groups=32, eps=1e-6)

    def conv3(self, x, x_f32, H, name, out, cout, resid=None, twin=None):
        self.conv(x, x_f32, H, H, name + ".weight", name + ".bias", out, cout, 0, cout, 3, 1, 1, resid=resid, twin=twin)

    def resnet_block(self, p, x, cout, H, twin=False):
        rows, HW, cin = x.rows, H * H, x.C
        a1 = self.bf16(rows, cin, HW)
        self.gn(x, p + ".norm1", a1)
        h = self.f32(rows, cout, HW)
        self.conv3(a1, False, H, p + ".conv1", h, cout)
        a2 = self.bf16(rows, cout, HW)
        self.gn(h, p + ".norm2", a2)
        out = self.f32(rows, cout, HW)
        tw = self.bf16(rows, cout, HW) if twin else None
        if cin != cout:
            xs = x.twin if self.u.conv_twin else None
            self.conv(xs if xs is not None else x, xs is None, H, H, p + ".nin_shortcut.weight", p + ".nin_shortcut.bias", out, cout, 0, cout, 1)
            self.conv3(a2, False, H, p + ".conv2", out, cout, twin=tw)
        else:
            self.conv3(a2, False, H, p + ".conv2", out, cout, resid=x, twin=tw)
        return out

    def attn_block(self, p, x, H):
        B, HW, C = self.B, H * H, x.C
        rows = x.rows
        hn = self.bf16(rows, C, HW)
        self.gn(x, p + ".norm", hn, silu=False)
        q, k, v = (self.f32(rows, C, HW) for _ in range(3))
        for t, n in ((q, "q"), (k, "k"), (v, "v")):
            self.conv(hn, False, H, H, f"{p}.{n}.weight", f"{p}.{n}.bias", t, C, 0, C, 1)
        att = self.f32(rows, C, HW)
        lib = _lib.lib()
        kp_elems = lib.sf_conv_packed_elems(HW, C, 1, 1)
        vp_elems = lib.sf_conv_packed_elems(C, (HW + 31) // 32 * 32, 1, 1)
        hwp = (HW + 31) // 32 * 32
        for b in range(B):
            kp = self.misc.alloc(kp_elems * 2)
            vp = self.misc.alloc(vp_elems * 2)
            s = self.f32(HW, HW)
            pr = _T(self.misc.alloc(HW * hwp * 2), HW, hwp)
            qb, kb, vb = (_T(t.ptr + b * HW * C * 4, HW, C, HW) for t in (q, k, v))
            ob = _T(att.ptr + b * HW * C * 4, HW, C, HW)
            self.op(OP_ELTWISE, 5, p=(kb.ptr, 0, 0, kp), i=(HW, C, C, 0))
            self.op(OP_ELTWISE, 5, p=(vb.ptr, 0, 0, vp), i=(C, HW, C, 1))
            self.conv(qb, True, 1, HW, None, None, s, HW, 0, HW, 1, w_ptr=kp, batch=1)
            if hwp != HW:
                raise NotImplementedError("AttnBlock token count must be a multiple of 32")
            self.op(OP_ELTWISE, 6, p=(s.ptr, 0, 0, pr.ptr), i=(HW, HW), f=(float(int(C) ** (-0.5)),))
            self.conv(pr, False, 1, HW, None, None, ob, C, 0, C, 1, w_ptr=vp, batch=1)
        out = self.f32(rows, C, HW)
        self.conv(att, True, H, H, p + ".proj_out.weight", p + ".proj_out.bias", out, C, 0, C, 1, resid=x)
        return out

    def build(self):
        v, B = self.u, self.B
        mult, nres, ch = v.ch_mult, v.num_res_blocks, v.ch
        n_lv = len(mult)
        self.op(OP_MEMSET, 0, p=(self.zero.buf.data_ptr() if self.zero.buf is not None else 1,), i=(0,))
        memset_op = self.ops[-1]
        if self.kind == "enc":
            R = v.resolution
            HW = R * R
            self.x_in = self.f32(B, v.in_channels * HW)
            xin = self.f32(B * HW, 32, HW)
            self.op(OP_ELTWISE, 2, p=(0, self.x_in.ptr, 0, xin.ptr), i=(B, HW, 0, v.in_channels, 32))
            h = self.f32(B * HW, ch, HW)
            self.conv3(xin, True, R, "encoder.conv_in", h, ch)
            H = R
            for lv in range(n_lv):
                for b in range(nres):
                    h = self.resnet_block(f"encoder.down.{lv}.block.{b}", h, ch * mult[lv], H,
                                          twin=(b == nres - 1 and lv != n_lv - 1 and v.conv_twin))
                if lv != n_lv - 1:
                    y = self.f32(B * (H // 2) ** 2, h.C, (H // 2) ** 2)
                    src = h.twin
                    ytw = self.bf16(y.rows, h.C, y.HW) if (v.conv_twin and ch * mult[lv + 1] != h.C) else None
                    self.conv(src if src is not None else h, src is None, H, H, f"encoder.down.{lv}.downsample.conv.weight",
                              f"encoder.down.{lv}.downsample.conv.bias", y, h.C, 0, h.C, 3, 2, 0, out_hw=(H // 2, H // 2), twin=ytw)
                    h, H = y, H // 2
            h = self.resnet_block("encoder.mid.block_1", h, h.C, H)
            h = self.attn_block("encoder.mid.attn_1", h, H)
            h = self.resnet_block("encoder.mid.block_2", h, h.C, H)
            a = self.bf16(h.rows, h.C, H * H)
            self.gn(h, "encoder.norm_out", a)
            zo = 2 * v.z_channels
            mo = _T(self.zero.alloc(h.rows * 32 * 4), h.rows, 32, H * H)
            self.conv(a, False, H, H, "encoder.conv_out.weight", "encoder.conv_out.bias", mo, 32, 0, zo, 3, 1, 1)
            qm = self.f32(h.rows, 2 * v.embed_dim, H * H)
            self.conv(mo, True, H, H, "quant_conv.weight", "quant_conv.bias", qm, 2 * v.embed_dim, 0, 2 * v.embed_dim, 1)
            self.out = self.f32(B, 2 * v.embed_dim * H * H)
            self.op(OP_ELTWISE, 3, p=(qm.ptr, 0, 0, self.out.ptr), i=(B, H * H, 2 * v.embed_dim, 2 * v.embed_dim))
            self.out_shape = (2 * v.embed_dim, H, H)
        else:
            H = v.resolution // 2 ** (n_lv - 1)
            HW = H * H
            self.x_in = self.f32(B, v.embed_dim * HW)
            zin = self.f32(B * HW, 32, HW)
            self.op(OP_ELTWISE, 2, p=(0, self.x_in.ptr, 0, zin.ptr), i=(B, HW, 0, v.embed_dim, 32))
            z = _T(self.zero.alloc(B * HW * 32 * 4), B * HW, 32, HW)
            self.conv(zin, True, H, H, "post_quant_conv.weight", "post_quant_conv.bias", z, 32, 0, v.z_channels, 1)
            block_in = ch * mult[-1]
            h = self.f32(B * HW, block_in, HW)
            self.conv3(z, True, H, "decoder.conv_in", h, block_in)
            h = self.resnet_block("decoder.mid.block_1", h, block_in, H)
            h = self.attn_block("decoder.mid.attn_1", h, H)
            h = self.resnet_block("decoder.mid.block_2", h, block_in, H)
            for lv in reversed(range(n_lv)):
                for b in range(nres + 1):
                    h = self.resnet_block(f"decoder.up.{lv}.block.{b}", h, ch * mult[lv], H, twin=(b == nres and lv != 0 and v.conv_twin))
                if lv != 0:
                    y = self.f32(B * 4 * H * H, h.C, 4 * H * H)
                    src = h.twin
                    ytw = self.bf16(y.rows, h.C, y.HW) if (v.conv_twin and ch * mult[lv - 1] != h.C) else None
                    self.conv(src if src is not None else h, src is None, 2 * H, 2 * H, f"decoder.up.{lv}.upsample.conv.weight",
                              f"decoder.up.{lv}.upsample.conv.bias", y, h.C, 0, h.C, 3, 1, 1, upsampled=True, twin=ytw)
                    h, H = y, 2 * H
            a = self.bf16(h.rows, h.C, H * H)
            self.gn(h, "decoder.norm_out", a)
            o = self.f32(h.rows, v.out_ch, H * H)
            self.conv3(a, False, H, "decoder.conv_out", o, v.out_ch)
            self.out = self.f32(B, v.out_ch * H * H)
            self.op(OP_ELTWISE, 3, p=(o.ptr, 0, 0, self.out.ptr), i=(B, H * H, v.out_ch, v.out_ch))
            self.out_shape = (v.out_ch, H, H)
        memset_op.i[0] = (self.zero.off + 3) // 4
        self.op_array = (_lib.SfOp * len(self.ops))(*self.ops)
        if self.misc.buf is not None:
            self.x_view, self.out_view = self.tview(self.x_in), self.tview(self.out)
        return self


class DiagonalGaussianDistribution:

    def __init__(self, parameters, deterministic=False):
        self.parameters = parameters
        self.mean, self.logvar = torch.chunk(parameters, 2, dim=1)
        self.logvar = torch.clamp(self.logvar, -30.0, 20.0)
        self.deterministic = deterministic
        self.std = torch.exp(0.5 * self.logvar)
        self.var = torch.exp(self.logvar)
        if self.deterministic:
            self.var = self.std = torch.zeros_like(self.mean)

    def sample(self):
        return self.mean + self.std * torch.randn(self.mean.shape, device=self.parameters.device)

    def mode(self):
        return self.mean

    def kl(self, other=None):
        if self.deterministic:
            return torch.Tensor([0.])
        if other is None:
            return 0.5 * torch.sum(torch.pow(self.mean, 2) + self.var - 1.0 - self.logvar, dim=[1, 2, 3])
        return 0.5 * torch.sum(torch.pow(self.mean - other.mean, 2) / other.var + self.var / other.var - 1.0 - self.logvar
                               + other.logvar, dim=[1, 2, 3])


class AutoencoderKL(PlanOwner, nn.Module):

    def __init__(self, ddconfig=None, lossconfig=None, embed_dim=4, ckpt_path=None, ignore_keys=(), **unsupported):
        super().__init__()
        dd = dict(SD_VAE_DDCONFIG if ddconfig is None else ddconfig)
        if not dd.get("double_z", True):
            raise NotImplementedError("AutoencoderKL asserts double_z (autoencoder.py:300)")
        if list(dd.get("attn_resolutions", ())):
            raise NotImplementedError("attn_resolutions is empty in sd-vae.yaml; per-level attention is not planned")
        if dd.get("dropout", 0.0) != 0.0:
            raise NotImplementedError("dropout is a training feature")
        self.ch, self.ch_mult, self.num_res_blocks = dd["ch"], tuple(dd["ch_mult"]), dd["num_res_blocks"]
        self.in_channels, self.out_ch, self.z_channels = dd["in_channels"], dd["out_ch"], dd["z_channels"]
        self.resolution, self.embed_dim = dd["resolution"], embed_dim
        if self.ch % 128 or self.in_channels > 32 or 2 * self.z_channels > 32:
            raise NotImplementedError("HIP plan: ch must be a multiple of 128 (GroupNorm(32) with >= 4 channels per group)")
        g = torch.Generator().manual_seed(0)
        self.spec_shapes = {}
        for name, shape in vae_param_spec(embed_dim=embed_dim, **dd):
            self.spec_shapes[name] = tuple(shape)
            _register(self, name, nn.Parameter(self._default_init(name, shape, g), requires_grad=False))
        self.lds_conv_min_blocks = 96
        self.conv_twin = True
        self.gn_epilogue = True
        self._pack_cache, self._plans = None, {}
        if ckpt_path is not None:
            self.init_from_ckpt(ckpt_path, ignore_keys=ignore_keys)

    @staticmethod
    def _default_init(name, shape, g):
        if ".norm" in name:
            return torch.ones(shape) if name.endswith("weight") else torch.zeros(shape)
        fan_in = int(np.prod(shape[1:])) if len(shape) > 1 else shape[0]
        bound = 1.0 / math.sqrt(fan_in)
        if name.endswith("bias"):
            return torch.zeros(shape)
        return (torch.rand(shape, generator=g) * 2 - 1) * bound

    def init_from_ckpt(self, path, ignore_keys=()):
        sd = torch.load(path, map_location="cpu")["state_dict"]
        for k in list(sd.keys()):
            if any(k.startswith(ik) for ik in ignore_keys):
                del sd[k]
        self.load_state_dict(sd, strict=False)

    def load_state_dict(self, *args, **kwargs):
        r = super().load_state_dict(*args, **kwargs)
        self.invalidate()
        return r

    def invalidate(self):
        self._pack_cache, self._plans = None, {}

    def _apply(self, fn, *a, **k):
        r = super()._apply(fn, *a, **k)
        self.invalidate()
        return r

    def _packed(self, device):
        if self._pack_cache is not None and self._pack_cache[0] == str(device):
            return self._pack_cache[1]
        lib = _lib.lib()
        packed = {}
        for name, w in self.named_parameters():
            wc = w.detach().float().cpu().contiguous()
            if wc.dim() == 4:
                co, ci, kh, kw = wc.shape
                cpad = (ci + 31) // 32 * 32
                buf = torch.empty(lib.sf_conv_packed_elems(co, cpad, kh, kw), dtype=torch.int16)
                _lib.check(lib.sf_conv_pack_weights(wc.data_ptr(), co, ci, cpad, kh, kw, buf.data_ptr()), "pack " + name)
                packed[name] = buf.to(device)
            else:
                packed[name] = wc.reshape(-1).to(device)
        self._pack_cache = (str(device), packed)
        return packed

    def _plan(self, kind, B, device):
        key = (kind, B, str(device))
        if key not in self._plans:
            sizing = _VaePlan(self, kind, B, device).build()
            self._plans[key] = _VaePlan(self, kind, B, device,
                                        (sizing.zero.off, sizing.misc.off + sizing.ws_bytes + 256, sizing.ws_bytes)).build()
        return self._plans[key]

    def _run(self, kind, x):
        _lib.require_cuda(x)
        B = x.shape[0]
        plan = self._plan(kind, B, x.device)
        plan.x_view.copy_(x.reshape(B, -1))
        _lib.check(_lib.lib().sf_plan_run(plan.op_array, len(plan.ops), _lib.stream_ptr()), f"vae {kind} plan")
        return plan.out_view.clone().view(B, *plan.out_shape)

    @torch.no_grad()
    def encode(self, x):
        assert x.shape[1:] == (self.in_channels, self.resolution, self.resolution), x.shape
        return DiagonalGaussianDistribution(self._run("enc", x.float()))

    @torch.no_grad()
    def decode(self, z):
        f = 2 ** (len(self.ch_mult) - 1)
        assert z.shape[1:] == (self.embed_dim, self.resolution // f, self.resolution // f), z.shape
        return self._run("dec", z.float())

    def forward(self, input, sample_posterior=True):
        posterior = self.encode(input)
        z = posterior.sample() if sample_posterior else posterior.mode()
        return self.decode(z), posterior
```

Before: 18.16.

## Group time-table LayerNorms and GEMVs into single launches; add per-pixel GN apply for VAE

Adds grouped kernels (k_layernorm_grp, k_gemm_rows_ks_grp) so the sampler's time-table to_context LayerNorms and k/v projections each run as one launch instead of many, cutting kernel launch overhead. It also adds a per-image, per-pixel-slab GroupNorm apply kernel, enabled for the VAE, that hoists stats, gamma/beta and scale-shift loads out of the inner loop and drops per-element index division. Grouped GEMV pads every member to the widest N, so some blocks exit early, and the plan executor now has to walk grouped ops and record events for each member.

```diff
diff --git a/sparsefusion_amd/csrc/attn_ln.h b/sparsefusion_amd/csrc/attn_ln.h
--- a/sparsefusion_amd/csrc/attn_ln.h
+++ b/sparsefusion_amd/csrc/attn_ln.h
@@ -1,12 +1,11 @@
 #pragma once
 #include "sf_dev.h"
 
-SF_KERNEL(256) void k_layernorm(const float* __restrict__ in, const float* __restrict__ gain,
-                                                   const float* __restrict__ bias, void* __restrict__ out,
-                                                   const float* __restrict__ resid, int R, int C, float eps, int pre_gelu,
-                                                   int out_f32) {
+SF_DEV void layernorm_body(const float* __restrict__ in, const float* __restrict__ gain, const float* __restrict__ bias,
+                           void* __restrict__ out, const float* __restrict__ resid, const int row, int C, float eps, int pre_gelu,
+                           int out_f32) {
   SF_SHARED float red[8];
-  const int row = blockIdx.x, lane = threadIdx.x & 63, wv = threadIdx.x >> 6;
+  const int lane = threadIdx.x & 63, wv = threadIdx.x >> 6;
   const float* x = in + (long)row * C;
   float v[8];
   float s = 0.0f;
@@ -42,6 +41,26 @@
       }
     }
   }
+}
+
+SF_KERNEL(256) void k_layernorm(const float* __restrict__ in, const float* __restrict__ gain,
+                                                   const float* __restrict__ bias, void* __restrict__ out,
+                                                   const float* __restrict__ resid, int R, int C, float eps, int pre_gelu,
+                                                   int out_f32) {
+  layernorm_body(in, gain, bias, out, resid, (int)blockIdx.x, C, eps, pre_gelu, out_f32);
+}
+
+#define LN_GROUP_MAX 16
+struct LnGroup {
+  const float* in[LN_GROUP_MAX];
+  const float* gain[LN_GROUP_MAX];
+  const float* bias[LN_GROUP_MAX];
+  void* out[LN_GROUP_MAX];
+};
+
+SF_KERNEL(256) void k_layernorm_grp(LnGroup g, int R, int C, float eps, int pre_gelu, int out_f32) {
+  const int set = sf_uniform((int)blockIdx.x / R), row = sf_uniform((int)blockIdx.x - set * R);
+  layernorm_body(g.in[set], g.gain[set], g.bias[set], g.out[set], nullptr, row, C, eps, pre_gelu, out_f32);
 }
 
 template <int NV>
diff --git a/sparsefusion_amd/csrc/gemm_rows.h b/sparsefusion_amd/csrc/gemm_rows.h
--- a/sparsefusion_amd/csrc/gemm_rows.h
+++ b/sparsefusion_amd/csrc/gemm_rows.h
@@ -91,7 +91,7 @@
 };
 
 template <int NW>
-SF_KERNEL(NW * 64) void k_gemm_rows_ks(GemmRowsArgs a) {
+SF_DEV void gemm_rows_ks_body(const GemmRowsArgs& a, const int bx) {
   using Gk = GemmRowsKs<NW>;
   constexpr int MFMAX = Gk::MFMAX;
   SF_DYN_LDS(lds);
@@ -100,7 +100,7 @@
   sf_opnd* lo = hi + Gk::ROWS * GR_LD;
   float* red = reinterpret_cast<float*>(lds + NW * Gk::WAVE_ELEMS * 2);
   const int n = lane & 15, g = lane >> 4;
-  const int ncol = blockIdx.x * 16 + n;
+  const int ncol = bx * 16 + n;
   const sf_opnd* __restrict__ wrow = a.W + (long)min(ncol, a.N - 1) * a.Kp;
   const int MF = (a.M + 15) >> 4;
   const bool vec = (a.ldx & 3) == 0 && (a.K & 7) == 0 && (reinterpret_cast<uintptr_t>(a.x) & 15) == 0;
@@ -218,3 +218,20 @@
       }
     }
 }
+
+template <int NW>
+SF_KERNEL(NW * 64) void k_gemm_rows_ks(GemmRowsArgs a) { gemm_rows_ks_body<NW>(a, (int)blockIdx.x); }
+
+#define GR_GROUP_MAX 16
+struct GemmRowsGroup {
+  GemmRowsArgs set[GR_GROUP_MAX];
+  int n, nbx;
+};
+
+template <int NW>
+SF_KERNEL(NW * 64) void k_gemm_rows_ks_grp(GemmRowsGroup g) {
+  const int set = sf_uniform((int)blockIdx.x / g.nbx), bx = sf_uniform((int)blockIdx.x - set * g.nbx);
+  const GemmRowsArgs a = g.set[set];
+  if (bx * 16 >= a.N) return;
+  gemm_rows_ks_body<NW>(a, bx);
+}
diff --git a/sparsefusion_amd/csrc/gn_apply.h b/sparsefusion_amd/csrc/gn_apply.h
--- /dev/null
+++ b/sparsefusion_amd/csrc/gn_apply.h
@@ -0,0 +1,99 @@
+#pragma once
+#include "sf_dev.h"
+
+SF_DEV f32x4 gn_load(const float* __restrict__ s1, const float* __restrict__ s2, int b, int HW, int C1, int C2, int p, int c,
+                     float s2_scale) {
+  if (c < C1) return *reinterpret_cast<const f32x4*>(s1 + ((long)b * HW + p) * C1 + c);
+  f32x4 v = *reinterpret_cast<const f32x4*>(s2 + ((long)b * HW + p) * C2 + (c - C1));
+  return v * s2_scale;
+}
+
+SF_KERNEL(256) void k_gn_apply(const float* __restrict__ s1, const float* __restrict__ s2,
+                               const float* __restrict__ gamma, const float* __restrict__ beta,
+                               const float* __restrict__ ss, const double* __restrict__ stats,
+                               sf_opnd* __restrict__ out, sf_opnd* __restrict__ raw, int B, int HW, int C1,
+                               int C2, int ss_stride, float eps, float s2_scale, int no_silu, int G) {
+  const int C = C1 + C2, Cg = C / G, c4 = C / 4;
+  const long total = (long)B * HW * c4;
+  const double inv_n = 1.0 / ((double)HW * Cg);
+  for (long i = blockIdx.x * 256L + threadIdx.x; i < total; i += (long)gridDim.x * 256) {
+    const int c = (int)(i % c4) * 4;
+    const long bp = i / c4;
+    const int p = (int)(bp % HW), b = (int)(bp / HW);
+    const int g = c / Cg;
+    const double m = stats[(b * G + g) * 2] * inv_n;
+    const double var = stats[(b * G + g) * 2 + 1] * inv_n - m * m;
+    const float mean = (float)m, rstd = sf_rsqrt((float)(var > 0.0 ? var : 0.0) + eps);
+    const f32x4 v = gn_load(s1, s2, b, HW, C1, C2, p, c, s2_scale);
+    const f32x4 ga = *reinterpret_cast<const f32x4*>(gamma + c), be = *reinterpret_cast<const f32x4*>(beta + c);
+    bf16x4 o, r;
+#pragma unroll
+    for (int j = 0; j < 4; ++j) {
+      float y = (v[j] - mean) * rstd * ga[j] + be[j];
+      if (ss) y = y * (ss[(long)b * ss_stride + c + j] + 1.0f) + ss[(long)b * ss_stride + C + c + j];
+      if (!no_silu) y = sf_silu(y);
+      o[j] = (sf_opnd)y;
+      r[j] = (sf_opnd)v[j];
+    }
+    *reinterpret_cast<bf16x4*>(out + ((long)b * HW + p) * C + c) = o;
+    if (raw) *reinterpret_cast<bf16x4*>(raw + ((long)b * HW + p) * C + c) = r;
+  }
+}
+
+#define GN_PX_U 4
+template <int C4>
+SF_KERNEL(256) void k_gn_apply_px(const float* __restrict__ s1, const float* __restrict__ gamma, const float* __restrict__ beta,
+                                  const float* __restrict__ ss, const double* __restrict__ stats, sf_opnd* __restrict__ out,
+                                  sf_opnd* __restrict__ raw, int HW, int ss_stride, float eps, int no_silu, int G, int ppw, int wpi) {
+  constexpr int C = 4 * C4, PPI = 256 / C4;
+  const int b = (int)blockIdx.x / wpi, sl = (int)blockIdx.x - b * wpi;
+  const int c = ((int)threadIdx.x % C4) * 4, pofs = (int)threadIdx.x / C4;
+  const int Cg = C / G, g = c / Cg;
+  const int p0 = sl * ppw, p1 = p0 + ppw < HW ? p0 + ppw : HW;
+  const double inv_n = 1.0 / ((double)HW * Cg);
+  const double m = stats[(b * G + g) * 2] * inv_n;
+  const double var = stats[(b * G + g) * 2 + 1] * inv_n - m * m;
+  const float mean = (float)m, rstd = sf_rsqrt((float)(var > 0.0 ? var : 0.0) + eps);
+  const f32x4 ga = *reinterpret_cast<const f32x4*>(gamma + c), be = *reinterpret_cast<const f32x4*>(beta + c);
+  f32x4 sc = {0.0f, 0.0f, 0.0f, 0.0f}, sh = {0.0f, 0.0f, 0.0f, 0.0f};
+  if (ss) {
+#pragma unroll
+    for (int j = 0; j < 4; ++j) { sc[j] = ss[(long)b * ss_stride + c + j] + 1.0f; sh[j] = ss[(long)b * ss_stride + C + c + j]; }
+  }
+  const long img = (long)b * HW * C + c;
+  const float* __restrict__ src = s1 + img;
+  sf_opnd* __restrict__ dst = out + img;
+  sf_opnd* __restrict__ rdst = raw ? raw + img : nullptr;
+  for (int p = p0 + pofs; p < p1; p += PPI * GN_PX_U) {
+    f32x4 v[GN_PX_U];
+#pragma unroll
+    for (int u = 0; u < GN_PX_U; ++u) {
+      const int pu = p + u * PPI;
+      if (pu < p1) v[u] = *reinterpret_cast<const f32x4*>(src + pu * C);
+    }
+#pragma unroll
+    for (int u = 0; u < GN_PX_U; ++u) {
+      const int pu = p + u * PPI;
+      if (pu >= p1) break;
+      bf16x4 o, r;
+#pragma unroll
+      for (int j = 0; j < 4; ++j) {
+        float y = (v[u][j] - mean) * rstd * ga[j] + be[j];
+        if (ss) y = y * sc[j] + sh[j];
+        if (!no_silu) y = sf_silu(y);
+        o[j] = (sf_opnd)y;
+        r[j] = (sf_opnd)v[u][j];
+      }
+      *reinterpret_cast<bf16x4*>(dst + pu * C) = o;
+      if (rdst) *reinterpret_cast<bf16x4*>(rdst + pu * C) = r;
+    }
+  }
+}
+
+static inline int gn_px_ppw(int B, int HW, int c4) {
+  const int ppi = 256 / c4;
+  int k = GN_PX_U;
+  while ((long)B * ((HW + ppi * k - 1) / (ppi * k)) > 2048) k *= 2;
+  while (k > 1 && (long)B * ((HW + ppi * k - 1) / (ppi * k)) < 512) k /= 2;
+  return ppi * k;
+}
diff --git a/sparsefusion_amd/csrc/unet_ops.hip b/sparsefusion_amd/csrc/unet_ops.hip
--- a/sparsefusion_amd/csrc/unet_ops.hip
+++ b/sparsefusion_amd/csrc/unet_ops.hip
@@ -3,6 +3,7 @@
 #include "plan_ops.h"
 #include "sf_dev.h"
 #include "gemm_rows.h"
+#include "gn_apply.h"
 #include "conv_halo.h"
 #include "conv_halo_small.h"
 #include "conv_igemm.h"
@@ -81,13 +82,6 @@
   return v;
 }
 
-__device__ __forceinline__ f32x4 gn_load(const float* __restrict__ s1, const float* __restrict__ s2, int b, int HW, int C1,
-                                         int C2, int p, int c, float s2_scale) {
-  if (c < C1) return *reinterpret_cast<const f32x4*>(s1 + ((long)b * HW + p) * C1 + c);
-  f32x4 v = *reinterpret_cast<const f32x4*>(s2 + ((long)b * HW + p) * C2 + (c - C1));
-  return v * s2_scale;
-}
-
 __global__ __launch_bounds__(256) void k_gn_stats(float* __restrict__ s1, const float* __restrict__ s2,
                                                   double* __restrict__ stats, int HW, int C1, int C2, int slices,
                                                   float s2_scale, LazySrc lz, int G) {
@@ -147,37 +141,6 @@
   }
 }
 
-__global__ __launch_bounds__(256) void k_gn_apply(const float* __restrict__ s1, const float* __restrict__ s2,
-                                                  const float* __restrict__ gamma, const float* __restrict__ beta,
-                                                  const float* __restrict__ ss, const double* __restrict__ stats,
-                                                  sf_opnd* __restrict__ out, sf_opnd* __restrict__ raw, int B, int HW, int C1,
-                                                  int C2, int ss_stride, float eps, float s2_scale, int no_silu, int G) {
-  const int C = C1 + C2, Cg = C / G, c4 = C / 4;
-  const long total = (long)B * HW * c4;
-  const double inv_n = 1.0 / ((double)HW * Cg);
-  for (long i = blockIdx.x * 256L + threadIdx.x; i < total; i += (long)gridDim.x * 256) {
-    const int c = (int)(i % c4) * 4;
-    const long bp = i / c4;
-    const int p = (int)(bp % HW), b = (int)(bp / HW);
-    const int g = c / Cg;
-    const double m = stats[(b * G + g) * 2] * inv_n;
-    const double var = stats[(b * G + g) * 2 + 1] * inv_n - m * m;
-    const float mean = (float)m, rstd = rsqrtf((float)(var > 0.0 ? var : 0.0) + eps);
-    const f32x4 v = gn_load(s1, s2, b, HW, C1, C2, p, c, s2_scale);
-    const f32x4 ga = *reinterpret_cast<const f32x4*>(gamma + c), be = *reinterpret_cast<const f32x4*>(beta + c);
-    bf16x4 o, r;
-#pragma unroll
-    for (int j = 0; j < 4; ++j) {
-      float y = (v[j] - mean) * rstd * ga[j] + be[j];
-      if (ss) y = y * (ss[(long)b * ss_stride + c + j] + 1.0f) + ss[(long)b * ss_stride + C + c + j];
-      if (!no_silu) y = silu_f(y);
-      o[j] = (sf_opnd)y;
-      r[j] = (sf_opnd)v[j];
-    }
-    *reinterpret_cast<bf16x4*>(out + ((long)b * HW + p) * C + c) = o;
-    if (raw) *reinterpret_cast<bf16x4*>(raw + ((long)b * HW + p) * C + c) = r;
-  }
-}
 
 template <int NT, int NCH>
 __global__ __launch_bounds__(NT) void k_gn_one(float* __restrict__ s1, const float* __restrict__ s2, const float* __restrict__ gamma,
@@ -699,6 +662,18 @@
                                                op.f[1], lz, G);
   }
   SF_CHECK_LAUNCH("gn_stats");
+  if ((op.flags & 16) && !op.p[1] && !lz.mode && (c4 == 32 || c4 == 64 || c4 == 128) && (long)HW * C < (1L << 31) &&
+      !(((uintptr_t)op.p[0] | (uintptr_t)op.p[2] | (uintptr_t)op.p[3]) & 15) && !(((uintptr_t)op.p[5] | (uintptr_t)op.p[6]) & 7)) {
+    const int ppw = gn_px_ppw(B, HW, c4), wpi = (HW + ppw - 1) / ppw;
+#define SF_GN_PX(C4) k_gn_apply_px<C4><<<B * wpi, 256, 0, st>>>((const float*)op.p[0], (const float*)op.p[2], (const float*)op.p[3], (const float*)op.p[4], \
+                                                           (const double*)op.p[7], (sf_opnd*)op.p[5], (sf_opnd*)op.p[6], HW, op.i[4], op.f[0], op.flags & 1, G, ppw, wpi)
+    if (c4 == 32) SF_GN_PX(32);
+    else if (c4 == 64) SF_GN_PX(64);
+    else SF_GN_PX(128);
+#undef SF_GN_PX
+    SF_CHECK_LAUNCH("gn_apply_px");
+    return SF_OK;
+  }
   const long total = (long)B * HW * (C / 4);
   k_gn_apply<<<sf_grid_cap(sf_div_up(total, 256)), 256, 0, st>>>(
       (const float*)op.p[0], (const float*)op.p[1], (const float*)op.p[2], (const float*)op.p[3], (const float*)op.p[4],
@@ -732,6 +707,21 @@
   return SF_OK;
 }
 
+static int gemm_rows_ks_lds_limit() {
+  static unsigned mask = 0;
+  int dev = 0;
+  if (hipGetDevice(&dev) != hipSuccess) SF_FAIL(SF_ERR_LAUNCH, "hipGetDevice failed");
+  if (dev >= 32 || !(mask & (1u << dev))) {
+    if (hipFuncSetAttribute(reinterpret_cast<const void*>(&k_gemm_rows_ks<4>), hipFuncAttributeMaxDynamicSharedMemorySize, GemmRowsKs<4>::LDS_BYTES) != hipSuccess ||
+        hipFuncSetAttribute(reinterpret_cast<const void*>(&k_gemm_rows_ks<8>), hipFuncAttributeMaxDynamicSharedMemorySize, GemmRowsKs<8>::LDS_BYTES) != hipSuccess ||
+        hipFuncSetAttribute(reinterpret_cast<const void*>(&k_gemm_rows_ks_grp<4>), hipFuncAttributeMaxDynamicSharedMemorySize, GemmRowsKs<4>::LDS_BYTES) != hipSuccess ||
+        hipFuncSetAttribute(reinterpret_cast<const void*>(&k_gemm_rows_ks_grp<8>), hipFuncAttributeMaxDynamicSharedMemorySize, GemmRowsKs<8>::LDS_BYTES) != hipSuccess)
+      SF_FAIL(SF_ERR_LAUNCH, "gemv: cannot raise the dynamic LDS limit of k_gemm_rows_ks");
+    if (dev < 32) mask |= 1u << dev;
+  }
+  return SF_OK;
+}
+
 static int run_gemv(const sf_op& op, hipStream_t st) {
   const int M = op.i[0], N = op.i[1];
   if (M > 64) SF_FAIL(SF_ERR_INVALID, "gemv: at most 64 rows");
@@ -741,15 +731,7 @@
     if (a.Kp < 8 || a.Kp % 8) SF_FAIL(SF_ERR_INVALID, "gemv: padded K must be a multiple of 8");
     if (N <= 4096 && !(op.flags & 8)) {
       const bool w8 = M <= 32 && a.K > 4 * GR_KC;
-      static unsigned mask = 0;
-      int dev = 0;
-      if (hipGetDevice(&dev) != hipSuccess) SF_FAIL(SF_ERR_LAUNCH, "hipGetDevice failed");
-      if (dev >= 32 || !(mask & (1u << dev))) {
-        if (hipFuncSetAttribute(reinterpret_cast<const void*>(&k_gemm_rows_ks<4>), hipFuncAttributeMaxDynamicSharedMemorySize, GemmRowsKs<4>::LDS_BYTES) != hipSuccess ||
-            hipFuncSetAttribute(reinterpret_cast<const void*>(&k_gemm_rows_ks<8>), hipFuncAttributeMaxDynamicSharedMemorySize, GemmRowsKs<8>::LDS_BYTES) != hipSuccess)
-          SF_FAIL(SF_ERR_LAUNCH, "gemv: cannot raise the dynamic LDS limit of k_gemm_rows_ks");
-        if (dev < 32) mask |= 1u << dev;
-      }
+      if (int rc = gemm_rows_ks_lds_limit()) return rc;
       if (w8) k_gemm_rows_ks<8><<<sf_div_up(N, 16), 512, GemmRowsKs<8>::LDS_BYTES, st>>>(a);
       else k_gemm_rows_ks<4><<<sf_div_up(N, 16), 256, GemmRowsKs<4>::LDS_BYTES, st>>>(a);
       SF_CHECK_LAUNCH("gemm_rows_ks");
@@ -766,6 +748,52 @@
     k_gemv<4><<<sf_div_up(N, 16), 256, 0, st>>>((const float*)op.p[0], (const sf_opnd*)op.p[1], (const float*)op.p[2], (float*)op.p[3], M,
                                                N, op.i[2], op.i[3], op.i[4], op.i[5], op.flags & 1, (op.flags >> 1) & 3);
   SF_CHECK_LAUNCH("gemv");
+  return SF_OK;
+}
+
+static int run_gemv_group(const sf_op* ops, int n, hipStream_t st) {
+  const sf_op& h = ops[0];
+  const int M = h.i[0], K = h.i[2], Kp = h.i[3], fl = h.flags & ~16;
+  if (n < 2 || n > GR_GROUP_MAX) SF_FAIL(SF_ERR_INVALID, "gemv group: %d members (2 .. %d)", n, GR_GROUP_MAX);
+  if (M <= 8 || M > 64 || (fl & ~7) || Kp < 8 || Kp % 8 || K < 1 || K > Kp) SF_FAIL(SF_ERR_INVALID, "gemv group: needs 9 .. 64 rows on k_gemm_rows_ks");
+  GemmRowsGroup g;
+  memset(&g, 0, sizeof(g));
+  int nmax = 0;
+  for (int j = 0; j < n; ++j) {
+    const sf_op& op = ops[j];
+    if (op.type != SF_OP_GEMV || (op.flags & ~16) != fl || (j && (op.flags & 16)) || op.i[0] != M || op.i[2] != K || op.i[3] != Kp || op.i[1] < 1 ||
+        op.i[1] > 4096 || !op.p[0] || !op.p[1] || !op.p[3])
+      SF_FAIL(SF_ERR_INVALID, "gemv group: member %d does not match its head", j);
+    g.set[j] = GemmRowsArgs{(const float*)op.p[0], (const sf_opnd*)op.p[1], (const float*)op.p[2], (float*)op.p[3], M, op.i[1], K, Kp, op.i[4],
+                            op.i[5], (int)(fl & 1), (int)((fl >> 1) & 3)};
+    nmax = op.i[1] > nmax ? op.i[1] : nmax;
+  }
+  g.n = n;
+  g.nbx = (int)sf_div_up(nmax, 16);
+  if (int rc = gemm_rows_ks_lds_limit()) return rc;
+  if (M <= 32 && K > 4 * GR_KC) k_gemm_rows_ks_grp<8><<<g.nbx * n, 512, GemmRowsKs<8>::LDS_BYTES, st>>>(g);
+  else k_gemm_rows_ks_grp<4><<<g.nbx * n, 256, GemmRowsKs<4>::LDS_BYTES, st>>>(g);
+  SF_CHECK_LAUNCH("gemm_rows_ks_grp");
+  return SF_OK;
+}
+
+static int run_ln_group(const sf_op* ops, int n, hipStream_t st) {
+  const sf_op& h = ops[0];
+  const int R = h.i[0], C = h.i[1], fl = h.flags & ~8;
+  if (n < 2 || n > LN_GROUP_MAX) SF_FAIL(SF_ERR_INVALID, "layernorm group: %d members (2 .. %d)", n, LN_GROUP_MAX);
+  if (R < 1 || C % 64 || C > 2048 || (C == 256 && R >= 1024) || (R <= 256 && (C == 512 || C == 1024 || C == 2048) && !(fl & 4)))
+    SF_FAIL(SF_ERR_INVALID, "layernorm group: needs a shape that runs on k_layernorm");
+  LnGroup g;
+  memset(&g, 0, sizeof(g));
+  for (int j = 0; j < n; ++j) {
+    const sf_op& op = ops[j];
+    if (op.type != SF_OP_LN || (op.flags & ~8) != fl || (j && (op.flags & 8)) || op.i[0] != R || op.i[1] != C || op.f[0] != h.f[0] || !op.p[0] ||
+        !op.p[1] || !op.p[3] || op.p[4] || op.p[5])
+      SF_FAIL(SF_ERR_INVALID, "layernorm group: member %d does not match its head", j);
+    g.in[j] = (const float*)op.p[0]; g.gain[j] = (const float*)op.p[1]; g.bias[j] = (const float*)op.p[2]; g.out[j] = op.p[3];
+  }
+  k_layernorm_grp<<<R * n, 256, 0, st>>>(g, R, C, h.f[0], fl & 1, (fl & 2) ? 1 : 0);
+  SF_CHECK_LAUNCH("layernorm_grp");
   return SF_OK;
 }
 
@@ -855,8 +883,19 @@
     switch (op.type) {
       case SF_OP_CONV: rc = run_conv(op, st); break;
       case SF_OP_GN_ACT: rc = run_gn(op, st); break;
-      case SF_OP_LN: rc = run_ln(op, st); break;
-      case SF_OP_GEMV: rc = run_gemv(op, st); break;
+      case SF_OP_LN:
+      case SF_OP_GEMV: {
+        const bool ln = op.type == SF_OP_LN;
+        if (!(op.flags & (ln ? 8 : 16))) { rc = ln ? run_ln(op, st) : run_gemv(op, st); break; }
+        const int n = ln ? op.i[2] : op.i[6];
+        if (n < 2 || k + (uint32_t)n > n_ops) SF_FAIL(SF_ERR_INVALID, "plan: op %u heads a group of %d ops that the plan does not hold", k, n);
+        rc = ln ? run_ln_group(&op, n, st) : run_gemv_group(&op, n, st);
+        for (int j = 1; j < n && !rc; ++j) {
+          ++k;
+          if (ev && hipEventRecord(ev[k], st) != hipSuccess) SF_FAIL(SF_ERR_LAUNCH, "plan: hipEventRecord failed");
+        }
+        break;
+      }
       case SF_OP_ATTN: rc = run_attn(op, st); break;
       case SF_OP_GCA_POOL: rc = run_gca_pool(op, st); break;
       case SF_OP_ELTWISE: rc = run_eltwise(op, st); break;
diff --git a/sparsefusion_amd/plan.py b/sparsefusion_amd/plan.py
--- a/sparsefusion_amd/plan.py
+++ b/sparsefusion_amd/plan.py
@@ -40,6 +40,7 @@
     lds_mid_min_batch = 8
     gn_epilogue = False
     gn_one = True
+    gn_apply_px = False
     ln_wave = True
     tb_stride = 0
     lazy_consumers = 0
@@ -243,7 +244,8 @@
             wr.i[15] = cg
             self.op(OP_GN_FINALIZE, 0, p=(part, stats), i=(self.B, x.HW // 128, groups))
             ready = 2
-        self.op(OP_GN_ACT, (0 if silu else 1) | ready | (0 if self.u.gn_one else 4),
+        px = 16 if (self.u.gn_apply_px and not skip and li[0] == 0 and C1 in (128, 256, 512)) else 0
+        self.op(OP_GN_ACT, (0 if silu else 1) | ready | (0 if self.u.gn_one else 4) | px,
                 p=(x.ptr, skip.ptr if skip else 0, self.wptr(gname + ".weight"), self.wptr(gname + ".bias"), ss_ptr, out.ptr,
                    raw.ptr if raw else 0, stats) + lp,
                 i=(self.B, x.HW, C1, C2, self.u.tb_stride) + li + (groups,), f=(eps, SKIP_SCALE))
@@ -265,6 +267,33 @@
             self.op(OP_GEMV, (1 if in_silu else 0) | (out_act << 1),
                     p=(x_ptr + m0 * ldx * 4, self.wptr(wname), self.wptr(bname) if bname else 0, y_ptr + m0 * ldy * 4),
                     i=(mm, N, K, Kp, ldx, ldy))
+
+    def ln_group(self, sets, C, rows, eps=1e-5):
+        first = len(self.ops)
+        for x, gname, bname, out in sets:
+            self.ln(x, gname, bname, out, C, rows, eps=eps, out_f32=True)
+        ops = self.ops[first:]
+        wave = self.u.ln_wave and rows <= 256 and C in (512, 1024, 2048)
+        if len(ops) == len(sets) and not wave and not (C == 256 and rows >= 1024):
+            for j in range(0, len(ops), 16):
+                if len(ops[j:j + 16]) > 1:
+                    ops[j].flags |= 8
+                    ops[j].i[2] = len(ops[j:j + 16])
+
+    def gemv_group(self, sets):
+        M = sets[0][1]
+        assert all(s[1] == M and s[8] == sets[0][8] and s[9:] == sets[0][9:] for s in sets)
+        for m0 in range(0, M, 8 if M <= 8 else 64):
+            first = len(self.ops)
+            for x_ptr, _, ldx, wname, bname, y_ptr, ldy, N, K, *act in sets:
+                mm = min(8 if M <= 8 else 64, M - m0)
+                self.gemv(x_ptr + m0 * ldx * 4, mm, ldx, wname, bname, y_ptr + m0 * ldy * 4, ldy, N, K, *act)
+            ops = self.ops[first:]
+            if ops[0].i[0] > 8 and all(o.i[1] <= 4096 for o in ops):
+                for j in range(0, len(ops), 16):
+                    if len(ops[j:j + 16]) > 1:
+                        ops[j].flags |= 16
+                        ops[j].i[6] = len(ops[j:j + 16])
 
     def attn(self, q, out, segs, heads, ldq, scale, out_f32=False):
         p = [q.ptr, out.ptr]
diff --git a/sparsefusion_amd/unet.py b/sparsefusion_amd/unet.py
--- a/sparsefusion_amd/unet.py
+++ b/sparsefusion_amd/unet.py
@@ -37,6 +37,7 @@
     ("merged_down_conv4", True, "r06: the merged 3x3 + 1x1 conv of the last Downsample on k_conv4_gn<64, 0, false> at B = 1; False: k_conv_igemm"),
     ("rc_small_tiles", 32, "r06: bit mask of map sides (32 | 16 | 8) whose B >= 2 (conv1 || res_conv) pairs keep the B = 1 tile of k_conv3s_rc (32: B = 2 eval 1.155 -> 1.139 ms, B = 4 1.562 -> 1.520; 32 | 16: B = 4 1.580, B = 8 2.451 -> 2.550)"),
     ("gn_one", True, "r06: GroupNorm passes of B >= 32 plans (B * 8 >= 256 workgroups) in one launch (k_gn_one); False: k_gn_stats + k_gn_apply everywhere"),
+    ("time_group", True, "a sampler's time table (_TimePlan): the to_context LayerNorms as one grouped launch, the k / v projections as another (k_layernorm_grp, k_gemm_rows_ks_grp: same bits); False: one launch each"),
     ("lds_mid_min_batch", 8, "... in plans of at least this many images (the B = 1 .. 4 plans keep their measured kernels)"),
     ("unfused_min_rows_4", 256, "r06: 4x4-level ResnetBlocks with B*16 >= this leave the fused kernels (as unfused_min_rows at 32x32 / 16x16; measured: B = 8 loses 0.12 ms, B = 16 gains 0.22, B = 32 0.49); 0 = never"),
     ("unfused_min_rows_8", 1024, "... 8x8 level (k_conv3_halo_sm; measured: B = 8 loses 0.14 ms, B = 16 gains 0.04, B = 32 0.56)"),
@@ -660,7 +661,7 @@
         self.conv(xn3, False, 1, rows // B, f"{name}.layers.0.1.4.weight", None, x2, d, 0, d, 1, resid=x1)
         return x2
 
-    def emit_time(self, rows, tb_ptr, t_ptr):
+    def emit_time(self, rows, tb_ptr, t_ptr, group=False):
         u = self.u
         st = u.tb_stride
         half = u.learned_sinu_pos_emb_dim // 2
@@ -674,16 +675,27 @@
         c = self.f32(2 * rows, u.cond_dim)
         self.ln(tok, "norm_cond.weight", "norm_cond.bias", c, u.cond_dim, 2 * rows, out_f32=True)
         self.gemv(t.ptr, rows, u.tdim, "__time_mlps__.weight", "__time_mlps__.bias", tb_ptr, st, u.ss_total, u.tdim, in_silu=True)
+        lns, kvs = [], []
         for name, off in u.tb_off.items():
             if name.endswith(".cross_attn.fn"):
                 n_out, src, wname, bname = 2 * heads * dh, c, f"{name}.to_kv.weight", None
             else:
                 src = self.f32(2 * rows, u.cond_dim)
-                self.ln(c, f"{name}.to_context.0.weight", f"{name}.to_context.0.bias", src, u.cond_dim, 2 * rows, out_f32=True)
+                if group:
+                    lns.append((c, f"{name}.to_context.0.weight", f"{name}.to_context.0.bias", src))
+                else:
+                    self.ln(c, f"{name}.to_context.0.weight", f"{name}.to_context.0.bias", src, u.cond_dim, 2 * rows, out_f32=True)
                 n_out, wname, bname = 2 * dh, f"{name}.to_context.1.weight", f"{name}.to_context.1.bias"
             for tk in range(2):
-                self.gemv(src.ptr + tk * u.cond_dim * 4, rows, 2 * u.cond_dim, wname, bname, tb_ptr + (off + tk * n_out) * 4, st,
-                          n_out, u.cond_dim)
+                kv = (src.ptr + tk * u.cond_dim * 4, rows, 2 * u.cond_dim, wname, bname, tb_ptr + (off + tk * n_out) * 4, st, n_out, u.cond_dim)
+                if group:
+                    kvs.append(kv)
+                else:
+                    self.gemv(*kv)
+        if lns:
+            self.ln_group(lns, u.cond_dim, 2 * rows)
+        if kvs:
+            self.gemv_group(kvs)
 
     def build(self):
         u, B = self.u, self.B
@@ -810,7 +822,7 @@
         T = self.B
         self.t_in = self.f32(T, 1)
         self.table = self.f32(T, self.u.tb_stride)
-        self.emit_time(T, self.table.ptr, self.t_in.ptr)
+        self.emit_time(T, self.table.ptr, self.t_in.ptr, group=bool(self.u.time_group))
         self.op_array = (_lib.SfOp * len(self.ops))(*self.ops)
         if self.misc.buf is not None:
             self.t_view, self.table_view = self.tview(self.t_in), self.tview(self.table)
diff --git a/sparsefusion_amd/vae.py b/sparsefusion_amd/vae.py
--- a/sparsefusion_amd/vae.py
+++ b/sparsefusion_amd/vae.py
@@ -260,6 +260,7 @@
         self.lds_conv_min_blocks = 96
         self.conv_twin = True
         self.gn_epilogue = True
+        self.gn_apply_px = True
         self._pack_cache, self._plans = None, {}
         if ckpt_path is not None:
             self.init_from_ckpt(ckpt_path, ignore_keys=ignore_keys)
```

New measurement: 18.18 (median of 6 runs). Within noise of the previous version (+0.1%).
